# KevinSpevak/openVO

Hardware: AMD Instinct MI355X
Metric: stereo frame-pairs/sec (1280x720) (higher is better)
Workload: dtype int16

## Files before the change

openvo_amd/csrc/match.hip:

```cpp
#include "vo_internal.h"

typedef int v4i __attribute__((ext_vector_type(4)));

#define NIB(x, i) ((__umul24(__builtin_amdgcn_ubfe((x), 4 * (i), 4), 0x00204081u)) & 0x01010101u)
__device__ __forceinline__ void expand64(uint32_t lo, uint32_t hi, v4i (&o)[4])
{
    o[0] = (v4i){ (int)NIB(lo, 0), (int)NIB(lo, 1), (int)NIB(lo, 2), (int)NIB(lo, 3) };
    o[1] = (v4i){ (int)NIB(lo, 4), (int)NIB(lo, 5), (int)NIB(lo, 6), (int)NIB(lo, 7) };
    o[2] = (v4i){ (int)NIB(hi, 0), (int)NIB(hi, 1), (int)NIB(hi, 2), (int)NIB(hi, 3) };
    o[3] = (v4i){ (int)NIB(hi, 4), (int)NIB(hi, 5), (int)NIB(hi, 6), (int)NIB(hi, 7) };
}
#undef NIB

__device__ __forceinline__ uint32_t med3_u32(uint32_t a, uint32_t b, uint32_t c)
{
    uint32_t r;
    asm("v_med3_u32 %0, %1, %2, %3" : "=v"(r) : "v"(a), "v"(b), "v"(c));
    return r;
}

__device__ __forceinline__ void merge2(uint32_t& a0, uint32_t& a1, uint32_t b0, uint32_t b1)
{
    const uint32_t hi = max(a0, b0);
    a0 = min(a0, b0);
// ... 408 lines not shown
{
    if (!ctx || nq < 0 || nt < 0 || (nq && (!q || !idx || !dist)) || (nt && !t)) return vo_fail(ctx, VO_E_ARG, "vo_bf_knn2_hamming: bad argument");
    if (nq > ctx->kp_cap || nt > ctx->kp_cap) return vo_fail(ctx, VO_E_CAP, "descriptor count exceeds capacity %d", ctx->kp_cap);
    if (nq == 0) return VO_OK;
    VO_HIP(ctx, hipSetDevice(ctx->device));
    StageTimer tm(ctx, VO_T_MATCH);
    int rc = xfer_h2d(ctx, ctx->mq, q, (size_t)nq * 32);
    if (!rc && nt) rc = xfer_h2d(ctx, ctx->mt, t, (size_t)nt * 32);
    if (rc) return rc;
    rc = match_knn2(ctx, ctx->mq, nq, ctx->mt, nt, ctx->mw->m_idx, ctx->mw->m_dist);
    if (rc) return rc;
    rc = xfer_d2h(ctx, idx, ctx->mw->m_idx, (size_t)nq * 8);
    if (!rc) rc = xfer_d2h(ctx, dist, ctx->mw->m_dist, (size_t)nq * 8);
    if (rc) return rc;
    return xfer_flush(ctx);
}

__global__ void k_mutual_decode(const int32_t* __restrict__ idx, int nq, const uint32_t* __restrict__ colmin, const uint8_t* __restrict__ t, int nt,
                                uint8_t* __restrict__ mutual, int32_t* __restrict__ t_best)
{
    const int i = blockIdx.x * blockDim.x + threadIdx.x;
    if (i < nq) mutual[i] = knn_mutual(idx[2 * i], i, colmin, nt) ? 1 : 0;
    if (i < nt) {
        const uint32_t key = colmin[i];
        const uint4* tp = (const uint4*)(t + (size_t)i * 32);
        const uint4 a = tp[0], b = tp[1];
        const int tn = __popc(a.x) + __popc(a.y) + __popc(a.z) + __popc(a.w) + __popc(b.x) + __popc(b.y) + __popc(b.z) + __popc(b.w);
        const bool h = key != 0xFFFFFFFFu;
        t_best[2 * i] = h ? (int32_t)(key & 0xFFFFu) : -1;
        t_best[2 * i + 1] = h ? (int32_t)(key >> 16) - 256 + tn : 0x7FFFFFFF;
    }
}

extern "C" int vo_bf_knn2_hamming_mutual(vo_ctx* ctx, const uint8_t* q, int nq, const uint8_t* t, int nt, int32_t* idx, int32_t* dist,
                                         uint8_t* mutual, int32_t* t_best)
{
    if (!ctx || nq < 0 || nt < 0 || (nq && (!q || !idx || !dist || !mutual)) || (nt && !t))
        return vo_fail(ctx, VO_E_ARG, "vo_bf_knn2_hamming_mutual: bad argument");
    if (nq > ctx->kp_cap || nt > ctx->kp_cap) return vo_fail(ctx, VO_E_CAP, "descriptor count exceeds capacity %d", ctx->kp_cap);
    if (nq > 65535) return vo_fail(ctx, VO_E_CAP, "cross-check: query set of %d descriptors exceeds 65535", nq);
    if (t_best)
        for (int j = 0; j < nt; j++) { t_best[2 * j] = -1; t_best[2 * j + 1] = 0x7FFFFFFF; }
    if (nq == 0) return VO_OK;
    VO_HIP(ctx, hipSetDevice(ctx->device));
    StageTimer tm(ctx, VO_T_MATCH);
    int rc = xfer_h2d(ctx, ctx->mq, q, (size_t)nq * 32);
    if (!rc && nt) rc = xfer_h2d(ctx, ctx->mt, t, (size_t)nt * 32);
    if (rc) return rc;
    if ((rc = match_knn2(ctx, ctx->mq, nq, ctx->mt, nt, ctx->mw->m_idx, ctx->mw->m_dist, 1))) return rc;
    int32_t* d_tbest = (int32_t*)ctx->mw->xy_a;
    hipLaunchKernelGGL(k_mutual_decode, dim3(div_up(std::max(nq, std::max(nt, 1)), 256)), dim3(256), 0, ctx->stream, ctx->mw->m_idx, nq,
                       match_colmin(ctx->mw->m_dist, ctx->kp_cap), ctx->mt, nt, ctx->mw->st_a, d_tbest);
    VO_CHECK_LAUNCH(ctx);
    rc = xfer_d2h(ctx, idx, ctx->mw->m_idx, (size_t)nq * 8);
    if (!rc) rc = xfer_d2h(ctx, dist, ctx->mw->m_dist, (size_t)nq * 8);
    if (!rc) rc = xfer_d2h(ctx, mutual, ctx->mw->st_a, (size_t)nq);
    if (!rc && t_best && nt) rc = xfer_d2h(ctx, t_best, d_tbest, (size_t)nt * 8);
    if (rc) return rc;
    return xfer_flush(ctx);
}

extern "C" int vo_bf_knn2_hamming_window(vo_ctx* ctx, const uint8_t* q, int nq, const uint8_t* t, int nt, const float* xy_q, const float* xy_t, float rx,
                                         float ry, int match_flags, int32_t* idx, int32_t* dist, uint8_t* mutual, int32_t* t_best)
{
    const int cross = match_flags & VO_MATCH_CROSSCHECK;
    if (!ctx || nq < 0 || nt < 0 || (nq && (!q || !xy_q || !idx || !dist || (cross && !mutual))) || (nt && (!t || !xy_t)) ||
        (match_flags & ~(VO_MATCH_CROSSCHECK | VO_MATCH_WINDOW)))
        return vo_fail(ctx, VO_E_ARG, "vo_bf_knn2_hamming_window: bad argument");
    if (!(rx >= 0.f) || !(ry >= 0.f) || rx > 3.4028234e38f || ry > 3.4028234e38f)
        return vo_fail(ctx, VO_E_ARG, "vo_bf_knn2_hamming_window: the radii must be finite and >= 0");
    if (nq > ctx->kp_cap || nt > ctx->kp_cap) return vo_fail(ctx, VO_E_CAP, "descriptor count exceeds capacity %d", ctx->kp_cap);
    if (cross && nq > 65535) return vo_fail(ctx, VO_E_CAP, "cross-check: query set of %d descriptors exceeds 65535", nq);
    if (cross && t_best)
        for (int j = 0; j < nt; j++) { t_best[2 * j] = -1; t_best[2 * j + 1] = 0x7FFFFFFF; }
    if (nq == 0) return VO_OK;
    VO_HIP(ctx, hipSetDevice(ctx->device));
    StageTimer tm(ctx, VO_T_MATCH);
    int rc = xfer_h2d(ctx, ctx->mq, q, (size_t)nq * 32);
    if (!rc) rc = xfer_h2d(ctx, ctx->mw->xy_a, xy_q, (size_t)nq * 8);
    if (!rc && nt) rc = xfer_h2d(ctx, ctx->mt, t, (size_t)nt * 32);
    if (!rc && nt) rc = xfer_h2d(ctx, ctx->mw->xy_b, xy_t, (size_t)nt * 8);
    if (rc) return rc;
    if ((rc = match_knn2(ctx, ctx->mq, nq, ctx->mt, nt, ctx->mw->m_idx, ctx->mw->m_dist, cross, ctx->mw->xy_a, ctx->mw->xy_b, rx, ry))) return rc;
    int32_t* d_tbest = (int32_t*)ctx->mw->pts_a;
    if (cross) {
        hipLaunchKernelGGL(k_mutual_decode, dim3(div_up(std::max(nq, std::max(nt, 1)), 256)), dim3(256), 0, ctx->stream, ctx->mw->m_idx, nq,
                           match_colmin(ctx->mw->m_dist, ctx->kp_cap), ctx->mt, nt, ctx->mw->st_a, d_tbest);
        VO_CHECK_LAUNCH(ctx);
    }
    rc = xfer_d2h(ctx, idx, ctx->mw->m_idx, (size_t)nq * 8);
    if (!rc) rc = xfer_d2h(ctx, dist, ctx->mw->m_dist, (size_t)nq * 8);
    if (!rc && cross) rc = xfer_d2h(ctx, mutual, ctx->mw->st_a, (size_t)nq);
    if (!rc && cross && t_best && nt) rc = xfer_d2h(ctx, t_best, d_tbest, (size_t)nt * 8);
    if (rc) return rc;
    return xfer_flush(ctx);
}

static void alt_release(int kind, vo_ctx::AsyncAlt& p)
{
    if (p.stream) (void)hipStreamSynchronize(p.stream);
    match_ws_free(p.mw);
    if (p.result) (void)hipHostFree(p.result);
    if (p.done) (void)hipEventDestroy(p.done);
    if (p.stream && kind == vo_ctx::ALT_MONO) (void)hipStreamDestroy(p.stream);
    p = vo_ctx::AsyncAlt();
}

static int alt_prepare(vo_ctx* ctx, int kind, int k)
{
    vo_ctx::AsyncAlt& p = ctx->alt(kind, k);
    if (p.ready) return VO_OK;
    const bool pose = kind == vo_ctx::ALT_POSE;
    hipError_t e = hipSuccess;
    if (pose) {
        hipStream_t& shared = ctx->pose_streams[k % ctx->n_pose_streams];
        if (!shared) e = hipStreamCreateWithFlags(&shared, hipStreamNonBlocking);
        p.stream = shared;
    } else
        e = hipStreamCreateWithFlags(&p.stream, hipStreamNonBlocking);
    if (e == hipSuccess) e = hipEventCreateWithFlags(&p.done, hipEventDisableTiming);
    const size_t record = pose ? PNP_HDR + pnp_cap(ctx->kp_cap) * 9 + 64 : MONO_HDR + (size_t)ctx->kp_cap * (1 + 4 + 4 + 8) + 64;
    if (e == hipSuccess) e = hipHostMalloc((void**)&p.result, record, hipHostMallocDefault);
    if (e == hipSuccess) e = match_ws_alloc(ctx, p.mw, pose ? MATCH_WS_POSE : 0);
    if (e != hipSuccess) {
        alt_release(kind, p);
        return vo_fail(ctx, VO_E_HIP, "asynchronous %s step: allocation failed: %s", pose ? "pose" : "monocular", hipGetErrorString(e));
    }
    p.ready = true;
    return VO_OK;
}

void alt_free(vo_ctx* ctx)
{
    for (int kind : { vo_ctx::ALT_POSE, vo_ctx::ALT_MONO })
        for (int k = 0; k < vo_ctx::alt_count(kind); k++) alt_release(kind, ctx->alt(kind, k));
    for (hipStream_t& st : ctx->pose_streams) {
        if (st) (void)hipStreamDestroy(st);
        st = nullptr;
    }
}

int alt_open(vo_ctx* ctx, int kind, FrameSlot& a, FrameSlot& b, const char* who, int* k_out)
{
    const int n = vo_ctx::alt_count(kind), next = ctx->alt_next[kind];
    int k = -1;
    for (int i = 0; i < n && k < 0; i++)
        if (!ctx->alt(kind, (next + i) % n).busy) k = (next + i) % n;
    if (k < 0)
        return vo_fail(ctx, VO_E_STATE, "%s: every asynchronous %sstep is still open (end one first)", who, kind == vo_ctx::ALT_POSE ? "pose " : "");
    for (int i = 0; i < n; i++)
        if (int rc = alt_prepare(ctx, kind, (k + i) % n)) return rc;
    if (int rc = sweep_group_close_for(ctx, a)) return rc;
    if (int rc = sweep_group_close_for(ctx, b)) return rc;
    const hipStream_t st = ctx->alt(kind, k).stream;
    VO_HIP(ctx, hipEventRecord(ctx->ev0, ctx->stream));
    hipError_t e = hipStreamWaitEvent(st, ctx->ev0, 0);
    if (e == hipSuccess && a.pending) e = hipStreamWaitEvent(st, a.ready, 0);
    if (e == hipSuccess && b.pending) e = hipStreamWaitEvent(st, b.ready, 0);
    if (e != hipSuccess) return vo_fail(ctx, VO_E_HIP, "hipStreamWaitEvent failed: %s", hipGetErrorString(e));
    *k_out = k;
    return VO_OK;
}

int alt_close(vo_ctx* ctx, int kind, int k, FrameSlot& a, FrameSlot& b, int* ticket_out)
{
    vo_ctx::AsyncAlt& p = ctx->alt(kind, k);
    if (hipEventRecord(p.done, p.stream) != hipSuccess) return vo_fail(ctx, VO_E_HIP, "hipEventRecord failed");
    slot_add_reader(a, p.done);
    slot_add_reader(b, p.done);
    p.busy = true;
    ctx->alt_next[kind] = (k + 1) % vo_ctx::alt_count(kind);
    *ticket_out = k;
    return VO_OK;
}

int alt_ticket(vo_ctx* ctx, int kind, int ticket, bool args_ok, const char* who)
{
    if (!ctx || !args_ok || ticket < 0 || ticket >= vo_ctx::alt_count(kind)) return vo_fail(ctx, VO_E_ARG, "%s: bad argument", who);
    if (!ctx->alt(kind, ticket).busy) return vo_fail(ctx, VO_E_STATE, "%s: ticket %d is not open", who, ticket);
    return VO_OK;
}

int alt_wait(vo_ctx* ctx, vo_ctx::AsyncAlt& p)
{
    VO_HIP(ctx, hipSetDevice(ctx->device));
    p.busy = false;
    VO_HIP(ctx, hipEventSynchronize(p.done));
    return VO_OK;
}
```

openvo_amd/csrc/orb.hip:

```cpp
#include <math.h>
#include <algorithm>
#include "vo_internal.h"

#define NL VO_ORB_LEVELS
#define EDGE VO_ORB_EDGE
#define HALF_PATCH VO_ORB_HALF_PATCH
#define FAST_T 20
#ifndef ORB_FAST_GRID_CAP
#define ORB_FAST_GRID_CAP 2048
#endif
#ifndef ORB_CONE_W
#define ORB_CONE_W 64
#define ORB_CONE_H 48
#endif
#ifndef ORB_FAST_TH
#define ORB_FAST_TH 32
#endif
static_assert(ORB_FAST_TH % 4 == 0 && ORB_FAST_TH >= 4 && (64 + 2) * (ORB_FAST_TH + 2) < 65536, "k_orb_fast_nms: tile height");

struct LevelDev {
    int w, h;
    unsigned off;
    float scale;
    int quota;
    int xt, yt;
    int min_x, max_x, min_y, max_y;
    int cand_off;
};
struct LevelsDev { LevelDev l[NL]; int umax[HALF_PATCH + 2]; };

__constant__ int8_t c_pattern[1024] = {
#include "../../include/vo_orb_pattern.inc"
};

#define CNT_CAND 0
#define CNT_A 8
#define CNT_FIN 16
#define CNT_TOTAL 24
#define CNT_HIST 32

static int cv_round_f(float v) { return (int)nearbyintf(v); }

static void make_lin_coeffs(int srcsize, int dstsize, int32_t* ofs, uint16_t* coef, int* mn, int* mx)
{
    const double inv_scale = (double)dstsize / srcsize;
    const double scale = 1.0 / inv_scale;
    *mn = 0; *mx = dstsize;
    for (int v = 0; v < dstsize; v++) {
        volatile double t = scale * ((double)v + 0.5);
        double fval = t - 0.5;
        int ival = (int)floor(fval);
        ofs[v] = 0; coef[2 * v] = 256; coef[2 * v + 1] = 0;
        if (ival >= 0 && srcsize > 1) {
            if (ival < srcsize - 1) {
                ofs[v] = ival;
                int c1 = (int)nearbyint((fval - (double)ival) * 256.0);
                coef[2 * v + 1] = (uint16_t)c1;
                coef[2 * v] = (uint16_t)(256 - c1);
            } else {
                ofs[v] = srcsize - 1;
                if (v < *mx) *mx = v;
            }
        } else if (v + 1 > *mn)
            *mn = v + 1;
    }
}


int orb_prepare_tables(vo_ctx* ctx, int w, int h)
{
    if (ctx->orb_w == w && ctx->orb_h == h) return VO_OK;
    LevelsDev L;
    memset(&L, 0, sizeof(L));
    std::vector<int32_t> ofs;
    std::vector<uint16_t> coef;
    size_t off = 0;
    int cand_off = 0;
    for (int l = 0; l < NL; l++) {
        float scale = (float)pow((double)1.2f, (double)l);
        float inv = 1.0f / scale;
        LevelDev& d = L.l[l];
        d.w = cv_round_f((float)w * inv);
        d.h = cv_round_f((float)h * inv);
        d.scale = scale;
        d.off = (unsigned)off;
        off += ((size_t)d.w * d.h + 255) & ~(size_t)255;
        d.cand_off = cand_off;
        cand_off += ((d.w + 1) / 2) * ((d.h + 1) / 2);
        ctx->lv[l].w = d.w; ctx->lv[l].h = d.h; ctx->lv[l].off = d.off; ctx->lv[l].scale = scale;
        if (l > 0) {
            const LevelDev& p = L.l[l - 1];
            d.xt = (int)ofs.size();
            ofs.resize(ofs.size() + d.w); coef.resize(coef.size() + 2 * (size_t)d.w);
            make_lin_coeffs(p.w, d.w, ofs.data() + d.xt, coef.data() + 2 * (size_t)d.xt, &d.min_x, &d.max_x);
            d.yt = (int)ofs.size();
            ofs.resize(ofs.size() + d.h); coef.resize(coef.size() + 2 * (size_t)d.h);
            make_lin_coeffs(p.h, d.h, ofs.data() + d.yt, coef.data() + 2 * (size_t)d.yt, &d.min_y, &d.max_y);
        }
    }
    if (off > ctx->pyr_bytes) return vo_fail(ctx, VO_E_CAP, "pyramid of %dx%d exceeds the context capacity", w, h);
    std::vector<int32_t> rects;
    int pyr_nbx, pyr_nby, pyr_buf[2] = { 0, 0 }, pyr_tab = 0;
    {
        const LevelDev& top = L.l[NL - 1];
        pyr_nbx = std::max(1, std::min({ div_up(w, ORB_CONE_W), top.w / 8, 48 }));
        pyr_nby = std::max(1, std::min({ div_up(h, ORB_CONE_H), top.h / 8, 48 }));
        auto intervals = [&](int nb, bool xaxis, std::vector<int32_t>& out) {
            out.assign((size_t)NL * nb * 2, 0);
            for (int b = 0; b < nb; b++) {
                int nlo = 0, nhi = -1;
                for (int l = NL - 1; l >= 0; l--) {
                    const LevelDev& d = L.l[l];
                    const int size = xaxis ? d.w : d.h;
                    int lo = (int)((int64_t)b * size / nb), hi = (int)((int64_t)(b + 1) * size / nb) - 1;
                    if (l < NL - 1 && nlo <= nhi) {
                        const LevelDev& u = L.l[l + 1];
                        const int32_t* o = ofs.data() + (xaxis ? u.xt : u.yt);
                        const int mn = xaxis ? u.min_x : u.min_y, mx = xaxis ? u.max_x : u.max_y;
                        const int slo = nlo < mn ? 0 : (nlo >= mx ? size - 1 : o[nlo]);
                        const int shi = nhi < mn ? 0 : (nhi >= mx ? size - 1 : std::min(o[nhi] + 1, size - 1));
                        if (lo > hi) { lo = slo; hi = shi; }
                        else { lo = std::min(lo, slo); hi = std::max(hi, shi); }
                    }
                    out[((size_t)l * nb + b) * 2] = lo; out[((size_t)l * nb + b) * 2 + 1] = hi;
                    nlo = lo; nhi = hi;
                }
            }
        };
        std::vector<int32_t> rx, ry;
        intervals(pyr_nbx, true, rx);
        intervals(pyr_nby, false, ry);
        for (int l = 0; l < NL; l++) {
            int mw = 0, mh = 0;
            for (int b = 0; b < pyr_nbx; b++) mw = std::max(mw, rx[((size_t)l * pyr_nbx + b) * 2 + 1] - rx[((size_t)l * pyr_nbx + b) * 2] + 1);
            for (int b = 0; b < pyr_nby; b++) mh = std::max(mh, ry[((size_t)l * pyr_nby + b) * 2 + 1] - ry[((size_t)l * pyr_nby + b) * 2] + 1);
            pyr_buf[l & 1] = std::max(pyr_buf[l & 1], ((mw * mh + 15) & ~15));
            if (l > 0) pyr_tab = std::max(pyr_tab, std::max(mw, mh));
        }
        rects = rx;
        rects.insert(rects.end(), ry.begin(), ry.end());
        if (rects.size() > 4096 / 4 * 4) return vo_fail(ctx, VO_E_CAP, "pyramid cone table exceeds its capacity");
    }
    if ((size_t)cand_off > (size_t)ctx->cand_cap * 4) return vo_fail(ctx, VO_E_CAP, "candidate capacity exceeded");
    if (ofs.size() > (size_t)(ctx->max_w + ctx->max_h) * 2 * NL) return vo_fail(ctx, VO_E_CAP, "resize tables exceed capacity");
    {
        int vmax = (int)floor(HALF_PATCH * sqrt(2.f) / 2 + 1);
        int vmin = (int)ceil(HALF_PATCH * sqrt(2.f) / 2);
        for (int v = 0; v <= vmax; v++) L.umax[v] = (int)nearbyint(sqrt((double)HALF_PATCH * HALF_PATCH - v * v));
        for (int v = HALF_PATCH, v0 = 0; v >= vmin; --v) {
            while (L.umax[v0] == L.umax[v0 + 1]) ++v0;
            L.umax[v] = v0;
            ++v0;
        }
    }
    for (int k = 0; k < vo_ctx::MAX_ENGINES; k++)
        if (ctx->la_stream[k]) VO_HIP(ctx, hipStreamSynchronize(ctx->la_stream[k]));
    for (int kind : { vo_ctx::ALT_POSE, vo_ctx::ALT_MONO })
        for (int k = 0; k < vo_ctx::alt_count(kind); k++)
            if (ctx->alt(kind, k).stream) VO_HIP(ctx, hipStreamSynchronize(ctx->alt(kind, k).stream));
    VO_HIP(ctx, hipMemcpyAsync(ctx->rs_ofs, ofs.data(), ofs.size() * 4, hipMemcpyHostToDevice, ctx->stream));
    VO_HIP(ctx, hipMemcpyAsync(ctx->rs_coef, coef.data(), coef.size() * 2, hipMemcpyHostToDevice, ctx->stream));
    VO_HIP(ctx, hipMemcpyAsync(ctx->pyr_rects, rects.data(), rects.size() * 4, hipMemcpyHostToDevice, ctx->stream));
    VO_HIP(ctx, hipStreamSynchronize(ctx->stream));
    ctx->pyr_nbx = pyr_nbx; ctx->pyr_nby = pyr_nby; ctx->pyr_buf[0] = pyr_buf[0]; ctx->pyr_buf[1] = pyr_buf[1]; ctx->pyr_tab = pyr_tab;
    static_assert(sizeof(LevelsDev) <= sizeof(ctx->rs_meta_host), "level table too large");
    memcpy(ctx->rs_meta_host, &L, sizeof(L));
    ctx->orb_quota_nfeatures = -1;
    ctx->orb_w = w; ctx->orb_h = h;
    return VO_OK;
}

struct PyrArgs { int mask_mode, min_d16, max_d16, nbx, nby, bufA, bufB, tab; };

struct OrbJob {
    const uint8_t* img; const int16_t* disp16; const uint8_t* mask;
    uint8_t *pyr_img, *pyr_mask;
    int32_t *cand_pos, *candA_pos, *candB_pos, *counters;
    float *cand_resp, *candA_resp, *candB_resp;
    float *kp_xy, *kp_size, *kp_resp, *kp_angle;
    int32_t* kp_oct;
    uint8_t* desc;
    int32_t* n_kp_host;
    int img_stride, disp_stride, mask_stride, pad;
};
struct OrbJobs { OrbJob j[VO_MAX_SWEEP_GROUP]; };
static_assert(sizeof(LevelsDev) + sizeof(PyrArgs) + sizeof(OrbJobs) + 64 <= 4096, "the ORB kernels' arguments must fit one kernel-argument segment");

template <bool MASK>
__global__ void __launch_bounds__(256) k_orb_pyramid(const LevelsDev L, const PyrArgs A, const OrbJobs jobs, const int32_t* __restrict__ rects,
                                                     const int32_t* __restrict__ ofs, const uint16_t* __restrict__ coef)
{
    const OrbJob& job = jobs.j[blockIdx.z];
    const uint8_t* __restrict__ const src_img = job.img;
    const int16_t* __restrict__ const src_disp = job.disp16;
    const uint8_t* __restrict__ const src_mask = job.mask;
    const int img_stride = job.img_stride, disp_stride = job.disp_stride, mask_stride = job.mask_stride;
    uint8_t* __restrict__ const pimg = job.pyr_img;
    uint8_t* __restrict__ const pmask = job.pyr_mask;
    int32_t* __restrict__ const cnt = job.counters;
    extern __shared__ __attribute__((aligned(16))) uint8_t s_pyr_generic[];
    typedef __attribute__((address_space(3))) uint8_t lds8;
    typedef __attribute__((address_space(3))) uint16_t lds16;
    typedef __attribute__((address_space(3))) int lds32;
    lds8* const s_pyr = (lds8*)s_pyr_generic;
    const unsigned o_img[2] = { 0u, (unsigned)A.bufA }, o_msk[2] = { (unsigned)(A.bufA + A.bufB), (unsigned)(2 * A.bufA + A.bufB) };
    lds16* const taps = (lds16*)(s_pyr + (MASK ? 2 : 1) * (A.bufA + A.bufB));
    lds32* const s_rect = (lds32*)(taps + (size_t)(NL - 1) * 2 * A.tab * 4);
#define RECT(l, k) s_rect[(l) * 4 + (k)]
    const int bx = blockIdx.x, by = blockIdx.y, lane = threadIdx.x & 63, wv = threadIdx.x >> 6;
    if (bx == 0 && by == 0 && threadIdx.x < CNT_HIST) cnt[threadIdx.x] = 0;
    if (threadIdx.x < NL * 4) {
        const int l = threadIdx.x >> 2, k = threadIdx.x & 3;
        RECT(l, k) = k < 2 ? rects[(l * A.nbx + bx) * 2 + k] : rects[NL * A.nbx * 2 + (l * A.nby + by) * 2 + (k - 2)];
    }
    __syncthreads();
    {
        constexpr int TB = 8;
        const int ntap = (NL - 1) * 2 * A.tab;
        for (int ib = threadIdx.x; ib < ntap; ib += TB * blockDim.x) {
            int o0[TB], c0[TB], c1[TB], org[TB], kind[TB];
#pragma unroll
            for (int u = 0; u < TB; u++) {
                const int i = ib + u * blockDim.x;
                kind[u] = 0; o0[u] = 0; c0[u] = 256; c1[u] = 0; org[u] = 0;
                if (i >= ntap) continue;
                const int l = 1 + i / (2 * A.tab), j = i - (l - 1) * 2 * A.tab;
                const bool isx = j < A.tab;
                const int e = isx ? j : j - A.tab;
                const int lo = RECT(l, isx ? 0 : 2), hi = RECT(l, isx ? 1 : 3);
                if (e > hi - lo) continue;
                const LevelDev d = L.l[l];
                const LevelDev p = L.l[l - 1];
                const int v = lo + e;
                const int mn = isx ? d.min_x : d.min_y, mx = isx ? d.max_x : d.max_y, t0 = isx ? d.xt : d.yt;
                const int ssz = isx ? p.w : p.h;
                org[u] = RECT(l - 1, isx ? 0 : 2);
                if (v < mn) { kind[u] = 1; o0[u] = 0; }
                else if (v >= mx) { kind[u] = 1; o0[u] = ssz - 1; }
                else { kind[u] = 2; o0[u] = ofs[t0 + v]; c0[u] = coef[2 * (size_t)(t0 + v)]; c1[u] = coef[2 * (size_t)(t0 + v) + 1]; }
            }
#pragma unroll
            for (int u = 0; u < TB; u++) {
                if (!kind[u]) continue;
                lds16* t = taps + (size_t)(ib + u * blockDim.x) * 4;
                t[0] = (uint16_t)(o0[u] - org[u]); t[1] = (uint16_t)(o0[u] + (kind[u] == 2 ? 1 : 0) - org[u]); t[2] = (uint16_t)c0[u]; t[3] = (uint16_t)c1[u];
            }
        }
    }
    {
        const LevelDev d = L.l[0];
        const int x0 = RECT(0, 0), x1 = RECT(0, 1), y0 = RECT(0, 2), y1 = RECT(0, 3);
        const int nw = x1 - x0 + 1, nh = y1 - y0 + 1;
        lds8* const b0i = s_pyr + o_img[0];
        lds8* const b0m = s_pyr + o_msk[0];
        const int ox0 = (int)((long long)bx * d.w / A.nbx), ox1 = (int)((long long)(bx + 1) * d.w / A.nbx);
        const int oy0 = (int)((long long)by * d.h / A.nby), oy1 = (int)((long long)(by + 1) * d.h / A.nby);
        constexpr int RB0 = 12;
        for (int xx = lane; xx < nw; xx += 64) {
            const int x = x0 + xx;
            const bool ownx = x >= ox0 && x < ox1;
            for (int yb = wv; yb < nh; yb += 4 * RB0) {
                uint8_t v[RB0], m[RB0];
#pragma unroll
                for (int u = 0; u < RB0; u++) {
                    const int yy = min(yb + 4 * u, nh - 1), y = y0 + yy;
                    v[u] = src_img[(size_t)y * img_stride + x];
                    if (MASK) {
                        if (A.mask_mode == 1) {
                            const int dd = src_disp[(size_t)y * disp_stride + x];
                            m[u] = (dd >= A.min_d16 && dd <= A.max_d16) ? 255 : 0;
                        } else
                            m[u] = src_mask[(size_t)y * mask_stride + x];
                    }
                }
#pragma unroll
                for (int u = 0; u < RB0; u++) {
                    const int yy = yb + 4 * u, y = y0 + yy;
                    if (yy >= nh) break;
                    const bool own = ownx && y >= oy0 && y < oy1;
                    b0i[yy * nw + xx] = v[u];
                    if (own) pimg[(size_t)y * d.w + x] = v[u];
                    if (MASK) {
                        b0m[yy * nw + xx] = m[u];
                        if (own) pmask[(size_t)y * d.w + x] = m[u];
                    }
                }
            }
        }
    }
    __syncthreads();
    for (int l = 1; l < NL; l++) {
        const LevelDev d = L.l[l];
        const int x0 = RECT(l, 0), x1 = RECT(l, 1), y0 = RECT(l, 2), y1 = RECT(l, 3);
        const int nw = x1 - x0 + 1, nh = y1 - y0 + 1;
        const int pnw = RECT(l - 1, 1) - RECT(l - 1, 0) + 1;
        const int ox0 = (int)((long long)bx * d.w / A.nbx), ox1 = (int)((long long)(bx + 1) * d.w / A.nbx);
        const int oy0 = (int)((long long)by * d.h / A.nby), oy1 = (int)((long long)(by + 1) * d.h / A.nby);
        lds8* const di = s_pyr + o_img[l & 1];
        lds8* const dm = s_pyr + o_msk[l & 1];
        const lds8* const si = s_pyr + o_img[(l - 1) & 1];
        const lds8* const sm = s_pyr + o_msk[(l - 1) & 1];
        const lds16* const tx = taps + (size_t)(l - 1) * 2 * A.tab * 4;
        const lds16* const ty = tx + (size_t)A.tab * 4;
        for (int xx = lane; xx < nw; xx += 64) {
            const int x = x0 + xx;
            const unsigned a0 = tx[4 * xx], a1 = tx[4 * xx + 1], xc0 = tx[4 * xx + 2], xc1 = tx[4 * xx + 3];
            const bool ownx = x >= ox0 && x < ox1;
            for (int yb = wv; yb < nh; yb += 16) {
                unsigned r0[4], r1[4], yc0[4], yc1[4], ti[4][4], tm[4][4];
// ... 829 lines not shown
```

openvo_amd/csrc/sgbm.hip:

```cpp
#include "vo_internal.h"
#include <stdlib.h>
#include <algorithm>
#include <type_traits>

typedef short s16x2 __attribute__((ext_vector_type(2)));
typedef unsigned short u16x2 __attribute__((ext_vector_type(2)));

#define MAXC 0x7FFF
#define MAXC2 0x7FFF7FFFu
#define D2_EMPTY 0x7FFFFFFF

__device__ __forceinline__ s16x2 as_s(uint32_t v) { return __builtin_bit_cast(s16x2, v); }
__device__ __forceinline__ uint32_t as_u(s16x2 v) { return __builtin_bit_cast(uint32_t, v); }
__device__ __forceinline__ uint32_t pk_min(uint32_t a, uint32_t b) { return as_u(__builtin_elementwise_min(as_s(a), as_s(b))); }
__device__ __forceinline__ uint32_t pk_max(uint32_t a, uint32_t b) { return as_u(__builtin_elementwise_max(as_s(a), as_s(b))); }
__device__ __forceinline__ uint32_t pk_add(uint32_t a, uint32_t b) { return as_u(as_s(a) + as_s(b)); }
__device__ __forceinline__ uint32_t pk_sub(uint32_t a, uint32_t b) { return as_u(as_s(a) - as_s(b)); }
__device__ __forceinline__ uint32_t pk_add_sat(uint32_t a, uint32_t b) { return as_u(__builtin_elementwise_add_sat(as_s(a), as_s(b))); }
__device__ __forceinline__ uint32_t pk_sub_sat_u(uint32_t a, uint32_t b)
{
    return __builtin_bit_cast(uint32_t, __builtin_elementwise_sub_sat(__builtin_bit_cast(u16x2, a), __builtin_bit_cast(u16x2, b)));
}
__device__ __forceinline__ uint32_t pk_shr2(uint32_t a)
{
// ... 1207 lines not shown
}
__device__ __forceinline__ void uf_union(int* L, int a, int b)
{
    for (int it = 0; it < (1 << 24); it++) {
        a = uf_find_halve(L, a);
        b = uf_find_halve(L, b);
        if (a == b) return;
        if (a < b) { int t = a; a = b; b = t; }
        int old = atomicMin(&L[a], b);
        if (old == a) return;
        a = old;
    }
}

__global__ void __launch_bounds__(256) k_ccl_rows(const int16_t* __restrict__ img, int W, int newVal, int maxDiff,
                                                 int* __restrict__ L, int* __restrict__ runlen, int* __restrict__ size)
{
    __shared__ int s_tot[256];
    const int y = blockIdx.x, tid = threadIdx.x;
    const int per = (W + 255) / 256;
    const int xa = tid * per, xb = min(xa + per, W);
    const int16_t* r = img + (size_t)y * W;
    int last = -1;
    for (int x = xa; x < xb; x++) {
        const int v = r[x];
        const bool valid = v != newVal;
        const bool start = valid && (x == 0 || r[x - 1] == newVal || abs(v - r[x - 1]) > maxDiff);
        if (start) last = x;
    }
    s_tot[tid] = last;
    __syncthreads();
    for (int o = 1; o < 256; o <<= 1) {
        int v = tid >= o ? s_tot[tid - o] : -1;
        __syncthreads();
        s_tot[tid] = max(s_tot[tid], v);
        __syncthreads();
    }
    int cur = tid > 0 ? s_tot[tid - 1] : -1;
    for (int x = xa; x < xb; x++) {
        const int v = r[x];
        const size_t i = (size_t)y * W + x;
        if (v == newVal) { L[i] = -1; continue; }
        const bool start = x == 0 || r[x - 1] == newVal || abs(v - r[x - 1]) > maxDiff;
        if (start) { cur = x; size[i] = 0; }
        L[i] = y * W + cur;
        const bool end = x == W - 1 || r[x + 1] == newVal || abs(v - r[x + 1]) > maxDiff;
        if (end) runlen[(size_t)y * W + cur] = x - cur + 1;
    }
}

#define RUN_TOUCH (1 << 30)
__global__ void k_ccl_vmerge(PostJobs jobs, int W, int H, int newVal, int maxDiff, int maxSize)
{
    const PostJob& job = jobs.j[blockIdx.z];
    const int16_t* __restrict__ const img = job.dst;
    int* __restrict__ const L = job.L;
    int* __restrict__ const runlen = job.runlen;
    const int x = blockIdx.x * blockDim.x + threadIdx.x;
    if (x >= W) return;
    for (int y = blockIdx.y; y + 1 < H; y += gridDim.y) {
    const int i = y * W + x;
    const int v = img[i], u = img[i + W];
    if (v == newVal || u == newVal || abs(v - u) > maxDiff) continue;
    const int a = L[i], b = L[i + W];
    bool head_a = x == 0, head_b = x == 0, joined_left = false;
    if (x > 0) {
        const int v1 = img[i - 1], u1 = img[i + W - 1];
        head_a = v1 == newVal || abs(v - v1) > maxDiff;
        head_b = u1 == newVal || abs(u - u1) > maxDiff;
        joined_left = v1 != newVal && u1 != newVal && abs(v1 - u1) <= maxDiff && !head_a && !head_b;
    }
    if (joined_left) continue;
    const int ha = head_a ? i : a, hb = head_b ? i + W : b;
    const int la = ((volatile int*)runlen)[ha], lb = ((volatile int*)runlen)[hb];
    const bool big_a = (la & ~RUN_TOUCH) > maxSize, big_b = (lb & ~RUN_TOUCH) > maxSize;
    if (big_a && big_b) continue;
    if (big_a != big_b) {
        const int hs = big_a ? hb : ha, ls = big_a ? lb : la;
        if (!(ls & RUN_TOUCH)) atomicOr(&runlen[hs], RUN_TOUCH);
        continue;
    }
    uf_union(L, a, b);
    }
}

__global__ void k_ccl_sizes(PostJobs jobs, int W, int H, int newVal, int maxDiff, int maxSize)
{
    const PostJob& job = jobs.j[blockIdx.z];
    const int16_t* __restrict__ const img = job.dst;
    int* __restrict__ const L = job.L;
    const int* __restrict__ const runlen = job.runlen;
    int* __restrict__ const size = job.size;
    const int x = blockIdx.x * blockDim.x + threadIdx.x;
    if (x >= W) return;
    for (int y = blockIdx.y; y < H; y += gridDim.y) {
    const int i = y * W + x;
    const int v = img[i];
    if (v == newVal) continue;
    const bool start = x == 0 || img[i - 1] == newVal || abs(v - img[i - 1]) > maxDiff;
    if (!start) continue;
    const int root = uf_find_halve(L, i);
    L[i] = root;
    if (((volatile int*)size)[root] > maxSize) continue;
    const int len = runlen[i];
    atomicAdd(&size[root], (len & ~RUN_TOUCH) + ((len & RUN_TOUCH) ? maxSize + 1 : 0));
    }
}

__global__ void k_ccl_apply(PostJobs jobs, int n, int newVal, int maxSize)
{
    const PostJob& job = jobs.j[blockIdx.y];
    int16_t* __restrict__ const img = job.dst;
    const int* __restrict__ const L = job.L;
    const int* __restrict__ const size = job.size;
    for (int i = blockIdx.x * blockDim.x + threadIdx.x; i < n; i += gridDim.x * blockDim.x) {
        const int r = L[i];
        if (r >= 0 && size[uf_find(L, r)] <= maxSize) img[i] = (int16_t)newVal;
    }
}

static PathPlan make_plan(const SgbmGeom& g, int mode)
{
    static const int sx5[] = { 1, -1, 1, -1, 0 }, sy5[] = { 0, 0, 1, 1, 1 };
    static const int sx8[] = { 1, -1, 1, -1, 1, -1, 0, 0 }, sy8[] = { 0, 0, 1, 1, -1, -1, -1, 1 };
    PathPlan p;
    p.n_dirs = mode == 1 ? 8 : 5;
    p.first_wave[0] = 0;
    for (int k = 0; k < p.n_dirs; k++) {
        p.sx[k] = mode == 1 ? sx8[k] : sx5[k];
        p.sy[k] = mode == 1 ? sy8[k] : sy5[k];
        p.nlines[k] = p.sy[k] == 0 ? g.H : (p.sx[k] == 0 ? g.W1 : g.W1 + g.H - 1);
        p.first_wave[k + 1] = p.first_wave[k] + div_up(p.nlines[k], 4);
    }
    for (int k = p.n_dirs; k < VO_MAX_DIRS; k++) { p.sx[k] = p.sy[k] = p.nlines[k] = 0; p.first_wave[k + 1] = p.first_wave[p.n_dirs]; }
    return p;
}

static int ensure_S(vo_ctx* ctx, int vols)
{
    if (ctx->ws->S_vols >= vols) return VO_OK;
    if (ctx->ws->S) (void)hipFree(ctx->ws->S);
    ctx->ws->S = nullptr; ctx->ws->S_vols = 0;
    VO_HIP(ctx, hipMalloc((void**)&ctx->ws->S, ctx->vol_cells * sizeof(int16_t) * vols + 256));
    ctx->ws->S_vols = vols;
    return VO_OK;
}

static_assert(VO_MAX_SWEEP_GROUP == DG_MAXJOBS, "include/vo355.h promises what one sweep launch carries");
struct SweepGroup {
    typedef int (*Launch)(vo_ctx*, const DiagJobs&, const SgbmGeom&);
    typedef int (*WeLaunch)(vo_ctx*, const WeJobs&, int, const SgbmGeom&);
    struct Member {
        int engine;
        FrameSlot* f;
        int w, h;
        SgbmGeom g;
        DiagJob job;
        WeJob we;
        PostJob post;
    };
    Launch launch = nullptr;
    WeLaunch we_launch = nullptr;
    int nstrips = 0;
    int n = 0;
    Member m[DG_MAXJOBS];
    bool want_defer = false, did_defer = false;
    Member cand;
    Launch cand_launch = nullptr;
    WeLaunch cand_we_launch = nullptr;
    int cand_nstrips = 0;
};

template <int NP>
static int we2_launch_jobs(vo_ctx* ctx, const WeJobs& jobs, int n, const SgbmGeom& g)
{
    const dim3 grid(n, div_up(div_up(g.H, 4), 2));
    if (g.D != g.Dp) hipLaunchKernelGGL((k_sgbm_we2<NP, true>), grid, dim3(256), 0, ctx->stream, jobs, g, ctx->dump);
    else hipLaunchKernelGGL((k_sgbm_we2<NP, false>), grid, dim3(256), 0, ctx->stream, jobs, g, ctx->dump);
    VO_CHECK_LAUNCH(ctx);
    return VO_OK;
}

template <int NP, bool PAD, int NWC, bool REV, bool WTA>
static int diag_launch_jobs(vo_ctx* ctx, const DiagJobs& jobs, const SgbmGeom& g)
{
    constexpr int UW = 4 * NWC, CW = UW + 2;
    const size_t lds = (size_t)DG_RING * 2 * CW * g.Dp * 2 + (WTA ? (size_t)NWC * 4 * 2 * g.Dp * 2 : 0) + 64 * 4;
    auto kern = k_sgbm_diag<NP, PAD, NWC, REV, WTA>;
    if (int rca = lds_allow_big(ctx, (const void*)kern)) return rca;
    const int per = ctx->tune_diag_wgs > 0 ? ctx->tune_diag_wgs : div_up(g.W1, UW) + 2;
    const int wgs = jobs.n * min(jobs.nstrips, per);
    hipLaunchKernelGGL(kern, dim3(wgs), dim3((NWC + 1) * 64), lds, ctx->stream, jobs, g, jobs.j[0].ctl, ctx->dump, ctx->sw_ctl_words / 2);
    VO_CHECK_LAUNCH(ctx);
    return VO_OK;
}

template <int NP, bool PAD, int NWC, bool REV, bool WTA>
static int launch_diag_k(vo_ctx* ctx, const SgbmGeom& g, const int16_t* in1, int16_t* sout, int* ctl)
{
    constexpr int UW = 4 * NWC;
    DiagJobs jobs;
    memset(&jobs, 0, sizeof(jobs));
    jobs.n = 1;
    jobs.nstrips = div_up(g.W1 + g.H - 1, UW);
    const size_t need = (size_t)jobs.nstrips * (g.H + 1) * DG_GLANES * NP * sizeof(uint64_t);
    bool cleared = false;
    if (need > ctx->ws->sw_bnd_bytes) {
        if (ctx->ws->sw_bnd) (void)hipFree(ctx->ws->sw_bnd);
        ctx->ws->sw_bnd = nullptr; ctx->ws->sw_bnd_bytes = 0;
        VO_HIP(ctx, hipMalloc((void**)&ctx->ws->sw_bnd, need + 256));
        ctx->ws->sw_bnd_bytes = need;
        VO_HIP(ctx, hipMemsetAsync(ctx->ws->sw_bnd, 0, need, ctx->stream));
        cleared = true;
    }
    DiagJob& j = jobs.j[0];
    j.C = ctx->ws->C; j.in1 = in1; j.sout = sout; j.bnd = ctx->ws->sw_bnd; j.aux0 = ctx->ws->rec; j.aux1 = ctx->ws->rec + (size_t)ctx->max_w * ctx->max_h + 64;
    j.tag = ++ctx->ws->sw_tag;
    if (j.tag == 0) j.tag = ++ctx->ws->sw_tag;
    j.sink = ctx->max_w * ctx->max_h;
    j.dbg = ctx->tune_diag_dbg;
    j.spin_limit = ctx->tune_spin_limit;
    j.vol_bytes = (uint32_t)(((size_t)g.W1 * g.H + 1) * g.Dp * 2);
    j.rec_bytes = (uint32_t)(((size_t)ctx->max_w * ctx->max_h + 64) * 4);
    j.ctl = ctl;
    if (ctx->fault_sweep > 0 && --ctx->fault_sweep == 0) {
        j.dbg |= 2;
        j.spin_limit = 64;
    }
    if constexpr (WTA && !REV) {
        SweepGroup* const G = ctx->grp;
        if (G && G->want_defer) {
            if (cleared) VO_HIP(ctx, hipEventRecord(ctx->ws_alt[ctx->cur_engine].mid, ctx->stream));
            G->cand.job = j; G->cand.g = g;
            G->cand_launch = &diag_launch_jobs<NP, PAD, NWC, REV, WTA>;
            G->cand_nstrips = jobs.nstrips;
            G->did_defer = true;
            return VO_OK;
        }
    }
    return diag_launch_jobs<NP, PAD, NWC, REV, WTA>(ctx, jobs, g);
}

template <int NP, bool REV, bool WTA>
static int launch_diag(vo_ctx* ctx, const SgbmGeom& g, const int16_t* in1, int16_t* sout, int* ctl)
{
    const bool pad = g.D != g.Dp;
    if constexpr (NP <= 4) {
        const int nwc = ctx->tune_diag_nwc ? ctx->tune_diag_nwc : (ctx->cur_engine >= 0 ? 11 : 7);
        if (nwc == 15)
            return pad ? launch_diag_k<NP, true, 15, REV, WTA>(ctx, g, in1, sout, ctl) : launch_diag_k<NP, false, 15, REV, WTA>(ctx, g, in1, sout, ctl);
        if (nwc == 11)
            return pad ? launch_diag_k<NP, true, 11, REV, WTA>(ctx, g, in1, sout, ctl) : launch_diag_k<NP, false, 11, REV, WTA>(ctx, g, in1, sout, ctl);
    }

    return pad ? launch_diag_k<NP, true, 7, REV, WTA>(ctx, g, in1, sout, ctl) : launch_diag_k<NP, false, 7, REV, WTA>(ctx, g, in1, sout, ctl);
}

template <int NP>
static int launch_agg(vo_ctx* ctx, const SgbmGeom& g, const PathPlan& plan, size_t vol)
{
    const bool pad = g.D != g.Dp;
    const bool hh = plan.n_dirs == 8;
    int rc;
    if (g.ur < 100) {
        if ((rc = ensure_S(ctx, 3))) return rc;
        int16_t* const Swe = ctx->ws->S;
        int16_t* const Srev = ctx->ws->S + vol;
        int16_t* const ck = ctx->ws->S + 2 * vol;
        int* const ctlA = ctx->ws->sw_ctl;
        int* const ctlB = ctx->ws->sw_ctl + ctx->sw_ctl_words / 2;
        const bool cut = g.W1 % 16 == 0 && g.W1 >= 32 && !(ctx->tune_diag_dbg & 8);
        SweepGroup* const G = ctx->grp;
        const bool defer_we = cut && G && G->want_defer && !hh && !(ctx->tune_diag_dbg & 16);
        if (G) G->cand_we_launch = nullptr;
        {
            StageTimer t(ctx, VO_T_SGBM_AGG, defer_we ? 0 : 1);
            if (ctx->tune_diag_dbg & 8) {
            } else if (cut) {
                WeJobs wj;
                memset(&wj, 0, sizeof(wj));
                wj.j[0].C = ctx->ws->C; wj.j[0].Swe = Swe; wj.j[0].ckpt = ck;
                if (defer_we) {
                    G->cand.we = wj.j[0];
                    G->cand_we_launch = &we2_launch_jobs<NP>;
                } else if ((rc = we2_launch_jobs<NP>(ctx, wj, 1, g))) return rc;
            } else if (g.W1 % 8 == 0 && g.W1 >= 16) {
                const int nw = div_up(g.H, 4);
                if (pad) hipLaunchKernelGGL((k_sgbm_we<NP, true>), dim3(div_up(nw, 4)), dim3(256), 0, ctx->stream, ctx->ws->C, Swe, ck, g, ctx->dump);
                else hipLaunchKernelGGL((k_sgbm_we<NP, false>), dim3(div_up(nw, 4)), dim3(256), 0, ctx->stream, ctx->ws->C, Swe, ck, g, ctx->dump);
            } else {
                PathPlan pp = plan;
                pp.n_dirs = 1;
                pp.sx[0] = 1; pp.sy[0] = 0; pp.nlines[0] = g.H;
                pp.first_wave[0] = 0;
                for (int k = 0; k < VO_MAX_DIRS; k++) pp.first_wave[k + 1] = div_up(g.H, 4);
                for (int k = 1; k < VO_MAX_DIRS; k++) pp.sx[k] = pp.sy[k] = pp.nlines[k] = 0;
                const int nwp = pp.first_wave[1];
                if (pad) hipLaunchKernelGGL((k_sgbm_pair<NP, true>), dim3(div_up(nwp, 4)), dim3(256), 0, ctx->stream, ctx->ws->C, Swe, ck, vol, g, pp, ctx->dump);
                else hipLaunchKernelGGL((k_sgbm_pair<NP, false>), dim3(div_up(nwp, 4)), dim3(256), 0, ctx->stream, ctx->ws->C, Swe, ck, vol, g, pp, ctx->dump);
            }
            VO_CHECK_LAUNCH(ctx);
            if (ctx->cur_engine >= 0 && ctx->ws_alt[ctx->cur_engine].mid) {
                vo_ctx::SgbmWs& a = ctx->ws_alt[ctx->cur_engine];
                if (hipEventRecord(a.mid, ctx->stream) == hipSuccess) a.mid_valid = true;
            }
            if (hh && (rc = launch_diag<NP, true, false>(ctx, g, Swe, Srev, ctlA))) return rc;
        }
        {
            StageTimer t(ctx, VO_T_SGBM_WTA, ctx->grp && ctx->grp->want_defer ? 0 : 1);
            if (!(ctx->tune_diag_dbg & 16) && (rc = launch_diag<NP, false, true>(ctx, g, hh ? Srev : Swe, nullptr, hh ? ctlB : ctlA))) return rc;
        }
        ctx->last_paths = 3;
        ctx->last_schedule = (g.W1 % 8 == 0 && g.W1 >= 16) ? VO_SCHED_DIAG : VO_SCHED_DIAG_RAGGED;
        return VO_OK;
    }
    if ((rc = ensure_S(ctx, plan.n_dirs))) return rc;
    {
        StageTimer t(ctx, VO_T_SGBM_AGG);
        const int nwaves = plan.first_wave[plan.n_dirs];
        constexpr int PF = NP <= 4 ? 8 : 4;
        if (pad) hipLaunchKernelGGL((k_sgbm_paths<NP, PF, true>), dim3(div_up(nwaves, 4)), dim3(256), 0, ctx->stream, ctx->ws->C, ctx->ws->S, vol, g, plan, ctx->dump);
        else hipLaunchKernelGGL((k_sgbm_paths<NP, PF, false>), dim3(div_up(nwaves, 4)), dim3(256), 0, ctx->stream, ctx->ws->C, ctx->ws->S, vol, g, plan, ctx->dump);
        VO_CHECK_LAUNCH(ctx);
    }
    {
        StageTimer t(ctx, VO_T_SGBM_WTA);
        const size_t sh = (size_t)16 * g.Dp * sizeof(int16_t);
        const long long npix = (long long)g.W1 * g.H;
        hipLaunchKernelGGL((k_sgbm_wta<NP>), dim3((unsigned)((npix + 15) / 16)), dim3(256), sh, ctx->stream, ctx->ws->S, vol, plan.n_dirs,
                           g, ctx->ws->disp_tmp, ctx->ws->ccl_size);
        VO_CHECK_LAUNCH(ctx);
    }
    ctx->last_paths = plan.n_dirs;
    ctx->last_schedule = VO_SCHED_UNFUSED;
    return VO_OK;
}

static int sgbm_run_impl(vo_ctx* ctx, FrameSlot& f, int w, int h, const uint8_t* srcL, const uint8_t* srcR);
static int sgbm_post(vo_ctx* ctx, FrameSlot& f, int w, int h, const SgbmGeom& g);
static PostJob post_job(const vo_ctx* ctx, const FrameSlot& f);
static int sgbm_post_launch(vo_ctx* ctx, const PostJobs& jobs, int n, const SgbmGeom& g, bool rows);
static uint32_t pk_rep_host(int v) { return (uint32_t)(v & 0xFFFF) * 0x00010001u; }
static int post_rows_per_block(int w) { return std::min(6, (int)(150 * 1024 / ((size_t)w * 6)) - 2); }

static int sgbm_run_done(vo_ctx* ctx)
{
    if (ctx->ws == &ctx->main_ws && ctx->ws->done) {
        VO_HIP(ctx, hipEventRecord(ctx->ws->done, ctx->stream));
        ctx->ws->done_valid = true;
        ctx->ws->done_on_engine0 = false;
    }
    return VO_OK;
}

int sgbm_run(vo_ctx* ctx, FrameSlot& f, int w, int h, const uint8_t* srcL, const uint8_t* srcR, bool* deferred)
{
    int rc;
    if (deferred) *deferred = false;
    if (ctx->cur_engine < 0 && sweep_group_has_engine(ctx, 0) && (rc = sweep_group_close(ctx, VO_GRP_CONSUMER))) return rc;
    const bool shared = ctx->ws == &ctx->main_ws;
    if (shared && ctx->ws->done_valid && !(ctx->cur_engine == 0 && ctx->ws->done_on_engine0)) VO_HIP(ctx, hipStreamWaitEvent(ctx->stream, ctx->ws->done, 0));
    if (++ctx->sweep_gen_next <= 0) ctx->sweep_gen_next = 1;
    f.disp_gen = ctx->sweep_gen_next;
    const bool defer = deferred && ctx->cur_engine >= 0 && sweep_group_size(ctx) > 1 && ctx->sg.set && ctx->sg.ur < 100 && ctx->sg.mode == 0 &&
                       ctx->ws_alt[ctx->cur_engine].mid != nullptr;
    if (defer) {
        if (!ctx->grp) ctx->grp = new SweepGroup();
        ctx->grp->want_defer = true;
        ctx->grp->did_defer = false;
    }
    rc = sgbm_run_impl(ctx, f, w, h, srcL, srcR);
    if (defer) {
        SweepGroup* const G = ctx->grp;
        G->want_defer = false;
        if (!rc && G->did_defer) {
            G->did_defer = false;
            if (G->n > 0 && (G->n >= DG_MAXJOBS || G->launch != G->cand_launch || G->we_launch != G->cand_we_launch || G->nstrips != G->cand_nstrips ||
                             memcmp(&G->m[0].g, &G->cand.g, sizeof(SgbmGeom))) &&
                (rc = sweep_group_close(ctx, VO_GRP_OTHER)))
                return rc;
            SweepGroup::Member& m = G->m[G->n++];
            m = G->cand;
            m.engine = ctx->cur_engine; m.f = &f; m.w = w; m.h = h;
            m.post = post_job(ctx, f);
            G->launch = G->cand_launch; G->we_launch = G->cand_we_launch; G->nstrips = G->cand_nstrips;
            f.in_group = true;
            *deferred = true;
            return VO_OK;
        }
    }
    if (int rcd = sgbm_run_done(ctx)) return rcd;
    return rc;
}

bool sweep_group_has_engine(const vo_ctx* ctx, int engine)
{
    if (ctx->grp)
        for (int i = 0; i < ctx->grp->n; i++)
            if (ctx->grp->m[i].engine == engine) return true;
    return false;
}
int sweep_group_members(const vo_ctx* ctx) { return ctx->grp ? ctx->grp->n : 0; }
void sweep_group_free(vo_ctx* ctx) { delete ctx->grp; ctx->grp = nullptr; }

struct MemberScope {
    vo_ctx* c;
    hipStream_t stream; uint8_t* stage_in; vo_ctx::SgbmWs* ws; OrbWs* orbws; int cur_engine;
    explicit MemberScope(vo_ctx* ctx) : c(ctx), stream(ctx->stream), stage_in(ctx->stage_in), ws(ctx->ws), orbws(ctx->orbws), cur_engine(ctx->cur_engine) {}
    void enter(int e)
    {
        c->stream = c->la_stream[e]; c->stage_in = c->la_stage[e];
        c->ws = e == 0 ? &c->main_ws : &c->ws_alt[e]; c->orbws = &c->ws_alt[e].orb; c->cur_engine = e;
    }
    ~MemberScope() { c->stream = stream; c->stage_in = stage_in; c->ws = ws; c->orbws = orbws; c->cur_engine = cur_engine; }
    MemberScope(const MemberScope&) = delete;
    MemberScope& operator=(const MemberScope&) = delete;
};

static int sweep_member_back(vo_ctx* ctx, SweepGroup::Member& m)
{
    FrameSlot& f = *m.f;
    int rc = sgbm_post(ctx, f, m.w, m.h, m.g);
    if (!rc) rc = sgbm_run_done(ctx);
    if (!rc && ctx->la_orb) {
        const int* q = ctx->la_orb_params;
        rc = orb_slot_enqueue(ctx, f, q[0], q[1], q[2], q[3]);
        if (!rc) { memcpy(f.kp_params, q, sizeof(f.kp_params)); f.kp_pending = true; }
    }
    if (!rc && hipEventRecord(f.ready, ctx->stream) != hipSuccess) rc = vo_fail(ctx, VO_E_HIP, "hipEventRecord failed");
    return rc;
}

int engine_behind_chain(vo_ctx* ctx, int engine)
{
    vo_ctx::SgbmWs& a = ctx->ws_alt[engine];
    if (!a.chain) return VO_OK;
    if (hipEventQuery(a.chain) != hipSuccess) {
        (void)hipGetLastError();
        VO_HIP(ctx, hipStreamWaitEvent(ctx->la_stream[engine], a.chain, 0));
    }
    a.chain = nullptr;
    return VO_OK;
}

int sweep_group_close(vo_ctx* ctx, int why)
{
    SweepGroup* const G = ctx->grp;
    if (!G || G->n == 0) return VO_OK;
    (void)hipSetDevice(ctx->device);
    const int n = G->n;
    G->n = 0;
    for (int i = 0; i < n; i++) G->m[i].f->in_group = false;
    ctx->grp_closed[why]++;
    int rc = VO_OK;
    {
        MemberScope scope(ctx);
        SweepGroup::Member& last = G->m[n - 1];
        scope.enter(last.engine);
        DiagJobs jobs;
        WeJobs we;
        PostJobs post;
        memset(&jobs, 0, sizeof(jobs));
        memset(&we, 0, sizeof(we));
        memset(&post, 0, sizeof(post));
        jobs.n = n; jobs.nstrips = G->nstrips;
        jobs.j[0] = last.job; we.j[0] = last.we; post.j[0] = last.post;
        bool main_member = last.engine == 0;
        for (int i = 0; i + 1 < n && !rc; i++) {
            jobs.j[i + 1] = G->m[i].job; we.j[i + 1] = G->m[i].we; post.j[i + 1] = G->m[i].post;
            main_member |= G->m[i].engine == 0;
            const vo_ctx::SgbmWs& a = ctx->ws_alt[G->m[i].engine];
            if (!a.mid_valid || hipStreamWaitEvent(ctx->stream, a.mid, 0) != hipSuccess) rc = vo_fail(ctx, VO_E_HIP, "sweep group: waiting for a member's early stages failed");
        }
        if (!rc && G->we_launch) {
            StageTimer t(ctx, VO_T_SGBM_AGG, n);
            rc = G->we_launch(ctx, we, n, last.g);
        }
        if (!rc) {
            StageTimer t(ctx, VO_T_SGBM_WTA, n);
            rc = G->launch(ctx, jobs, last.g);
        }
        const bool post_here = post_rows_per_block(last.g.W) >= 1;
        if (!rc && post_here) {
            if (!(ctx->tune_diag_dbg & 32)) {
                StageTimer t(ctx, VO_T_SGBM_POST, n);
                rc = sgbm_post_launch(ctx, post, n, last.g, true);
            }
            if (!rc && main_member && ctx->main_ws.done) {
                if (hipEventRecord(ctx->main_ws.done, ctx->stream) == hipSuccess) { ctx->main_ws.done_valid = true; ctx->main_ws.done_on_engine0 = false; }
                else rc = vo_fail(ctx, VO_E_HIP, "hipEventRecord failed");
            }
        }
        hipEvent_t const swept = ctx->ws_alt[last.engine].swept;
        if (!rc && post_here) {
            if (ctx->la_orb) {
                const int* q = ctx->la_orb_params;
                FrameSlot* fs[DG_MAXJOBS];
                OrbWs* ows[DG_MAXJOBS];
                for (int i = 0; i < n; i++) { fs[i] = G->m[i].f; ows[i] = &ctx->ws_alt[G->m[i].engine].orb; }
                rc = orb_slots_enqueue(ctx, fs, ows, n, q[0], q[1], q[2], q[3]);
                for (int i = 0; i < n && !rc; i++) { memcpy(fs[i]->kp_params, q, sizeof(fs[i]->kp_params)); fs[i]->kp_pending = true; }
            }
            for (int i = 0; i < n && !rc; i++)
                if (hipEventRecord(G->m[i].f->ready, ctx->stream) != hipSuccess) rc = vo_fail(ctx, VO_E_HIP, "hipEventRecord failed");
            if (!rc && n > 1) {
                if (hipEventRecord(swept, ctx->stream) != hipSuccess) rc = vo_fail(ctx, VO_E_HIP, "hipEventRecord failed");
                for (int i = 0; i + 1 < n && !rc; i++) ctx->ws_alt[G->m[i].engine].chain = swept;
            }
            if (!rc && main_member) ctx->main_ws.done_on_engine0 = last.engine == 0;
        } else if (!rc) {
            if (n > 1 && hipEventRecord(swept, ctx->stream) != hipSuccess) rc = vo_fail(ctx, VO_E_HIP, "hipEventRecord failed");
            if (!rc) rc = sweep_member_back(ctx, last);
            for (int i = 0; i + 1 < n && !rc; i++) {
                scope.enter(G->m[i].engine);
                if (hipStreamWaitEvent(ctx->stream, swept, 0) != hipSuccess) rc = vo_fail(ctx, VO_E_HIP, "hipStreamWaitEvent failed");
                if (!rc) rc = sweep_member_back(ctx, G->m[i]);
            }
        }
    }
    if (rc) {
        for (int i = 0; i < n; i++) {
            FrameSlot& f = *G->m[i].f;
            f.kp_pending = false; f.has_pair = false; f.has_disp = false;
            if (f.counted && ctx->inflight > 0) ctx->inflight--;
            f.counted = false;
        }
    }
    return rc;
}

static int sgbm_run_impl(vo_ctx* ctx, FrameSlot& f, int w, int h, const uint8_t* srcL, const uint8_t* srcR)
{
    const uint8_t* const dL = srcL ? srcL : f.left;
    const uint8_t* const dR = srcL ? srcR : f.right;
    int16_t* const d_disp = f.disp16;
    const SgbmEff& e = ctx->sg;
    if (!e.set) return vo_fail(ctx, VO_E_STATE, "vo_set_sgbm has not been called");
    SgbmGeom g;
    g.W = w; g.H = h; g.D = e.D; g.Dp = (e.D + 31) & ~31; g.minD = e.minD; g.P1 = e.P1; g.P2 = e.P2; g.ur = e.ur; g.d12 = e.d12;
    g.ftzero = e.ftzero; g.SW2 = e.SW2;
    {
        const int u = 100 - e.ur;
        g.urM = u > 1 ? (uint32_t)((0x100000000ull + (uint64_t)u - 1) / (uint64_t)u) : 0xFFFFFFFFu;
        g.urAdd = u > 1 ? (uint32_t)(u - 1) : 1u;
    }
    g.minX1 = e.maxD > 0 ? e.maxD : 0;
    int maxX1 = w + (e.minD < 0 ? e.minD : 0);
    g.W1 = maxX1 - g.minX1;
    g.invalid16 = (e.minD - 1) * 16;
    const int n = w * h;
    if (g.W1 <= 0) {
        if (srcL) {
            VO_HIP(ctx, hipMemcpyAsync(f.left, srcL, (size_t)n, hipMemcpyDeviceToDevice, ctx->stream));
            VO_HIP(ctx, hipMemcpyAsync(f.right, srcR, (size_t)n, hipMemcpyDeviceToDevice, ctx->stream));
        }
        std::vector<int16_t> inv((size_t)n, (int16_t)g.invalid16);
        VO_HIP(ctx, hipMemcpyAsync(d_disp, inv.data(), (size_t)n * 2, hipMemcpyHostToDevice, ctx->stream));
        VO_HIP(ctx, hipStreamSynchronize(ctx->stream));
        ctx->last_cells = 0;
        return VO_OK;
    }
    const size_t vol = (size_t)g.W1 * h * g.Dp;
    if (vol > ctx->vol_cells || e.D > 256)
        return vo_fail(ctx, VO_E_CAP, "cost volume %zu cells exceeds the capacity given to vo_create (or D > 256)", vol);
    if (((size_t)g.W1 * h + 1) * g.Dp * 2 >= 0xFFFFFF00ull)
        return vo_fail(ctx, VO_E_CAP, "cost volume of %zu bytes exceeds the 4 GiB a volume kernel addresses", ((size_t)g.W1 * h + 1) * g.Dp * 2);
    const PathPlan plan = make_plan(g, e.mode);
    ctx->last_cells = (int64_t)g.W1 * h * g.D;
    {
        StageTimer t(ctx, VO_T_SGBM_COST);
        const int dbg = ctx->tune_diag_dbg;
        hipLaunchKernelGGL(k_sgbm_planes, dim3(div_up(w, 256), std::min(h, 128)), dim3(256), 0, ctx->stream, dL, dR, w, h, g.ftzero,
                           ctx->ws->planesL, ctx->ws->planesR, (g.ur >= 100 || post_rows_per_block(w) < 1) ? ctx->ws->ccl_size : nullptr, ctx->ws->sw_ctl, ctx->sw_ctl_words,
                           (uint32_t*)(ctx->ws->C + vol), g.Dp / 2, pk_rep_host(g.P2), srcL ? f.left : nullptr, srcL ? f.right : nullptr);
        const int bx = ((g.Dp / 2 + 63) / 64) * 64;
        const int TY = ctx->tune_sweep_ty;
        const int nw = bx / 64;
#define LAUNCH_SWEEP(XT, SW)                                                                                                   \
    hipLaunchKernelGGL((k_sgbm_cost_sweep<XT, SW>), dim3(8 * div_up(div_up(g.W1, XT) * div_up(h, TY), 8)), dim3(bx),            \
                       (size_t)nw * (((2 * SW + 1) <= 5 ? 0 : (2 * SW + 1) * XT * 64) + 12 * (64 + (XT + 2 * SW - 1) / 2)) * 4, ctx->stream, ctx->ws->planesL, ctx->ws->planesR, g, TY, ctx->ws->C)
        if (dbg & 4) {
        } else
        switch (g.SW2) {
            case 0: LAUNCH_SWEEP(8, 0); break;
            case 1: LAUNCH_SWEEP(8, 1); break;
            case 2: LAUNCH_SWEEP(8, 2); break;
            case 3: LAUNCH_SWEEP(8, 3); break;
            case 4: LAUNCH_SWEEP(8, 4); break;
            case 5: LAUNCH_SWEEP(8, 5); break;
            default:
                hipLaunchKernelGGL(k_sgbm_cost_generic, dim3(g.W1, h), dim3(bx), 0, ctx->stream, ctx->ws->planesL, ctx->ws->planesR, g, ctx->ws->C);
        }
#undef LAUNCH_SWEEP
        VO_CHECK_LAUNCH(ctx);
    }
    int rc;
    switch (g.Dp / 32) {
        case 1: rc = launch_agg<1>(ctx, g, plan, vol); break;
        case 2: rc = launch_agg<2>(ctx, g, plan, vol); break;
        case 3: rc = launch_agg<3>(ctx, g, plan, vol); break;
        case 4: rc = launch_agg<4>(ctx, g, plan, vol); break;
        case 5: rc = launch_agg<5>(ctx, g, plan, vol); break;
        case 6: rc = launch_agg<6>(ctx, g, plan, vol); break;
        case 7: rc = launch_agg<7>(ctx, g, plan, vol); break;
        default: rc = launch_agg<8>(ctx, g, plan, vol); break;
    }
    if (rc) return rc;
    if (ctx->grp && ctx->grp->did_defer) return VO_OK;
    return sgbm_post(ctx, f, w, h, g);
}

static PostJob post_job(const vo_ctx* ctx, const FrameSlot& f)
{
    PostJob j;
    j.aux0 = ctx->ws->rec; j.aux1 = ctx->ws->rec + (size_t)ctx->max_w * ctx->max_h + 64;
    j.dst = f.disp16;
    j.L = ctx->ws->ccl_label; j.runlen = ctx->ws->ccl_runlen; j.size = ctx->ws->ccl_size;
    j.ctlA = ctx->ws->sw_ctl; j.ctlB = ctx->ws->sw_ctl + ctx->sw_ctl_words / 2;
    j.sweep_word = f.sweep_word; j.gen = f.disp_gen;
    return j;
}

static int sgbm_post_launch(vo_ctx* ctx, const PostJobs& jobs, int n, const SgbmGeom& g, bool rows)
{
    const SgbmEff& e = ctx->sg;
    const int w = g.W, h = g.H, npix = w * h;
    const int newVal = g.invalid16, maxDiff = 16 * e.speckleRange;
    const bool speckle = e.speckleWindow > 0;
    if (rows) {
        const int rb = post_rows_per_block(w);
        if (int rca = lds_allow_big(ctx, (const void*)k_sgbm_post_rows)) return rca;
        hipLaunchKernelGGL(k_sgbm_post_rows, dim3(div_up(h, rb), n), dim3(512), (size_t)(rb + 2) * w * 6, ctx->stream, jobs, g, rb, speckle ? 1 : 0, maxDiff,
                           ctx->d_sweep_errs);
    }
    if (speckle) {
        hipLaunchKernelGGL(k_ccl_vmerge, dim3(div_up(w, 256), std::min(h, 128), n), dim3(256), 0, ctx->stream, jobs, w, h, newVal, maxDiff, e.speckleWindow);
        hipLaunchKernelGGL(k_ccl_sizes, dim3(div_up(w, 256), std::min(h, 128), n), dim3(256), 0, ctx->stream, jobs, w, h, newVal, maxDiff, e.speckleWindow);
        hipLaunchKernelGGL(k_ccl_apply, dim3(std::min(div_up(npix, 256), 1024), n), dim3(256), 0, ctx->stream, jobs, npix, newVal, e.speckleWindow);
    }
    VO_CHECK_LAUNCH(ctx);
    return VO_OK;
}

static int sgbm_post(vo_ctx* ctx, FrameSlot& f, int w, int h, const SgbmGeom& g)
{
    const SgbmEff& e = ctx->sg;
    int16_t* const d_disp = f.disp16;
    const bool fused = g.ur < 100;
    if (!(ctx->tune_diag_dbg & 32)) {
        StageTimer t(ctx, VO_T_SGBM_POST);
        const int newVal = g.invalid16, maxDiff = 16 * e.speckleRange;
        const bool speckle = e.speckleWindow > 0;
        PostJobs jobs;
        memset(&jobs, 0, sizeof(jobs));
        jobs.j[0] = post_job(ctx, f);
        const bool rows = fused && post_rows_per_block(w) >= 1;
        if (!rows) {
            if (fused) {
                hipLaunchKernelGGL(k_sgbm_fin, dim3(div_up(g.W1, 256), g.H), dim3(256), 0, ctx->stream, ctx->ws->rec, ctx->ws->rec + (size_t)ctx->max_w * ctx->max_h + 64,
                                   g, ctx->ws->disp_tmp, ctx->ws->ccl_size, ctx->ws->sw_ctl, ctx->ws->sw_ctl + ctx->sw_ctl_words / 2, f.sweep_word, f.disp_gen, ctx->d_sweep_errs);
            }
            hipLaunchKernelGGL(k_lr_median3, dim3(div_up(w, 256), h), dim3(256), 0, ctx->stream, ctx->ws->disp_tmp, ctx->ws->ccl_size, g, d_disp);
            if (speckle)
                hipLaunchKernelGGL(k_ccl_rows, dim3(h), dim3(256), 0, ctx->stream, d_disp, w, newVal, maxDiff, ctx->ws->ccl_label, ctx->ws->ccl_runlen, ctx->ws->ccl_size);
            VO_CHECK_LAUNCH(ctx);
        }
        return sgbm_post_launch(ctx, jobs, 1, g, rows);
    }
// ... 3 lines not shown
```

openvo_amd/csrc/vo_ctx.hip:

```cpp
#include <stdarg.h>
#include <stdlib.h>
#include "vo_internal.h"

int vo_fail(vo_ctx* ctx, int code, const char* fmt, ...)
{
    char buf[1024];
    va_list ap;
    va_start(ap, fmt);
    vsnprintf(buf, sizeof(buf), fmt, ap);
    va_end(ap);
    if (ctx) ctx->err = buf;
    return code;
}

static thread_local std::string g_create_err;

static const size_t ARENA_BASE = 4096;

static void* arena_take(vo_ctx* ctx, size_t bytes)
{
    const size_t need = (bytes + 63) & ~(size_t)63;
    if (ARENA_BASE + ctx->arena_off + need > ctx->pinned_bytes) return nullptr;
    void* p = (char*)ctx->pinned + ARENA_BASE + ctx->arena_off;
    ctx->arena_off += need;
    return p;
}

void* xfer_stage(vo_ctx* ctx, size_t bytes) { return arena_take(ctx, bytes); }

int xfer_flush(vo_ctx* ctx)
{
    VO_HIP(ctx, hipStreamSynchronize(ctx->stream));
    for (const auto& c : ctx->pending) memcpy(c.dst, c.src, c.bytes);
    ctx->pending.clear();
    ctx->arena_off = 0;
    return VO_OK;
}

int xfer_h2d(vo_ctx* ctx, void* dev_dst, const void* host_src, size_t bytes)
{
    if (bytes == 0) return VO_OK;
    void* st = arena_take(ctx, bytes);
    if (!st && bytes + 64 <= ctx->pinned_bytes - ARENA_BASE) {
        int rc = xfer_flush(ctx);
        if (rc) return rc;
        st = arena_take(ctx, bytes);
    }
    if (!st) {
        VO_HIP(ctx, hipMemcpyAsync(dev_dst, host_src, bytes, hipMemcpyHostToDevice, ctx->stream));
        return VO_OK;
    }
    memcpy(st, host_src, bytes);
    VO_HIP(ctx, hipMemcpyAsync(dev_dst, st, bytes, hipMemcpyHostToDevice, ctx->stream));
    return VO_OK;
}

int xfer_d2h(vo_ctx* ctx, void* host_dst, const void* dev_src, size_t bytes)
{
    if (bytes == 0) return VO_OK;
    void* st = arena_take(ctx, bytes);
    if (!st && bytes + 64 <= ctx->pinned_bytes - ARENA_BASE) {
        int rc = xfer_flush(ctx);
        if (rc) return rc;
        st = arena_take(ctx, bytes);
    }
    if (!st) {
        VO_HIP(ctx, hipMemcpyAsync(host_dst, dev_src, bytes, hipMemcpyDeviceToHost, ctx->stream));
        return VO_OK;
    }
    VO_HIP(ctx, hipMemcpyAsync(st, dev_src, bytes, hipMemcpyDeviceToHost, ctx->stream));
    ctx->pending.push_back({host_dst, st, bytes});
    return VO_OK;
}

template <typename T>
static int dalloc(vo_ctx* ctx, T** p, size_t count)
{
    VO_HIP(ctx, hipMalloc((void**)p, count * sizeof(T) + 256));
    return VO_OK;
}
#define DALLOC(p, n)                         \
    do {                                     \
        int rc__ = dalloc(ctx, &(p), (n));   \
        if (rc__) { g_create_err = ctx->err; vo_destroy(ctx); return rc__; } \
    } while (0)

extern "C" const char* vo_last_error(const vo_ctx* ctx)
{
    return ctx ? ctx->err.c_str() : g_create_err.c_str();
}

int orb_ws_alloc(vo_ctx* ctx, OrbWs& o)
{
    const size_t cand = (size_t)ctx->cand_cap * 4 * sizeof(int32_t);
    void** ps[] = { (void**)&o.pyr_img, (void**)&o.pyr_mask,
                    (void**)&o.cand_pos, (void**)&o.cand_resp, (void**)&o.candA_pos, (void**)&o.candA_resp, (void**)&o.candB_pos,
                    (void**)&o.candB_resp, (void**)&o.counters };
    const size_t sz[] = { ctx->pyr_bytes, ctx->pyr_bytes, cand, cand, cand, cand, cand,
                          cand, 8192 * 4 };
    for (size_t k = 0; k < sizeof(ps) / sizeof(ps[0]); k++)
        if (hipMalloc(ps[k], sz[k] + 256) != hipSuccess) return VO_E_HIP;
    return VO_OK;
}

void orb_ws_free(OrbWs& o)
{
    void* ps[] = { o.pyr_img, o.pyr_mask, o.cand_pos, o.cand_resp, o.candA_pos, o.candA_resp,
                   o.candB_pos, o.candB_resp, o.counters };
    for (void* p : ps) if (p) (void)hipFree(p);
    o = OrbWs();
}

static void sgbm_ws_free(vo_ctx::SgbmWs& a)
{
    void** ps[] = { (void**)&a.planesL, (void**)&a.planesR, (void**)&a.C, (void**)&a.S, (void**)&a.sw_ctl, (void**)&a.disp_tmp,
                    (void**)&a.ccl_runlen, (void**)&a.ccl_label, (void**)&a.ccl_size, (void**)&a.rec, (void**)&a.sw_bnd };
    for (void** q : ps) { if (*q) (void)hipFree(*q); *q = nullptr; }
    if (a.done) (void)hipEventDestroy(a.done);
    a.done = nullptr;
    a.S_vols = 0; a.sw_bnd_bytes = 0; a.ready = false; a.done_valid = false;
}

static hipError_t sgbm_ws_alloc(vo_ctx* ctx, vo_ctx::SgbmWs& a)
{
    const size_t npx = (size_t)ctx->max_w * ctx->max_h;
    const int vols = 3;
    void** ps[] = { (void**)&a.planesL, (void**)&a.planesR, (void**)&a.C, (void**)&a.S, (void**)&a.sw_ctl, (void**)&a.disp_tmp,
                    (void**)&a.ccl_runlen, (void**)&a.ccl_label, (void**)&a.ccl_size, (void**)&a.rec };
    const size_t sz[] = { npx * 2 * 4, npx * 6 * 4, ctx->vol_cells * 2, ctx->vol_cells * 2 * vols, ctx->sw_ctl_words * sizeof(int), npx * 2,
                          npx * 4, npx * 4, npx * 4, (npx + 64) * 8 };
    hipError_t e = hipSuccess;
    for (size_t k = 0; k < sizeof(ps) / sizeof(ps[0]) && e == hipSuccess; k++) e = hipMalloc(ps[k], sz[k] + 256);
    if (e == hipSuccess) e = dev_zero(a.sw_ctl, ctx->sw_ctl_words * sizeof(int));
    if (e == hipSuccess && !a.done) e = hipEventCreateWithFlags(&a.done, hipEventDisableTiming);
    if (e != hipSuccess) { sgbm_ws_free(a); return e; }
    a.S_vols = vols;
    a.ready = true;
    return hipSuccess;
}

int lds_allow_big(vo_ctx* ctx, const void* fn)
{
    for (const void* f : ctx->big_lds) if (f == fn) return VO_OK;
    VO_HIP(ctx, hipFuncSetAttribute(fn, hipFuncAttributeMaxDynamicSharedMemorySize, 160 * 1024));
    ctx->big_lds.push_back(fn);
    return VO_OK;
}

extern "C" int vo_create(int device_id, int max_w, int max_h, int max_disp, int max_kp, vo_ctx** out)
{
    if (!out) return VO_E_ARG;
    *out = nullptr;
    if (max_w < 64 || max_h < 64 || max_disp < 16 || max_disp > 256 || max_disp % 16 || max_kp < 16) {
        g_create_err = "vo_create: need max_w,max_h >= 64, 16 <= max_disp <= 256 (multiple of 16), max_kp >= 16";
        return VO_E_ARG;
    }
    int ndev = 0;
    hipError_t e = hipGetDeviceCount(&ndev);
    if (e != hipSuccess || ndev <= 0) {
        g_create_err = std::string("vo_create: no HIP device available (") + hipGetErrorString(e) +
                       "); libvo355 has no CPU fallback";
        return VO_E_HIP;
    }
    if (device_id < 0 || device_id >= ndev) { g_create_err = "vo_create: bad device id"; return VO_E_ARG; }
    vo_ctx* ctx = new vo_ctx();
    ctx->device = device_id;
    ctx->max_w = max_w; ctx->max_h = max_h; ctx->max_disp = max_disp; ctx->max_kp = max_kp;
    if ((e = hipSetDevice(device_id)) != hipSuccess) { g_create_err = hipGetErrorString(e); delete ctx; return VO_E_HIP; }
    hipDeviceProp_t prop;
    if (hipGetDeviceProperties(&prop, device_id) == hipSuccess) {
        char generic[96];
        snprintf(generic, sizeof(generic), "AMD GPU, %d CUs, %.0f GB", prop.multiProcessorCount, (double)prop.totalGlobalMem / 1e9);
        snprintf(ctx->devname, sizeof(ctx->devname), "%s (%s)", prop.name[0] ? prop.name : generic, prop.gcnArchName);
    }
    if ((e = hipStreamCreateWithFlags(&ctx->stream, hipStreamNonBlocking)) != hipSuccess) { g_create_err = hipGetErrorString(e); delete ctx; return VO_E_HIP; }
    (void)hipEventCreate(&ctx->ev0);
    (void)hipEventCreate(&ctx->ev1);

    const size_t npx = (size_t)max_w * max_h;
    ctx->kp_cap = max_kp * 2 + 1024;
    for (int s = 0; s <= VO_NUM_SLOTS; s++) {
        FrameSlot& f = ctx->slots[s];
        DALLOC(f.left, npx); DALLOC(f.right, npx); DALLOC(f.disp16, npx);
        (void)hipEventCreateWithFlags(&f.ready, hipEventDisableTiming);
        DALLOC(f.kp_xy, (size_t)ctx->kp_cap * 2); DALLOC(f.kp_size, ctx->kp_cap); DALLOC(f.kp_angle, ctx->kp_cap);
        DALLOC(f.kp_resp, ctx->kp_cap); DALLOC(f.kp_oct, ctx->kp_cap); DALLOC(f.desc, (size_t)ctx->kp_cap * 32);
        DALLOC(f.mono_depth, ctx->kp_cap); DALLOC(f.mono_serial_dev, 16);
        DALLOC(f.kp_xyz, (size_t)ctx->kp_cap * 3); DALLOC(f.kp_disp, ctx->kp_cap); DALLOC(f.kp_rdesc, (size_t)ctx->kp_cap * 32);
        if (dev_zero(f.mono_serial_dev, 64) != hipSuccess) { g_create_err = "clearing a slot's depth serial failed"; vo_destroy(ctx); return VO_E_HIP; }
    }
    {
        FrameSlot& r = ctx->sparse_r;
        DALLOC(r.kp_xy, (size_t)ctx->kp_cap * 2); DALLOC(r.kp_size, ctx->kp_cap); DALLOC(r.kp_angle, ctx->kp_cap);
        DALLOC(r.kp_resp, ctx->kp_cap); DALLOC(r.kp_oct, ctx->kp_cap); DALLOC(r.desc, (size_t)ctx->kp_cap * 32);
        ctx->sp_main.l = &ctx->slots[VO_NUM_SLOTS]; ctx->sp_main.r = &r;
    }
    ctx->stage_bytes = npx * 3;
    DALLOC(ctx->stage_in, ctx->stage_bytes * 2);
    for (int c = 0; c < 2; c++) { DALLOC(ctx->map1[c], npx * 2); DALLOC(ctx->map2[c], npx); }
    ctx->vol_cells = npx * (size_t)((max_disp + 31) & ~31);
    ctx->sw_ctl_words = 2 * 2048;
    if (sgbm_ws_alloc(ctx, ctx->main_ws) != hipSuccess) { g_create_err = "hipMalloc failed (SGBM workspace)"; vo_destroy(ctx); return VO_E_HIP; }
    DALLOC(ctx->dump, 4096);
    ctx->pyr_bytes = npx * 4;
    DALLOC(ctx->rs_ofs, (size_t)(max_w + max_h) * 2 * VO_ORB_LEVELS);
    DALLOC(ctx->rs_coef, (size_t)(max_w + max_h) * 4 * VO_ORB_LEVELS);
    DALLOC(ctx->pyr_rects, 4096);
    ctx->cand_cap = (int)((size_t)((max_w + 1) / 2) * ((max_h + 1) / 2));
    if (orb_ws_alloc(ctx, (*ctx->orbws))) { g_create_err = "hipMalloc failed (ORB workspace)"; vo_destroy(ctx); return VO_E_HIP; }
    DALLOC(ctx->host_mask_dev, npx);
    DALLOC(ctx->mq, (size_t)ctx->kp_cap * 32); DALLOC(ctx->mt, (size_t)ctx->kp_cap * 32);
    if (match_ws_alloc(ctx, ctx->main_mw, MATCH_WS_POSE) != hipSuccess) { g_create_err = "hipMalloc failed (match scratch)"; vo_destroy(ctx); return VO_E_HIP; }
    DALLOC(ctx->red, 4096);
    ctx->pinned_bytes = 8 << 20;
    if (hipHostMalloc(&ctx->pinned, ctx->pinned_bytes, hipHostMallocDefault) != hipSuccess ||
        hipHostMalloc((void**)&ctx->slot_words, 256 * sizeof(int32_t), hipHostMallocDefault) != hipSuccess) {
        g_create_err = "hipHostMalloc failed"; vo_destroy(ctx); return VO_E_HIP;
    }
    memset(ctx->slot_words, 0, 256 * sizeof(int32_t));
    static_assert(128 + 4 * (VO_NUM_SLOTS + 1) <= 256 && VO_NUM_SLOTS + 1 <= 32, "slot_words layout");
    for (int s = 0; s <= VO_NUM_SLOTS; s++) {
        ctx->slots[s].n_kp_host = ctx->slot_words + s; ctx->slots[s].sweep_word = ctx->slot_words + 64 + s;
        ctx->slots[s].sp_rec = ctx->slot_words + 128 + 4 * s;
    }
    ctx->sparse_r.n_kp_host = ctx->slot_words + 32;
    DALLOC(ctx->d_sweep_errs, 64);
    if (dev_zero(ctx->d_sweep_errs, 64 * sizeof(int)) != hipSuccess) { g_create_err = "clearing the sweep error counter failed"; vo_destroy(ctx); return VO_E_HIP; }
    if (const char* e8 = getenv("VO_ENGINES")) { int v = atoi(e8); if (v >= 1 && v <= vo_ctx::MAX_ENGINES) ctx->n_engines = v; }
    {
        const double per_engine = (double)ctx->vol_cells * 2.0 * 5.0 + (double)npx * 64.0;
        size_t free_b = 0, total_b = 0;
        double budget = 96e9;
        if (hipMemGetInfo(&free_b, &total_b) == hipSuccess) budget = 0.4 * (double)free_b;
        const int fit = (int)(budget / per_engine);
        ctx->engines_fit = fit < 2 ? 2 : fit;
        if (ctx->n_engines > ctx->engines_fit) ctx->n_engines = ctx->engines_fit;
    }
    if (const char* eq = getenv("GPU_MAX_HW_QUEUES")) { int v = atoi(eq); if (v >= 1) ctx->hw_queues = v; }
    if (const char* eg = getenv("VO_SWEEP_GROUP")) { int v = atoi(eg); if (v >= 1 && v <= VO_MAX_SWEEP_GROUP) ctx->sweep_group_req = v; }
    if (const char* e9 = getenv("VO_POSE_STREAMS")) { int v = atoi(e9); if (v >= 1 && v <= vo_ctx::N_POSE_STREAMS) ctx->n_pose_streams = v; }
    if (const char* e27 = getenv("VO_STAGGER")) ctx->tune_stagger = atoi(e27);
    if (const char* e25 = getenv("VO_DIAG_WAVES")) { const int v = atoi(e25); ctx->tune_diag_nwc = (v == 7 || v == 11 || v == 15) ? v : 0; }
#ifdef VO_TEST_HOOKS
    if (const char* e27 = getenv("VO_DIAG_WGS")) ctx->tune_diag_wgs = atoi(e27);
    if (const char* e26 = getenv("VO_DIAG_DEBUG")) ctx->tune_diag_dbg = atoi(e26);
    if (const char* e10 = getenv("VO_FAULT_PREFETCH")) ctx->fault_prefetch = atoi(e10);
    if (const char* e11 = getenv("VO_FAULT_SWEEP")) ctx->fault_sweep = atoi(e11);
    if (const char* e12 = getenv("VO_FAULT_PNP_RANGE")) ctx->fault_pnp_range = atoi(e12);
#endif
    if (const char* e6 = getenv("VO_SWEEP_TY")) { int v = atoi(e6); if (v >= 4 && v <= 4096) ctx->tune_sweep_ty = v; }
    *out = ctx;
    return VO_OK;
}

extern "C" void vo_destroy(vo_ctx* ctx)
{
    if (!ctx) return;
    (void)hipSetDevice(ctx->device);
    (void)sweep_group_close(ctx, VO_GRP_OTHER);
    sweep_group_free(ctx);
    if (ctx->stage_thread.joinable()) {
        { std::lock_guard<std::mutex> lk(ctx->stage_mu); ctx->stage_stop = true; }
        ctx->stage_cv.notify_all();
        ctx->stage_thread.join();
    }
    for (int k = 0; k < vo_ctx::MAX_ENGINES; k++) if (ctx->la_stream[k]) (void)hipStreamSynchronize(ctx->la_stream[k]);
    if (ctx->stream) (void)hipStreamSynchronize(ctx->stream);
    for (int s = 0; s <= VO_NUM_SLOTS; s++) {
        FrameSlot& f = ctx->slots[s];
        void* ps[] = { f.left, f.right, f.disp16, f.kp_xy, f.kp_size, f.kp_angle, f.kp_resp, f.kp_oct, f.desc, f.mono_depth, f.mono_serial_dev,
                       f.kp_xyz, f.kp_disp, f.kp_rdesc };
        for (void* p : ps) if (p) (void)hipFree(p);
        if (f.ready) (void)hipEventDestroy(f.ready);
    }
    void* ps[] = { ctx->stage_in, ctx->map1[0], ctx->map1[1], ctx->map2[0], ctx->map2[1], ctx->dump, ctx->rs_ofs, ctx->rs_coef, ctx->pyr_rects,
                   ctx->host_mask_dev, ctx->mq, ctx->mt, ctx->red, ctx->img3_ws, ctx->d_sweep_errs, ctx->sparse_r.kp_xy, ctx->sparse_r.kp_size,
                   ctx->sparse_r.kp_angle, ctx->sparse_r.kp_resp, ctx->sparse_r.kp_oct, ctx->sparse_r.desc };
    for (void* p : ps) if (p) (void)hipFree(p);
    alt_free(ctx);
    for (LandmarkMap& m : ctx->maps) map_free(m);
    sparse_ws_free(ctx->sp_main);
    for (SparseWs& w : ctx->sp_alt) sparse_ws_free(w);
    match_ws_free(ctx->main_mw);
    sgbm_ws_free(ctx->main_ws);
    orb_ws_free(ctx->main_ws.orb);
    if (ctx->pinned) (void)hipHostFree(ctx->pinned);
    if (ctx->slot_words) (void)hipHostFree(ctx->slot_words);
    for (hipEvent_t e : ctx->ev_pool) (void)hipEventDestroy(e);
    if (ctx->staged) (void)hipFree(ctx->staged);
    for (int k = 0; k < vo_ctx::MAX_ENGINES; k++) {
        vo_ctx::SgbmWs& a = ctx->ws_alt[k];
        sgbm_ws_free(a);
        orb_ws_free(a.orb);
        if (ctx->la_stage[k]) (void)hipFree(ctx->la_stage[k]);
        if (a.pinned) (void)hipHostFree(a.pinned);
        if (a.h2d_done) (void)hipEventDestroy(a.h2d_done);
        if (a.mid) (void)hipEventDestroy(a.mid);
        if (a.swept) (void)hipEventDestroy(a.swept);
        if (ctx->la_stream[k]) (void)hipStreamDestroy(ctx->la_stream[k]);
    }
    for (vo_ctx::HostStage& hs : ctx->host_stage) {
        if (hs.pinned) (void)hipHostFree(hs.pinned);
        if (hs.h2d_done) (void)hipEventDestroy(hs.h2d_done);
    }
    if (ctx->ev0) (void)hipEventDestroy(ctx->ev0);
    if (ctx->ev1) (void)hipEventDestroy(ctx->ev1);
    if (ctx->stream) (void)hipStreamDestroy(ctx->stream);
    delete ctx;
}

extern "C" int vo_set_engines(vo_ctx* ctx, int n)
{
    if (!ctx) return VO_E_ARG;
    if (n > 0) {
        if (int rc = sweep_group_close(ctx, VO_GRP_OTHER)) return rc;
        if (n > vo_ctx::MAX_ENGINES) n = vo_ctx::MAX_ENGINES;
        if (n > ctx->engines_fit) n = ctx->engines_fit;
        ctx->n_engines = n;
        ctx->next_engine %= n;
    }
    return ctx->n_engines;
}

extern "C" int vo_set_sweep_group(vo_ctx* ctx, int n)
{
    if (!ctx) return VO_E_ARG;
    if (n > 0) {
        if (int rc = sweep_group_close(ctx, VO_GRP_OTHER)) return rc;
        ctx->sweep_group_req = n > VO_MAX_SWEEP_GROUP ? VO_MAX_SWEEP_GROUP : n;
    }
    return sweep_group_size(ctx);
}

extern "C" int vo_lookahead_flush(vo_ctx* ctx)
{
    if (!ctx) return VO_E_ARG;
    if (sweep_group_members(ctx) > 0) {
        VO_HIP(ctx, hipSetDevice(ctx->device));
        if (int rc = sweep_group_close(ctx, VO_GRP_FLUSH)) return rc;
    }
    return sweep_group_size(ctx);
}

extern "C" int vo_sweep_group_stats(vo_ctx* ctx, int64_t* closed4, int* open_members)
{
    if (!ctx || !closed4) return vo_fail(ctx, VO_E_ARG, "vo_sweep_group_stats: bad argument");
    for (int i = 0; i < 4; i++) closed4[i] = ctx->grp_closed[i];
    if (open_members) *open_members = sweep_group_members(ctx);
    return VO_OK;
}

extern "C" int vo_device_name(const vo_ctx* ctx, char* buf, int buflen)
{
    if (!ctx || !buf || buflen <= 0) return VO_E_ARG;
    snprintf(buf, buflen, "%s", ctx->devname);
    return VO_OK;
}

extern "C" int vo_synchronize(vo_ctx* ctx)
{
    if (!ctx) return VO_E_ARG;
    if (int rc = sweep_group_close(ctx, VO_GRP_CONSUMER)) return rc;
    for (int k = 0; k < vo_ctx::MAX_ENGINES; k++)
        if (ctx->la_stream[k]) VO_HIP(ctx, hipStreamSynchronize(ctx->la_stream[k]));
    for (int kind : { vo_ctx::ALT_POSE, vo_ctx::ALT_MONO })
        for (int k = 0; k < vo_ctx::alt_count(kind); k++)
            if (ctx->alt(kind, k).stream) VO_HIP(ctx, hipStreamSynchronize(ctx->alt(kind, k).stream));
    VO_HIP(ctx, hipStreamSynchronize(ctx->stream));
    return VO_OK;
}

extern "C" int vo_set_rectify_maps(vo_ctx* ctx, int cam, const int16_t* map1, const uint16_t* map2, int w, int h)
{
    if (!ctx || cam < 0 || cam > 1 || !map1 || !map2) return vo_fail(ctx, VO_E_ARG, "vo_set_rectify_maps: bad argument");
    if (w > ctx->max_w || h > ctx->max_h || w <= 0 || h <= 0) return vo_fail(ctx, VO_E_CAP, "maps %dx%d exceed context %dx%d", w, h, ctx->max_w, ctx->max_h);
    VO_HIP(ctx, hipSetDevice(ctx->device));
    VO_HIP(ctx, hipMemcpyAsync(ctx->map1[cam], map1, (size_t)w * h * 4, hipMemcpyHostToDevice, ctx->stream));
    VO_HIP(ctx, hipMemcpyAsync(ctx->map2[cam], map2, (size_t)w * h * 2, hipMemcpyHostToDevice, ctx->stream));
    VO_HIP(ctx, hipStreamSynchronize(ctx->stream));
    ctx->map_w = w; ctx->map_h = h; ctx->has_map[cam] = true;
    return VO_OK;
}

extern "C" int vo_set_sgbm(vo_ctx* ctx, int minDisparity, int numDisparities, int blockSize, int P1, int P2,
                           int disp12MaxDiff, int preFilterCap, int uniquenessRatio, int speckleWindowSize,
                           int speckleRange, int mode)
{
    if (!ctx) return VO_E_ARG;
    if (numDisparities <= 0 || numDisparities % 16) return vo_fail(ctx, VO_E_ARG, "numDisparities must be a positive multiple of 16");
    if (numDisparities > ctx->max_disp) return vo_fail(ctx, VO_E_CAP, "numDisparities %d > max_disp %d", numDisparities, ctx->max_disp);
    if (mode != 0 && mode != 1) return vo_fail(ctx, VO_E_ARG, "mode must be 0 (MODE_SGBM) or 1 (MODE_HH)");
    if (int rc = sweep_group_close(ctx, VO_GRP_OTHER)) return rc;
    SgbmEff& e = ctx->sg;
    e.minD = minDisparity; e.D = numDisparities; e.maxD = minDisparity + numDisparities;
    e.ur = uniquenessRatio >= 0 ? uniquenessRatio : 10;
    e.d12 = disp12MaxDiff > 0 ? disp12MaxDiff : 1;
    e.P1 = P1 > 0 ? P1 : 2;
    int p2 = P2 > 0 ? P2 : 5;
    e.P2 = p2 > e.P1 + 1 ? p2 : e.P1 + 1;
    int bs = blockSize > 0 ? blockSize : 5;
    e.SW2 = e.SH2 = bs / 2;
    e.ftzero = (preFilterCap > 15 ? preFilterCap : 15) | 1;
    e.speckleWindow = speckleWindowSize; e.speckleRange = speckleRange; e.mode = mode;
    if (e.SW2 > 5) return vo_fail(ctx, VO_E_ARG, "blockSize > 11 is not supported");
    if (e.P2 > 8000 || e.ftzero > 127) return vo_fail(ctx, VO_E_ARG, "P2 > 8000 or preFilterCap > 127 would overflow int16 costs");
    {
        const int side = 2 * e.SW2 + 1, cmax = side * side * (2 * e.ftzero + 63);
        if (cmax + e.P2 > 32767)
            return vo_fail(ctx, VO_E_ARG, "blockSize %d with preFilterCap %d and P2 %d lets a path cost reach %d: beyond the int16 OpenCV computes in",
                           side, e.ftzero, e.P2, cmax + e.P2);
    }
    e.set = true;
    return VO_OK;
}

static void sparse_void_ahead(vo_ctx* ctx)
{
    for (int s = 0; s < VO_NUM_SLOTS; s++) { ctx->slots[s].sp_pending = false; ctx->slots[s].sp_ahead = false; }
}

extern "C" int vo_set_Q(vo_ctx* ctx, const double* Q16)
{
    if (!ctx || !Q16) return VO_E_ARG;
    memcpy(ctx->Q, Q16, sizeof(ctx->Q));
    ctx->has_Q = true;
    sparse_void_ahead(ctx);
    return VO_OK;
}

extern "C" int vo_set_roi(vo_ctx* ctx, int x0, int y0, int x1, int y1)
{
    if (!ctx) return VO_E_ARG;
    if (x0 < 0 || y0 < 0) return vo_fail(ctx, VO_E_ARG, "negative ROI origin is not supported");
    if (int rc = sweep_group_close(ctx, VO_GRP_OTHER)) return rc;
    ctx->roi[0] = x0; ctx->roi[1] = y0; ctx->roi[2] = x1; ctx->roi[3] = y1;
    ctx->has_roi = true;
    sparse_void_ahead(ctx);
    return VO_OK;
}

__global__ void k_bgr2gray(const uint8_t* __restrict__ bgr, int n, uint8_t* __restrict__ gray)
{
    int i = blockIdx.x * blockDim.x + threadIdx.x;
    if (i >= n) return;
    int b = bgr[3 * (size_t)i], g = bgr[3 * (size_t)i + 1], r = bgr[3 * (size_t)i + 2];
    gray[i] = (uint8_t)((b * 3735 + g * 19235 + r * 9798 + (1 << 14)) >> 15);
}

__global__ void k_remap(const uint8_t* __restrict__ src, int sw, int sh, const int16_t* __restrict__ map1,
                        const uint16_t* __restrict__ map2, int w, int h, uint8_t* __restrict__ dst)
{
    int x = blockIdx.x * blockDim.x + threadIdx.x, y = blockIdx.y;
    if (x >= w) return;
    size_t i = (size_t)y * w + x;
    int sx = map1[2 * i], sy = map1[2 * i + 1];
    int f = map2[i] & 1023, fx = f & 31, fy = f >> 5;
    int w00 = (32 - fx) * (32 - fy) * 32, w01 = fx * (32 - fy) * 32, w10 = (32 - fx) * fy * 32, w11 = fx * fy * 32;
    int p00 = 0, p01 = 0, p10 = 0, p11 = 0;
    bool x0ok = (unsigned)sx < (unsigned)sw, x1ok = (unsigned)(sx + 1) < (unsigned)sw;
    if ((unsigned)sy < (unsigned)sh) {
        if (x0ok) p00 = src[(size_t)sy * sw + sx];
        if (x1ok) p01 = src[(size_t)sy * sw + sx + 1];
    }
    if ((unsigned)(sy + 1) < (unsigned)sh) {
        if (x0ok) p10 = src[(size_t)(sy + 1) * sw + sx];
        if (x1ok) p11 = src[(size_t)(sy + 1) * sw + sx + 1];
    }
    int v = (p00 * w00 + p01 * w01 + p10 * w10 + p11 * w11 + (1 << 14)) >> 15;
    dst[i] = (uint8_t)min(v, 255);
}

static int check_slot(vo_ctx* ctx, int slot)
{
    if (!ctx) return VO_E_ARG;
    if (slot < 0 || slot >= VO_NUM_SLOTS) return vo_fail(ctx, VO_E_ARG, "slot %d out of range [0,%d)", slot, VO_NUM_SLOTS);
    return VO_OK;
}

typedef uint32_t ingest_u32x4 __attribute__((ext_vector_type(4)));
__global__ void __launch_bounds__(256) k_ingest_copy(const uint8_t* __restrict__ src, uint8_t* __restrict__ dst, size_t bytes)
{
    const size_t n16 = bytes / 16, stride = (size_t)gridDim.x * blockDim.x, i0 = (size_t)blockIdx.x * blockDim.x + threadIdx.x;
    for (size_t i = i0; i < n16; i += stride)
        ((ingest_u32x4*)dst)[i] = __builtin_nontemporal_load((const ingest_u32x4*)src + i);
    for (size_t i = n16 * 16 + i0; i < bytes; i += stride) dst[i] = src[i];
}

static int ingest_bytes(vo_ctx* ctx, uint8_t* dst, const uint8_t* src, size_t bytes, hipMemcpyKind kind, bool by_kernel)
{
    if (by_kernel && ((uintptr_t)src % 16 == 0) && ((uintptr_t)dst % 16 == 0)) {
        const int blocks = (int)((bytes / 16 + 255) / 256 < 2048 ? (bytes / 16 + 255) / 256 : 2048);
        hipLaunchKernelGGL(k_ingest_copy, dim3(blocks < 1 ? 1 : blocks), dim3(256), 0, ctx->stream, src, dst, bytes);
        return VO_OK;
    }
    VO_HIP(ctx, hipMemcpyAsync(dst, src, bytes, kind, ctx->stream));
    return VO_OK;
}

static int ingest(vo_ctx* ctx, int cam, const uint8_t* host, int w, int h, int channels, int preprocessed, uint8_t* dst,
                  uint8_t* stage, hipMemcpyKind kind = hipMemcpyHostToDevice, bool by_kernel = false)
{
    const size_t n = (size_t)w * h;
    const bool need_remap = !preprocessed;
    if (need_remap && (!ctx->has_map[cam] || ctx->map_w != w || ctx->map_h != h))
        return vo_fail(ctx, VO_E_STATE, "rectification maps for camera %d not set for %dx%d", cam, w, h);
    uint8_t* gray = need_remap ? stage + n * 3 : dst;
    if (channels == 3) {
        if (int rcb = ingest_bytes(ctx, stage, host, n * 3, kind, by_kernel)) return rcb;
        hipLaunchKernelGGL(k_bgr2gray, dim3(div_up((int)n, 256)), dim3(256), 0, ctx->stream, stage, (int)n, gray);
    } else {
        if (int rcb = ingest_bytes(ctx, gray, host, n, kind, by_kernel)) return rcb;
    }
    if (need_remap)
        hipLaunchKernelGGL(k_remap, dim3(div_up(w, 256), h), dim3(256), 0, ctx->stream, gray, w, h, ctx->map1[cam],
                           ctx->map2[cam], w, h, dst);
    VO_CHECK_LAUNCH(ctx);
    return VO_OK;
}

extern "C" int vo_upload_pair(vo_ctx* ctx, int slot, const uint8_t* left, const uint8_t* right, int w, int h,
                              int channels, int preprocessed)
{
    int rc = check_slot(ctx, slot);
    if (rc) return rc;
    if (!left || !right || (channels != 1 && channels != 3)) return vo_fail(ctx, VO_E_ARG, "vo_upload_pair: bad argument");
    if (w > ctx->max_w || h > ctx->max_h || w < 16 || h < 16) return vo_fail(ctx, VO_E_CAP, "image %dx%d exceeds context %dx%d", w, h, ctx->max_w, ctx->max_h);
    VO_HIP(ctx, hipSetDevice(ctx->device));
    FrameSlot& f = ctx->slots[slot];
    if ((rc = slot_wait(ctx, f)) || (rc = slot_before_overwrite(ctx, f))) return rc;
    StageTimer t(ctx, VO_T_UPLOAD);
    rc = ingest(ctx, 0, left, w, h, channels, preprocessed, f.left, ctx->stage_in);
    if (rc) return rc;
    rc = ingest(ctx, 1, right, w, h, channels, preprocessed, f.right, ctx->stage_in);
    if (rc) return rc;
    f.w = w; f.h = h; f.has_pair = true; f.has_disp = false; f.has_kp = false; f.kp_depth = false; f.sp_pending = false; f.n_kp = 0; f.kp_pending = false;
    return VO_OK;
}

extern "C" int vo_upload_mono(vo_ctx* ctx, int slot, const uint8_t* img, int w, int h, int channels)
{
    int rc = check_slot(ctx, slot);
    if (rc) return rc;
    if (!img || (channels != 1 && channels != 3)) return vo_fail(ctx, VO_E_ARG, "vo_upload_mono: bad argument");
    if (w > ctx->max_w || h > ctx->max_h || w < 16 || h < 16) return vo_fail(ctx, VO_E_CAP, "image %dx%d exceeds context %dx%d", w, h, ctx->max_w, ctx->max_h);
    VO_HIP(ctx, hipSetDevice(ctx->device));
    FrameSlot& f = ctx->slots[slot];
    if ((rc = slot_wait(ctx, f)) || (rc = slot_before_overwrite(ctx, f))) return rc;
    StageTimer t(ctx, VO_T_UPLOAD);
    if ((rc = ingest(ctx, 0, img, w, h, channels, 1, f.left, ctx->stage_in))) return rc;
    f.w = w; f.h = h; f.has_pair = true; f.has_disp = false; f.has_kp = false; f.kp_depth = false; f.sp_pending = false; f.n_kp = 0; f.kp_pending = false;
    return VO_OK;
}

extern "C" int vo_stage_pairs_alloc(vo_ctx* ctx, int n, int w, int h, int channels)
{
    if (!ctx || n <= 0 || (channels != 1 && channels != 3)) return vo_fail(ctx, VO_E_ARG, "vo_stage_pairs_alloc: bad argument");
    if (w > ctx->max_w || h > ctx->max_h || w < 16 || h < 16) return vo_fail(ctx, VO_E_CAP, "image %dx%d exceeds context", w, h);
    VO_HIP(ctx, hipSetDevice(ctx->device));
    if (ctx->staged) { (void)hipFree(ctx->staged); ctx->staged = nullptr; }
    ctx->staged_n = 0;
    const size_t per = (size_t)w * h * channels;
    VO_HIP(ctx, hipMalloc((void**)&ctx->staged, per * 2 * n));
    ctx->staged_n = n; ctx->staged_w = w; ctx->staged_h = h; ctx->staged_ch = channels;
    return VO_OK;
}

extern "C" int vo_stage_pair(vo_ctx* ctx, int index, const uint8_t* left, const uint8_t* right)
{
    if (!ctx || !left || !right || index < 0 || index >= ctx->staged_n) return vo_fail(ctx, VO_E_ARG, "vo_stage_pair: bad index");
    VO_HIP(ctx, hipSetDevice(ctx->device));
    const size_t per = (size_t)ctx->staged_w * ctx->staged_h * ctx->staged_ch;
    VO_HIP(ctx, hipMemcpyAsync(ctx->staged + per * 2 * index, left, per, hipMemcpyHostToDevice, ctx->stream));
    VO_HIP(ctx, hipMemcpyAsync(ctx->staged + per * (2 * index + 1), right, per, hipMemcpyHostToDevice, ctx->stream));
    VO_HIP(ctx, hipStreamSynchronize(ctx->stream));
    return VO_OK;
}

extern "C" int vo_load_staged_pair(vo_ctx* ctx, int slot, int index, int preprocessed)
{
    int rc = check_slot(ctx, slot);
    if (rc) return rc;
    if (index < 0 || index >= ctx->staged_n) return vo_fail(ctx, VO_E_ARG, "vo_load_staged_pair: bad index");
    VO_HIP(ctx, hipSetDevice(ctx->device));
    FrameSlot& f = ctx->slots[slot];
    const int w = ctx->staged_w, h = ctx->staged_h;
    const size_t per = (size_t)w * h * ctx->staged_ch;
    StageTimer t(ctx, VO_T_UPLOAD);
    if ((rc = slot_wait(ctx, f)) || (rc = slot_before_overwrite(ctx, f))) return rc;
    rc = ingest(ctx, 0, ctx->staged + per * 2 * index, w, h, ctx->staged_ch, preprocessed, f.left, ctx->stage_in, hipMemcpyDeviceToDevice);
    if (rc) return rc;
    rc = ingest(ctx, 1, ctx->staged + per * (2 * index + 1), w, h, ctx->staged_ch, preprocessed, f.right, ctx->stage_in, hipMemcpyDeviceToDevice);
    if (rc) return rc;
    f.w = w; f.h = h; f.has_pair = true; f.has_disp = false; f.has_kp = false; f.kp_depth = false; f.sp_pending = false; f.n_kp = 0; f.kp_pending = false;
    return VO_OK;
}

struct EngineScope {
    vo_ctx* ctx;
    int engine;
    hipStream_t stream0;
    EngineScope(vo_ctx* c, int e) : ctx(c), engine(e), stream0(c->stream)
    {
        ctx->stream = ctx->la_stream[engine];
        std::swap(ctx->stage_in, ctx->la_stage[engine]);
        ctx->ws = engine == 0 ? &ctx->main_ws : &ctx->ws_alt[engine];
        ctx->orbws = &ctx->ws_alt[engine].orb;
        ctx->cur_engine = engine;
    }
    ~EngineScope()
    {
        ctx->cur_engine = -1;
        ctx->ws = &ctx->main_ws;
        ctx->orbws = &ctx->main_ws.orb;
        std::swap(ctx->stage_in, ctx->la_stage[engine]);
        ctx->stream = stream0;
    }
    EngineScope(const EngineScope&) = delete;
    EngineScope& operator=(const EngineScope&) = delete;
};

static int engine_prepare(vo_ctx* ctx, int engine, bool want_sgbm)
{
    if (!ctx->la_stream[engine]) VO_HIP(ctx, hipStreamCreateWithFlags(&ctx->la_stream[engine], hipStreamNonBlocking));
    if (!ctx->ws_alt[engine].mid) {
        VO_HIP(ctx, hipEventCreateWithFlags(&ctx->ws_alt[engine].mid, hipEventDisableTiming));
        VO_HIP(ctx, hipEventCreateWithFlags(&ctx->ws_alt[engine].swept, hipEventDisableTiming));
    }
    if (!ctx->la_stage[engine]) {
        VO_HIP(ctx, hipMalloc((void**)&ctx->la_stage[engine], ctx->stage_bytes * 2 + 256));
        if (orb_ws_alloc(ctx, ctx->ws_alt[engine].orb)) return vo_fail(ctx, VO_E_HIP, "hipMalloc failed (look-ahead ORB workspace)");
    }
    if (!want_sgbm || engine == 0 || ctx->ws_alt[engine].ready) return VO_OK;
    const hipError_t e = sgbm_ws_alloc(ctx, ctx->ws_alt[engine]);
    if (e != hipSuccess) return vo_fail(ctx, VO_E_HIP, "look-ahead engine %d: workspace allocation failed: %s", engine, hipGetErrorString(e));
    return VO_OK;
}

int slot_wait(vo_ctx* ctx, FrameSlot& f)
{
    if (int rc = sweep_group_close_for(ctx, f)) return rc;
    if (f.pending) {
        VO_HIP(ctx, hipStreamWaitEvent(ctx->stream, f.ready, 0));
        f.pending = false;
        if (f.counted && ctx->inflight > 0) ctx->inflight--;
        f.counted = false;
    }
    return VO_OK;
}

extern "C" int vo_lookahead_drop(vo_ctx* ctx, int slot)
{
    if (!ctx || slot < 0 || slot >= VO_NUM_SLOTS) return vo_fail(ctx, VO_E_ARG, "vo_lookahead_drop: bad slot");
    FrameSlot& f = ctx->slots[slot];
    if (int rc = sweep_group_close_for(ctx, f)) return rc;
    if (f.pending && f.counted && ctx->inflight > 0) ctx->inflight--;
    f.counted = false;
    return VO_OK;
}

int slot_before_overwrite(vo_ctx* ctx, FrameSlot& f)
{
    if (int rc = sweep_group_close_for(ctx, f)) return rc;
    if (f.pending) VO_HIP(ctx, hipStreamWaitEvent(ctx->stream, f.ready, 0));
    for (hipEvent_t& r : f.readers)
        if (r) { VO_HIP(ctx, hipStreamWaitEvent(ctx->stream, r, 0)); r = nullptr; }
    if (f.depth_writer) { VO_HIP(ctx, hipStreamWaitEvent(ctx->stream, f.depth_writer, 0)); f.depth_writer = nullptr; }
    f.mono_serial = 0;
    return VO_OK;
}

void slot_add_reader(FrameSlot& f, hipEvent_t done)
{
    for (hipEvent_t r : f.readers) if (r == done) return;
    for (hipEvent_t& r : f.readers)
        if (!r || hipEventQuery(r) == hipSuccess) { r = done; return; }
    (void)hipEventSynchronize(f.readers[0]);
    f.readers[0] = f.readers[1];
    f.readers[1] = done;
}

static int prefetch_pair(vo_ctx* ctx, int slot, const uint8_t* srcL, const uint8_t* srcR, bool from_host, int w, int h,
                         int channels, int preprocessed, vo_ctx::HostStage* hs = nullptr, const SparseReq* sp = nullptr)
{
    int rc;
    FrameSlot& f = ctx->slots[slot];
    const int engine = ctx->next_engine;
    if ((rc = engine_prepare(ctx, engine, sp == nullptr))) return rc;
    if (sp && (rc = sparse_ws_prepare(ctx, ctx->sp_alt[engine], ctx->la_stream[engine], true))) return rc;
    if ((f.in_group || sweep_group_has_engine(ctx, engine)) && (rc = sweep_group_close(ctx, f.in_group ? VO_GRP_CONSUMER : VO_GRP_OTHER))) return rc;
    bool deferred = false;
    const size_t per = (size_t)w * h * channels;
    hipMemcpyKind kind = hipMemcpyDeviceToDevice;
    if (hs) {
        kind = hipMemcpyHostToDevice;
    } else if (from_host) {
        vo_ctx::SgbmWs& a = ctx->ws_alt[engine];
        if (!a.pinned) {
            VO_HIP(ctx, hipHostMalloc((void**)&a.pinned, ctx->stage_bytes * 2, hipHostMallocDefault));
            VO_HIP(ctx, hipEventCreateWithFlags(&a.h2d_done, hipEventDisableTiming));
        }
        if (a.h2d_valid) VO_HIP(ctx, hipEventSynchronize(a.h2d_done));
        memcpy(a.pinned, srcL, per);
        memcpy(a.pinned + per, srcR, per);
        srcL = a.pinned; srcR = a.pinned + per;
        kind = hipMemcpyHostToDevice;
    }
    ctx->next_engine = (engine + 1) % ctx->n_engines;
    f.w = w; f.h = h; f.has_kp = false; f.kp_depth = false; f.sp_pending = false; f.sp_ahead = false; f.n_kp = 0; f.kp_pending = false;
    if (sp) { f.mono_serial = 0; f.kp_params[0] = f.kp_params[1] = f.kp_params[2] = f.kp_params[3] = -1; }
    {
        EngineScope on_engine(ctx, engine);
        rc = engine_behind_chain(ctx, engine);
        const int stagger = ctx->tune_stagger >= 0 ? ctx->tune_stagger : (7 * ctx->n_engines + 8) / 16;
        if (!sp && stagger > 0 && stagger < ctx->n_engines) {
            vo_ctx::SgbmWs& p = ctx->ws_alt[(engine - stagger + ctx->n_engines) % ctx->n_engines];
            if (p.mid_valid) (void)hipStreamWaitEvent(ctx->stream, p.mid, 0);
        }
        if (!rc) rc = slot_before_overwrite(ctx, f);
        const bool in_place = !sp && kind == hipMemcpyDeviceToDevice && preprocessed && channels == 1;
        if (!rc && !in_place) {
            StageTimer t(ctx, VO_T_UPLOAD);
            const bool pinned_src = hs != nullptr || from_host;
            rc = ingest(ctx, 0, srcL, w, h, channels, preprocessed, f.left, ctx->stage_in, kind, pinned_src);
            if (!rc) rc = ingest(ctx, 1, srcR, w, h, channels, preprocessed, f.right, ctx->stage_in, kind, pinned_src);
        }
        if (!rc && hs) {
            std::lock_guard<std::mutex> lk(ctx->stage_mu);
            if (hipEventRecord(hs->h2d_done, ctx->stream) == hipSuccess) hs->valid = true;
            else rc = vo_fail(ctx, VO_E_HIP, "hipEventRecord failed");
        } else if (!rc && from_host) {
            vo_ctx::SgbmWs& a = ctx->ws_alt[engine];
            if (hipEventRecord(a.h2d_done, ctx->stream) == hipSuccess) a.h2d_valid = true;
            else rc = vo_fail(ctx, VO_E_HIP, "hipEventRecord failed");
        }
#ifdef VO_TEST_HOOKS
        if (!rc && ctx->fault_prefetch > 0 && --ctx->fault_prefetch == 0)
            rc = vo_fail(ctx, VO_E_STATE, "injected failure (VO_FAULT_PREFETCH) inside the engine scope");
#endif
        if (!rc && sp) rc = sparse_enqueue(ctx, f, ctx->sp_alt[engine], *sp);
        else if (!rc) rc = in_place ? sgbm_run(ctx, f, w, h, srcL, srcR, &deferred) : sgbm_run(ctx, f, w, h, nullptr, nullptr, &deferred);
        if (!rc && !sp && !deferred && ctx->la_orb) {
            const int* q = ctx->la_orb_params;
            rc = orb_slot_enqueue(ctx, f, q[0], q[1], q[2], q[3]);
            if (!rc) { memcpy(f.kp_params, q, sizeof(f.kp_params)); f.kp_pending = true; }
        }
        if (!rc && !deferred && hipEventRecord(f.ready, ctx->stream) != hipSuccess) rc = vo_fail(ctx, VO_E_HIP, "hipEventRecord failed");
    }
    if (rc) {
        f.kp_pending = false; f.has_pair = false; f.has_disp = false;
        if (f.counted && ctx->inflight > 0) ctx->inflight--;
        f.counted = false;
        return rc;
    }
    f.has_pair = true; f.has_disp = sp == nullptr;
    if (sp) { f.sp_req = *sp; f.sp_pending = true; }
    if (!f.counted) ctx->inflight++;
    f.pending = true; f.counted = true;
    if (deferred && sweep_group_members(ctx) >= sweep_group_size(ctx)) return sweep_group_close(ctx, VO_GRP_FULL);
    return VO_OK;
}

extern "C" int vo_prefetch_staged_pair(vo_ctx* ctx, int slot, int index, int preprocessed)
{
    int rc = check_slot(ctx, slot);
    if (rc) return rc;
    if (index < 0 || index >= ctx->staged_n) return vo_fail(ctx, VO_E_ARG, "vo_prefetch_staged_pair: bad index");
    if (!ctx->sg.set) return vo_fail(ctx, VO_E_STATE, "vo_set_sgbm has not been called");
    VO_HIP(ctx, hipSetDevice(ctx->device));
    const size_t per = (size_t)ctx->staged_w * ctx->staged_h * ctx->staged_ch;
    return prefetch_pair(ctx, slot, ctx->staged + per * 2 * index, ctx->staged + per * (2 * index + 1), false, ctx->staged_w,
                         ctx->staged_h, ctx->staged_ch, preprocessed);
}

static int host_stage_wait(vo_ctx* ctx, int buf);
static int sparse_entry_check(vo_ctx* ctx, const SparseReq& q, const char* who)
{
    if (int rc = sparse_req_check(ctx, q, who)) return rc;
    if (!ctx->has_Q) return vo_fail(ctx, VO_E_STATE, "vo_set_Q has not been called");
    return VO_OK;
}

extern "C" int vo_prefetch_staged_pair_sparse(vo_ctx* ctx, int slot, int index, int preprocessed, int nfeatures, float min_disp, float max_disp,
                                              float row_tol, int max_hamming)
{
    int rc = check_slot(ctx, slot);
    if (rc) return rc;
    if (index < 0 || index >= ctx->staged_n) return vo_fail(ctx, VO_E_ARG, "vo_prefetch_staged_pair_sparse: bad index");
    const SparseReq q = { nfeatures, min_disp, max_disp, row_tol, max_hamming, ctx->sp_assoc_flags, ctx->sp_assoc_ratio };
    if ((rc = sparse_entry_check(ctx, q, "vo_prefetch_staged_pair_sparse"))) return rc;
    VO_HIP(ctx, hipSetDevice(ctx->device));
    const size_t per = (size_t)ctx->staged_w * ctx->staged_h * ctx->staged_ch;
    return prefetch_pair(ctx, slot, ctx->staged + per * 2 * index, ctx->staged + per * (2 * index + 1), false, ctx->staged_w,
                         ctx->staged_h, ctx->staged_ch, preprocessed, nullptr, &q);
}

extern "C" int vo_prefetch_pair_sparse(vo_ctx* ctx, int slot, const uint8_t* left, const uint8_t* right, int w, int h, int channels,
                                       int preprocessed, int nfeatures, float min_disp, float max_disp, float row_tol, int max_hamming)
{
    int rc = check_slot(ctx, slot);
    if (rc) return rc;
    if (!left || !right || (channels != 1 && channels != 3)) return vo_fail(ctx, VO_E_ARG, "vo_prefetch_pair_sparse: bad argument");
    if (w > ctx->max_w || h > ctx->max_h || w < 16 || h < 16) return vo_fail(ctx, VO_E_CAP, "image %dx%d exceeds context %dx%d", w, h, ctx->max_w, ctx->max_h);
    const SparseReq q = { nfeatures, min_disp, max_disp, row_tol, max_hamming, ctx->sp_assoc_flags, ctx->sp_assoc_ratio };
    if ((rc = sparse_entry_check(ctx, q, "vo_prefetch_pair_sparse"))) return rc;
    VO_HIP(ctx, hipSetDevice(ctx->device));
    return prefetch_pair(ctx, slot, left, right, true, w, h, channels, preprocessed, nullptr, &q);
}

extern "C" int vo_prefetch_host_staged_sparse(vo_ctx* ctx, int slot, int buf, int w, int h, int channels, int preprocessed, int nfeatures,
                                              float min_disp, float max_disp, float row_tol, int max_hamming)
{
    int rc = check_slot(ctx, slot);
    if (rc) return rc;
    if (buf < 0 || buf >= vo_ctx::N_HOST_STAGE || (channels != 1 && channels != 3)) return vo_fail(ctx, VO_E_ARG, "vo_prefetch_host_staged_sparse: bad argument");
    if (w > ctx->max_w || h > ctx->max_h || w < 16 || h < 16) return vo_fail(ctx, VO_E_CAP, "image %dx%d exceeds context %dx%d", w, h, ctx->max_w, ctx->max_h);
    const SparseReq q = { nfeatures, min_disp, max_disp, row_tol, max_hamming, ctx->sp_assoc_flags, ctx->sp_assoc_ratio };
    if ((rc = sparse_entry_check(ctx, q, "vo_prefetch_host_staged_sparse"))) return rc;
    vo_ctx::HostStage& hs = ctx->host_stage[buf];
    if (!hs.pinned) return vo_fail(ctx, VO_E_STATE, "staging buffer %d has not been filled (vo_host_stage_pair / vo_host_stage_begin)", buf);
    if ((rc = host_stage_wait(ctx, buf))) return vo_fail(ctx, rc, "the copy into staging buffer %d failed", buf);
    VO_HIP(ctx, hipSetDevice(ctx->device));
    const size_t per = (size_t)w * h * channels;
    return prefetch_pair(ctx, slot, hs.pinned, hs.pinned + per, true, w, h, channels, preprocessed, &hs, &q);
}

extern "C" int vo_prefetch_staged_mono(vo_ctx* ctx, int slot, int index, int nfeatures)
{
    int rc = check_slot(ctx, slot);
    if (rc) return rc;
    if (index < 0 || index >= ctx->staged_n) return vo_fail(ctx, VO_E_ARG, "vo_prefetch_staged_mono: bad index");
    if (nfeatures < 0 || nfeatures > ctx->max_kp) return vo_fail(ctx, VO_E_CAP, "nfeatures %d exceeds max_kp %d", nfeatures, ctx->max_kp);
    VO_HIP(ctx, hipSetDevice(ctx->device));
    FrameSlot& f = ctx->slots[slot];
    const int span = ctx->n_engines < 4 ? ctx->n_engines : 4;
    const int engine = ctx->mono_engine % span;
    if ((rc = engine_prepare(ctx, engine, true))) return rc;
    if ((f.in_group || sweep_group_has_engine(ctx, engine)) && (rc = sweep_group_close(ctx, f.in_group ? VO_GRP_CONSUMER : VO_GRP_OTHER))) return rc;
    ctx->mono_engine = (engine + 1) % span;
    const size_t per = (size_t)ctx->staged_w * ctx->staged_h * ctx->staged_ch;
    const int w = ctx->staged_w, h = ctx->staged_h;
    f.w = w; f.h = h; f.has_kp = false; f.kp_depth = false; f.sp_pending = false; f.n_kp = 0; f.kp_pending = false; f.has_disp = false;
    {
        EngineScope on_engine(ctx, engine);
        rc = engine_behind_chain(ctx, engine);
        if (!rc) rc = slot_before_overwrite(ctx, f);
        if (!rc) {
            StageTimer t(ctx, VO_T_UPLOAD);
            rc = ingest(ctx, 0, ctx->staged + per * 2 * index, w, h, ctx->staged_ch, 1, f.left, ctx->stage_in, hipMemcpyDeviceToDevice);
        }
        const int params[4] = { nfeatures, 0, 0, 0 };
        if (!rc) rc = orb_slot_enqueue(ctx, f, nfeatures, 0, 0, 0);
        if (!rc) { memcpy(f.kp_params, params, sizeof(f.kp_params)); f.kp_pending = true; }
        if (!rc && hipEventRecord(f.ready, ctx->stream) != hipSuccess) rc = vo_fail(ctx, VO_E_HIP, "hipEventRecord failed");
    }
    if (rc) {
        f.kp_pending = false; f.has_pair = false;
        if (f.counted && ctx->inflight > 0) ctx->inflight--;
        f.counted = false;
        return rc;
    }
    f.has_pair = true;
    if (!f.counted) ctx->inflight++;
    f.pending = true; f.counted = true;
    return VO_OK;
}

extern "C" int vo_prefetch_pair(vo_ctx* ctx, int slot, const uint8_t* left, const uint8_t* right, int w, int h, int channels,
                                int preprocessed)
{
    int rc = check_slot(ctx, slot);
    if (rc) return rc;
    if (!left || !right || (channels != 1 && channels != 3)) return vo_fail(ctx, VO_E_ARG, "vo_prefetch_pair: bad argument");
    if (w > ctx->max_w || h > ctx->max_h || w < 16 || h < 16) return vo_fail(ctx, VO_E_CAP, "image %dx%d exceeds context %dx%d", w, h, ctx->max_w, ctx->max_h);
    if (!ctx->sg.set) return vo_fail(ctx, VO_E_STATE, "vo_set_sgbm has not been called");
    VO_HIP(ctx, hipSetDevice(ctx->device));
    return prefetch_pair(ctx, slot, left, right, true, w, h, channels, preprocessed);
}

static int host_stage_alloc(vo_ctx* ctx)
{
    std::lock_guard<std::mutex> lk(ctx->stage_mu);
    for (vo_ctx::HostStage& q : ctx->host_stage) {
        if (q.pinned) continue;
        if (hipHostMalloc((void**)&q.pinned, ctx->stage_bytes * 2, hipHostMallocDefault) != hipSuccess) return VO_E_HIP;
        if (hipEventCreateWithFlags(&q.h2d_done, hipEventDisableTiming) != hipSuccess) return VO_E_HIP;
    }
    return VO_OK;
}

static void host_stage_loop(vo_ctx* ctx)
{
    (void)hipSetDevice(ctx->device);
    for (;;) {
        vo_ctx::StageJob job;
        hipEvent_t wait_for = nullptr;
        {
            std::unique_lock<std::mutex> lk(ctx->stage_mu);
            ctx->stage_cv.wait(lk, [&] { return ctx->stage_stop || !ctx->stage_jobs.empty(); });
            if (ctx->stage_stop) return;
            job = ctx->stage_jobs.front();
            ctx->stage_jobs.pop_front();
            vo_ctx::HostStage& hs = ctx->host_stage[job.buf];
            if (hs.valid) wait_for = hs.h2d_done;
        }
        int rc = VO_OK;
        if (wait_for && hipEventSynchronize(wait_for) != hipSuccess) rc = VO_E_HIP;
        if (!rc) {
            vo_ctx::HostStage& hs = ctx->host_stage[job.buf];
            memcpy(hs.pinned, job.left, job.per);
            memcpy(hs.pinned + job.per, job.right, job.per);
        }
        {
            std::lock_guard<std::mutex> lk(ctx->stage_mu);
            ctx->host_stage[job.buf].state = rc;
        }
        ctx->stage_cv.notify_all();
    }
}

static int host_stage_wait(vo_ctx* ctx, int buf)
{
    std::unique_lock<std::mutex> lk(ctx->stage_mu);
    vo_ctx::HostStage& hs = ctx->host_stage[buf];
    ctx->stage_cv.wait(lk, [&] { return hs.state != 1; });
    const int rc = hs.state;
    hs.state = 0;
    return rc;
}

extern "C" int vo_host_stage_begin(vo_ctx* ctx, int buf, const uint8_t* left, const uint8_t* right, int w, int h, int channels)
{
    if (!ctx || buf < 0 || buf >= vo_ctx::N_HOST_STAGE || !left || !right || (channels != 1 && channels != 3))
        return vo_fail(ctx, VO_E_ARG, "vo_host_stage_begin: bad argument");
    if (w > ctx->max_w || h > ctx->max_h || w < 16 || h < 16) return vo_fail(ctx, VO_E_CAP, "image %dx%d exceeds context %dx%d", w, h, ctx->max_w, ctx->max_h);
    VO_HIP(ctx, hipSetDevice(ctx->device));
    if (host_stage_alloc(ctx)) return vo_fail(ctx, VO_E_HIP, "pinned staging memory: allocation failed");
    {
        std::lock_guard<std::mutex> lk(ctx->stage_mu);
        vo_ctx::HostStage& hs = ctx->host_stage[buf];
        if (hs.state == 1) return vo_fail(ctx, VO_E_STATE, "vo_host_stage_begin: a copy into buffer %d is still pending", buf);
        hs.state = 1;
        ctx->stage_jobs.push_back({ buf, left, right, (size_t)w * h * channels });
        if (!ctx->stage_thread.joinable()) ctx->stage_thread = std::thread(host_stage_loop, ctx);
    }
    ctx->stage_cv.notify_all();
    return VO_OK;
}

extern "C" int vo_host_stage_wait(vo_ctx* ctx, int buf)
{
    if (!ctx || buf < 0 || buf >= vo_ctx::N_HOST_STAGE) return vo_fail(ctx, VO_E_ARG, "vo_host_stage_wait: bad argument");
    const int rc = host_stage_wait(ctx, buf);
    return rc ? vo_fail(ctx, rc, "the copy into staging buffer %d failed", buf) : VO_OK;
}

extern "C" int vo_host_stage_pair(vo_ctx* ctx, int buf, const uint8_t* left, const uint8_t* right, int w, int h, int channels)
{
    if (!ctx || buf < 0 || buf >= vo_ctx::N_HOST_STAGE || !left || !right || (channels != 1 && channels != 3)) return VO_E_ARG;
    if (w > ctx->max_w || h > ctx->max_h || w < 16 || h < 16) return VO_E_CAP;
    if (hipSetDevice(ctx->device) != hipSuccess) return VO_E_HIP;
    if (host_stage_alloc(ctx)) return VO_E_HIP;
    if (int rcw = host_stage_wait(ctx, buf)) return rcw;
    vo_ctx::HostStage& hs = ctx->host_stage[buf];
    hipEvent_t wait_for = nullptr;
    { std::lock_guard<std::mutex> lk(ctx->stage_mu); if (hs.valid) wait_for = hs.h2d_done; }
    if (wait_for && hipEventSynchronize(wait_for) != hipSuccess) return VO_E_HIP;
    const size_t per = (size_t)w * h * channels;
    memcpy(hs.pinned, left, per);
    memcpy(hs.pinned + per, right, per);
    return VO_OK;
}

extern "C" int vo_host_stage_fetch(vo_ctx* ctx, int buf, uint8_t* left, uint8_t* right, int w, int h, int channels)
{
    if (!ctx || buf < 0 || buf >= vo_ctx::N_HOST_STAGE || !left || !right || (channels != 1 && channels != 3)) return VO_E_ARG;
    vo_ctx::HostStage& hs = ctx->host_stage[buf];
    if (!hs.pinned || (size_t)w * h * channels > ctx->stage_bytes) return VO_E_STATE;
    if (int rcw = host_stage_wait(ctx, buf)) return rcw;
    const size_t per = (size_t)w * h * channels;
    memcpy(left, hs.pinned, per);
    memcpy(right, hs.pinned + per, per);
    return VO_OK;
}

extern "C" int vo_prefetch_host_staged(vo_ctx* ctx, int slot, int buf, int w, int h, int channels, int preprocessed)
{
    int rc = check_slot(ctx, slot);
    if (rc) return rc;
    if (buf < 0 || buf >= vo_ctx::N_HOST_STAGE || (channels != 1 && channels != 3)) return vo_fail(ctx, VO_E_ARG, "vo_prefetch_host_staged: bad argument");
    if (w > ctx->max_w || h > ctx->max_h || w < 16 || h < 16) return vo_fail(ctx, VO_E_CAP, "image %dx%d exceeds context %dx%d", w, h, ctx->max_w, ctx->max_h);
    if (!ctx->sg.set) return vo_fail(ctx, VO_E_STATE, "vo_set_sgbm has not been called");
    vo_ctx::HostStage& hs = ctx->host_stage[buf];
    if (!hs.pinned) return vo_fail(ctx, VO_E_STATE, "staging buffer %d has not been filled (vo_host_stage_pair / vo_host_stage_begin)", buf);
    if ((rc = host_stage_wait(ctx, buf))) return vo_fail(ctx, rc, "the copy into staging buffer %d failed", buf);
    VO_HIP(ctx, hipSetDevice(ctx->device));
    const size_t per = (size_t)w * h * channels;
    return prefetch_pair(ctx, slot, hs.pinned, hs.pinned + per, true, w, h, channels, preprocessed, &hs);
// ... 57 lines not shown
    hipLaunchKernelGGL(k_bgr2gray, dim3(div_up((int)n, 256)), dim3(256), 0, ctx->stream, ctx->stage_in, (int)n, ctx->stage_in + n * 3);
    VO_CHECK_LAUNCH(ctx);
    VO_HIP(ctx, hipMemcpyAsync(gray, ctx->stage_in + n * 3, n, hipMemcpyDeviceToHost, ctx->stream));
    VO_HIP(ctx, hipStreamSynchronize(ctx->stream));
    return VO_OK;
}

extern "C" int vo_remap(vo_ctx* ctx, int cam, const uint8_t* src, int w, int h, uint8_t* dst)
{
    if (!ctx || !src || !dst || cam < 0 || cam > 1) return vo_fail(ctx, VO_E_ARG, "vo_remap: bad argument");
    if (!ctx->has_map[cam]) return vo_fail(ctx, VO_E_STATE, "maps of camera %d not set", cam);
    if ((size_t)w * h > (size_t)ctx->max_w * ctx->max_h) return vo_fail(ctx, VO_E_CAP, "image too large");
    VO_HIP(ctx, hipSetDevice(ctx->device));
    const size_t n = (size_t)w * h, nm = (size_t)ctx->map_w * ctx->map_h;
    VO_HIP(ctx, hipMemcpyAsync(ctx->stage_in, src, n, hipMemcpyHostToDevice, ctx->stream));
    uint8_t* out = ctx->stage_in + ctx->stage_bytes;
    hipLaunchKernelGGL(k_remap, dim3(div_up(ctx->map_w, 256), ctx->map_h), dim3(256), 0, ctx->stream, ctx->stage_in, w, h,
                       ctx->map1[cam], ctx->map2[cam], ctx->map_w, ctx->map_h, out);
    VO_CHECK_LAUNCH(ctx);
    VO_HIP(ctx, hipMemcpyAsync(dst, out, nm, hipMemcpyDeviceToHost, ctx->stream));
    VO_HIP(ctx, hipStreamSynchronize(ctx->stream));
    return VO_OK;
}

__global__ void k_disp_to_f32(const int16_t* __restrict__ d, int n, float* __restrict__ out)
{
    int i = blockIdx.x * blockDim.x + threadIdx.x;
    if (i < n) out[i] = (float)d[i] / 16.0f;
}

static int ensure_img3(vo_ctx* ctx, size_t bytes)
{
    if (ctx->img3_ws_bytes >= bytes) return VO_OK;
    if (ctx->img3_ws) (void)hipFree(ctx->img3_ws);
    ctx->img3_ws = nullptr; ctx->img3_ws_bytes = 0;
    VO_HIP(ctx, hipMalloc((void**)&ctx->img3_ws, bytes));
    ctx->img3_ws_bytes = bytes;
    return VO_OK;
}

extern "C" int vo_download_disparity_f32(vo_ctx* ctx, int slot, float* out)
{
    int rc = check_slot(ctx, slot);
    if (rc) return rc;
    FrameSlot& f = ctx->slots[slot];
    if (!f.has_disp || !out) return vo_fail(ctx, VO_E_STATE, "slot %d holds no disparity", slot);
    VO_HIP(ctx, hipSetDevice(ctx->device));
    if ((rc = slot_wait(ctx, f))) return rc;
    const int n = f.w * f.h;
    if ((rc = ensure_img3(ctx, (size_t)n * 12))) return rc;
    hipLaunchKernelGGL(k_disp_to_f32, dim3(div_up(n, 256)), dim3(256), 0, ctx->stream, f.disp16, n, ctx->img3_ws);
    VO_CHECK_LAUNCH(ctx);
    VO_HIP(ctx, hipMemcpyAsync(out, ctx->img3_ws, (size_t)n * 4, hipMemcpyDeviceToHost, ctx->stream));
    VO_HIP(ctx, hipStreamSynchronize(ctx->stream));
    return slot_health(ctx, f, slot);
}

extern "C" int vo_download_left(vo_ctx* ctx, int slot, uint8_t* out)
{
    int rc = check_slot(ctx, slot);
    if (rc) return rc;
    FrameSlot& f = ctx->slots[slot];
    if (!f.has_pair || !out) return vo_fail(ctx, VO_E_STATE, "slot %d holds no image", slot);
    VO_HIP(ctx, hipSetDevice(ctx->device));
    if ((rc = slot_wait(ctx, f))) return rc;
    VO_HIP(ctx, hipMemcpyAsync(out, f.left, (size_t)f.w * f.h, hipMemcpyDeviceToHost, ctx->stream));
    VO_HIP(ctx, hipStreamSynchronize(ctx->stream));
    return VO_OK;
}

extern "C" int vo_download_right(vo_ctx* ctx, int slot, uint8_t* out)
{
    int rc = check_slot(ctx, slot);
    if (rc) return rc;
    FrameSlot& f = ctx->slots[slot];
    if (!f.has_pair || !out) return vo_fail(ctx, VO_E_STATE, "slot %d holds no image", slot);
    VO_HIP(ctx, hipSetDevice(ctx->device));
    if ((rc = slot_wait(ctx, f))) return rc;
    VO_HIP(ctx, hipMemcpyAsync(out, f.right, (size_t)f.w * f.h, hipMemcpyDeviceToHost, ctx->stream));
    VO_HIP(ctx, hipStreamSynchronize(ctx->stream));
    return VO_OK;
}

extern "C" int vo_slot_num_keypoints(vo_ctx* ctx, int slot, int* n_out)
{
    int rc = check_slot(ctx, slot);
    if (rc) return rc;
    if (!n_out) return VO_E_ARG;
    *n_out = ctx->slots[slot].has_kp ? ctx->slots[slot].n_kp : 0;
    return VO_OK;
}

extern "C" int vo_enable_timing(vo_ctx* ctx, int on)
{
    if (!ctx) return VO_E_ARG;
    ctx->timing = on != 0;
    ctx->timing_mask = on == 1 ? ~0u : (unsigned)on >> 1;
    return VO_OK;
}

static void resolve_events(vo_ctx* ctx)
{
    if (ctx->ev_used == 0) return;
    (void)hipStreamSynchronize(ctx->stream);
    for (size_t i = 0; i < ctx->ev_used; i++) {
        float ms = 0;
        if (hipEventElapsedTime(&ms, ctx->ev_pool[2 * i], ctx->ev_pool[2 * i + 1]) == hipSuccess) {
            ctx->t_ms[ctx->ev_stage[i]] += ms;
            ctx->t_n[ctx->ev_stage[i]] += ctx->ev_entries[i];
        }
    }
    ctx->ev_used = 0;
}

StageTimer::StageTimer(vo_ctx* ctx, int s, int entries) : c(ctx), stage(s), idx(-1)
{
    if (!c->timing || !((c->timing_mask >> s) & 1u) || entries <= 0) return;
    if (c->ev_used * 2 + 2 > c->ev_pool.size()) {
        if (c->ev_pool.size() >= 32768) resolve_events(c);
        else
            for (int k = 0; k < 512; k++) { hipEvent_t e; if (hipEventCreate(&e) == hipSuccess) c->ev_pool.push_back(e); }
    }
    if (c->ev_used * 2 + 2 > c->ev_pool.size()) return;
    idx = (long)c->ev_used++;
    if (c->ev_stage.size() <= (size_t)idx) { c->ev_stage.resize(idx + 1); c->ev_entries.resize(idx + 1); }
    c->ev_stage[idx] = s;
    c->ev_entries[idx] = entries;
    (void)hipEventRecord(c->ev_pool[2 * idx], c->stream);
}
StageTimer::~StageTimer()
{
    if (idx >= 0) (void)hipEventRecord(c->ev_pool[2 * idx + 1], c->stream);
}

extern "C" int vo_get_timings(vo_ctx* ctx, double* ms_out, int64_t* launches_out, int reset)
{
    if (!ctx) return VO_E_ARG;
    resolve_events(ctx);
    for (int i = 0; i < VO_T_NSTAGES; i++) {
        if (ms_out) ms_out[i] = ctx->t_ms[i];
        if (launches_out) launches_out[i] = ctx->t_n[i];
        if (reset) { ctx->t_ms[i] = 0; ctx->t_n[i] = 0; }
    }
    return VO_OK;
}

extern "C" int vo_get_stage_timeline(vo_ctx* ctx, int cap, int32_t* stage_out, int32_t* entries_out, double* begin_ms_out, double* end_ms_out, int* n_out)
{
    if (!ctx || !n_out || cap < 0 || (cap > 0 && (!stage_out || !entries_out || !begin_ms_out || !end_ms_out)))
        return vo_fail(ctx, VO_E_ARG, "vo_get_stage_timeline: bad argument");
    *n_out = 0;
    if (ctx->ev_used == 0) return VO_OK;
    VO_HIP(ctx, hipSetDevice(ctx->device));
    for (int k = 0; k < vo_ctx::MAX_ENGINES; k++)
        if (ctx->la_stream[k]) VO_HIP(ctx, hipStreamSynchronize(ctx->la_stream[k]));
    for (int kind : { vo_ctx::ALT_POSE, vo_ctx::ALT_MONO })
        for (int k = 0; k < vo_ctx::alt_count(kind); k++)
            if (ctx->alt(kind, k).stream) VO_HIP(ctx, hipStreamSynchronize(ctx->alt(kind, k).stream));
    VO_HIP(ctx, hipStreamSynchronize(ctx->stream));
    int n = 0;
    for (size_t i = 0; i < ctx->ev_used; i++) {
        float t0 = 0, dt = 0;
        if (hipEventElapsedTime(&t0, ctx->ev_pool[0], ctx->ev_pool[2 * i]) != hipSuccess ||
            hipEventElapsedTime(&dt, ctx->ev_pool[2 * i], ctx->ev_pool[2 * i + 1]) != hipSuccess) {
            (void)hipGetLastError();
            continue;
        }
        if (n < cap) { stage_out[n] = ctx->ev_stage[i]; entries_out[n] = ctx->ev_entries[i]; begin_ms_out[n] = t0; end_ms_out[n] = (double)t0 + (double)dt; }
        n++;
    }
    *n_out = n;
    return VO_OK;
}

int slot_health(vo_ctx* ctx, const FrameSlot& f, int slot)
{
    if (f.disp_gen != 0 && f.sweep_word && *(volatile int32_t*)f.sweep_word == f.disp_gen)
        return vo_fail(ctx, VO_E_SWEEP, "slot %d: a strip hand-off of this pair's aggregation sweep gave up waiting (GPU oversubscribed?): "
                                        "its disparity is undefined and nothing computed from it is handed out; submit the pair again", slot);
    return VO_OK;
}

extern "C" int vo_sgbm_sweep_status(vo_ctx* ctx, int* error_out)
{
    if (!ctx || !error_out) return VO_E_ARG;
    VO_HIP(ctx, hipSetDevice(ctx->device));
    int rc = vo_synchronize(ctx);
    if (rc) return rc;
    int n = 0;
    VO_HIP(ctx, hipMemcpy(&n, ctx->d_sweep_errs, sizeof(int), hipMemcpyDeviceToHost));
    *error_out = n;
    return VO_OK;
}

typedef uint32_t copy_u32x4 __attribute__((ext_vector_type(4)));
template <bool NT>
__global__ void __launch_bounds__(256) k_copy_stream(const copy_u32x4* __restrict__ src, copy_u32x4* __restrict__ dst, size_t n16)
{
    const size_t stride = (size_t)gridDim.x * blockDim.x;
    for (size_t i = (size_t)blockIdx.x * blockDim.x + threadIdx.x; i < n16; i += stride) {
        if (NT) __builtin_nontemporal_store(__builtin_nontemporal_load(src + i), dst + i);
        else dst[i] = src[i];
    }
}

extern "C" int vo_measure_copy(vo_ctx* ctx, int64_t bytes, int reps, int nontemporal, double* gb_per_s)
{
    if (!ctx || !gb_per_s || reps <= 0) return vo_fail(ctx, VO_E_ARG, "vo_measure_copy: bad argument");
    const int64_t cap = (int64_t)ctx->vol_cells * 2;
    if (bytes <= 0 || bytes > cap) bytes = cap;
    bytes &= ~(int64_t)4095;
    if (bytes <= 0 || !ctx->ws->C || !ctx->ws->S) return vo_fail(ctx, VO_E_STATE, "vo_measure_copy: no volumes to copy between");
    VO_HIP(ctx, hipSetDevice(ctx->device));
    for (int k = 0; k < vo_ctx::MAX_ENGINES; k++)
        if (ctx->la_stream[k]) VO_HIP(ctx, hipStreamSynchronize(ctx->la_stream[k]));
    VO_HIP(ctx, hipStreamSynchronize(ctx->stream));
    hipEvent_t e0, e1;
    VO_HIP(ctx, hipEventCreate(&e0));
    VO_HIP(ctx, hipEventCreate(&e1));
    const size_t n16 = (size_t)bytes / 16;
    const int blocks = 256 * 16;
    auto kern = nontemporal ? k_copy_stream<true> : k_copy_stream<false>;
    auto launch = [&]() { hipLaunchKernelGGL(kern, dim3(blocks), dim3(256), 0, ctx->stream, (const copy_u32x4*)ctx->ws->S, (copy_u32x4*)ctx->ws->C, n16); };
    launch();
    VO_HIP(ctx, hipEventRecord(e0, ctx->stream));
    for (int r = 0; r < reps; r++) launch();
    VO_HIP(ctx, hipEventRecord(e1, ctx->stream));
    VO_HIP(ctx, hipEventSynchronize(e1));
    float ms = 0.f;
    VO_HIP(ctx, hipEventElapsedTime(&ms, e0, e1));
    (void)hipEventDestroy(e0);
    (void)hipEventDestroy(e1);
    *gb_per_s = ms > 0.f ? 2.0 * (double)bytes * reps / (ms * 1e-3) / 1e9 : 0.0;
    return VO_OK;
}

__global__ void k_clock_probe(unsigned long long* out, unsigned long long ticks)
{
    const unsigned long long c0 = __builtin_amdgcn_s_memtime(), w0 = __builtin_amdgcn_s_memrealtime();
    unsigned long long w = w0;
    unsigned v = threadIdx.x;
    while (w - w0 < ticks) {
#pragma unroll
        for (int i = 0; i < 64; i++) asm volatile("v_pk_add_i16 %0, %0, %0" : "+v"(v));
        w = __builtin_amdgcn_s_memrealtime();
    }
    const unsigned long long c1 = __builtin_amdgcn_s_memtime();
    if (threadIdx.x == 0) { out[0] = c1 - c0; out[1] = w - w0; out[2] = v; }
}

extern "C" int vo_shader_clock(vo_ctx* ctx, int micros, double* mhz)
{
    if (!ctx || !mhz || micros <= 0 || micros > 1000000) return vo_fail(ctx, VO_E_ARG, "vo_shader_clock: bad argument");
    VO_HIP(ctx, hipSetDevice(ctx->device));
    unsigned long long* d = (unsigned long long*)ctx->red;
    hipLaunchKernelGGL(k_clock_probe, dim3(1), dim3(64), 0, ctx->stream, d, (unsigned long long)micros * 100ull);
    VO_CHECK_LAUNCH(ctx);
    unsigned long long h[2] = { 0, 0 };
    VO_HIP(ctx, hipStreamSynchronize(ctx->stream));
    VO_HIP(ctx, hipMemcpy(h, d, 16, hipMemcpyDeviceToHost));
    *mhz = h[1] ? (double)h[0] / ((double)h[1] / 100.0) : 0.0;
    return VO_OK;
}

extern "C" int vo_sgbm_sweep_stats(vo_ctx* ctx, int block, int32_t* out, int n_words)
{
    if (!ctx || !out || block < 0 || block > 1 || n_words <= 0) return vo_fail(ctx, VO_E_ARG, "vo_sgbm_sweep_stats: bad argument");
    VO_HIP(ctx, hipSetDevice(ctx->device));
    int rc = vo_synchronize(ctx);
    if (rc) return rc;
    const int half = ctx->sw_ctl_words / 2;
    if (n_words > half) n_words = half;
    VO_HIP(ctx, hipMemcpy(out, ctx->ws->sw_ctl + block * half, (size_t)n_words * sizeof(int32_t), hipMemcpyDeviceToHost));
    return VO_OK;
}

extern "C" int vo_lookahead_depth(vo_ctx* ctx, int* depth_out)
{
    if (!ctx || !depth_out) return VO_E_ARG;
    *depth_out = ctx->inflight;
    return VO_OK;
}

extern "C" int vo_slot_ready(vo_ctx* ctx, int slot, int* ready_out)
{
    if (!ctx || slot < 0 || slot >= VO_NUM_SLOTS || !ready_out) return vo_fail(ctx, VO_E_ARG, "vo_slot_ready: bad argument");
    FrameSlot& f = ctx->slots[slot];
    *ready_out = 1;
    if (int rc = sweep_group_close_for(ctx, f)) return rc;
    if (f.pending) {
        const hipError_t e = hipEventQuery(f.ready);
        if (e == hipErrorNotReady) *ready_out = 0;
        else if (e != hipSuccess) return vo_fail(ctx, VO_E_HIP, "hipEventQuery failed: %s", hipGetErrorString(e));
    }
    return VO_OK;
}

extern "C" int vo_sgbm_last_schedule(vo_ctx* ctx, int* schedule_out)
{
    if (!ctx || !schedule_out) return VO_E_ARG;
    *schedule_out = ctx->last_schedule;
    return VO_OK;
}

extern "C" int vo_sgbm_last_geometry(vo_ctx* ctx, int64_t* cells, int* n_paths)
{
    if (!ctx) return VO_E_ARG;
    if (cells) *cells = ctx->last_cells;
    if (n_paths) *n_paths = ctx->last_paths;
    return VO_OK;
}

#ifdef VO_TEST_HOOKS
extern "C" int vo_test_plant_keypoints(vo_ctx* ctx, int slot, int n, const float* xy, const uint8_t* desc, const float* xyz, const uint8_t* rdesc)
{
    if (!ctx || slot < 0 || slot >= VO_NUM_SLOTS || n < 0) return vo_fail(ctx, VO_E_ARG, "vo_test_plant_keypoints: bad argument");
    if (n > ctx->kp_cap) return vo_fail(ctx, VO_E_CAP, "vo_test_plant_keypoints: %d keypoints exceed capacity %d", n, ctx->kp_cap);
    if (n > 0 && (!xy || !desc || !xyz)) return vo_fail(ctx, VO_E_ARG, "vo_test_plant_keypoints: null pointer");
    FrameSlot& f = ctx->slots[slot];
    VO_HIP(ctx, hipSetDevice(ctx->device));
    int rc;
    if ((rc = slot_wait(ctx, f)) || (rc = slot_before_overwrite(ctx, f))) return rc;
    f.has_kp = false; f.kp_depth = false; f.kp_pending = false; f.sp_pending = false; f.sp_ahead = false;
    f.mono_serial = 0;
    f.kp_params[0] = f.kp_params[1] = f.kp_params[2] = f.kp_params[3] = -1;
    f.sp_req.nfeatures = -1;
    if ((rc = xfer_h2d(ctx, f.kp_xy, xy, (size_t)n * 8))) return rc;
    if ((rc = xfer_h2d(ctx, f.desc, desc, (size_t)n * 32))) return rc;
    if ((rc = xfer_h2d(ctx, f.kp_xyz, xyz, (size_t)n * 12))) return rc;
    if (rdesc) { if ((rc = xfer_h2d(ctx, f.kp_rdesc, rdesc, (size_t)n * 32))) return rc; }
    else if (n > 0) VO_HIP(ctx, hipMemsetAsync(f.kp_rdesc, 0, (size_t)n * 32, ctx->stream));
    if (n > 0) {
        VO_HIP(ctx, hipMemsetAsync(f.kp_size, 0, (size_t)n * 4, ctx->stream));
        VO_HIP(ctx, hipMemsetAsync(f.kp_angle, 0, (size_t)n * 4, ctx->stream));
        VO_HIP(ctx, hipMemsetAsync(f.kp_resp, 0, (size_t)n * 4, ctx->stream));
        VO_HIP(ctx, hipMemsetAsync(f.kp_oct, 0, (size_t)n * 4, ctx->stream));
        VO_HIP(ctx, hipMemsetAsync(f.kp_disp, 0, (size_t)n * 4, ctx->stream));
    }
    if ((rc = xfer_flush(ctx))) return rc;
    f.sp_rec[0] = f.sp_rec[1] = f.sp_rec[2] = f.sp_rec[3] = n;
    *f.n_kp_host = n;
    f.n_kp = n;
    f.has_kp = true; f.kp_depth = true;
    return VO_OK;
}

extern "C" int vo_test_plant_map(vo_ctx* ctx, int map, int n, const float* xyz, const uint8_t* desc, const uint8_t* rdesc, const int32_t* octave,
                                 const int32_t* obs, const int32_t* last)
{
    if (!ctx || map < 0 || map >= VO_NUM_MAPS || !ctx->maps[map].used || n < 0) return vo_fail(ctx, VO_E_ARG, "vo_test_plant_map: bad argument");
    LandmarkMap& m = ctx->maps[map];
    if (n > m.capacity) return vo_fail(ctx, VO_E_CAP, "vo_test_plant_map: %d landmarks exceed capacity %d", n, m.capacity);
    if (n > 0 && (!xyz || !desc || !rdesc || !octave || !obs || !last)) return vo_fail(ctx, VO_E_ARG, "vo_test_plant_map: null pointer");
    int top = -1;
    for (int i = 0; i < n; i++) {
        if (last[i] < 0 || obs[i] < 1) return vo_fail(ctx, VO_E_ARG, "vo_test_plant_map: need last >= 0 and obs >= 1");
        if (last[i] > top) top = last[i];
    }
    VO_HIP(ctx, hipSetDevice(ctx->device));
    const MapSet& s = m.set[m.cur];
    int rc;
    if ((rc = xfer_h2d(ctx, s.xyz, xyz, (size_t)n * 12)) || (rc = xfer_h2d(ctx, s.desc, desc, (size_t)n * 32)) ||
        (rc = xfer_h2d(ctx, s.rdesc, rdesc, (size_t)n * 32)) || (rc = xfer_h2d(ctx, s.oct, octave, (size_t)n * 4)) ||
        (rc = xfer_h2d(ctx, s.obs, obs, (size_t)n * 4)) || (rc = xfer_h2d(ctx, s.last, last, (size_t)n * 4)) || (rc = xfer_flush(ctx)))
        return rc;
    m.n = n; m.view_n = 0; m.max_serial = top;
    return VO_OK;
}
// ... 2 lines not shown
```

openvo_amd/csrc/vo_internal.h:

```cpp
#pragma once
#include <hip/hip_runtime.h>
#include <stdint.h>
#include <stdio.h>
#include <string.h>
#include <string>
#include <vector>
#include <deque>
#include <thread>
#include <mutex>
#include <condition_variable>
#include "../../include/vo355.h"

#define VO_ORB_LEVELS 8
#define VO_ORB_EDGE 31
#define VO_ORB_HALF_PATCH 15

struct SgbmEff {
    int minD, maxD, D, ur, d12, P1, P2, SW2, SH2, ftzero, minX1, maxX1, W1, invalid16;
    int speckleWindow, speckleRange, mode;
    bool set;
};

struct OrbLevel {
    int w, h;
    size_t off;
    float scale;
    int quota;
};

struct FrameSlot {
    uint8_t* left = nullptr;
    uint8_t* right = nullptr;
    int16_t* disp16 = nullptr;
    float* kp_xy = nullptr;
    float* kp_size = nullptr;
    float* kp_angle = nullptr;
    float* kp_resp = nullptr;
    int32_t* kp_oct = nullptr;
    uint8_t* desc = nullptr;
    int n_kp = 0;
    int w = 0, h = 0;
    bool has_pair = false, has_disp = false, has_kp = false;
    hipEvent_t ready = nullptr;
    bool pending = false;
    bool counted = false;
    hipEvent_t readers[2] = {nullptr, nullptr};
    double* mono_depth = nullptr;
    uint32_t* mono_serial_dev = nullptr;
    uint32_t mono_serial = 0;
    hipEvent_t depth_writer = nullptr;
    int32_t* n_kp_host = nullptr;
    bool kp_pending = false;
    int32_t* sweep_word = nullptr;
    int32_t disp_gen = 0;
    int kp_params[4] = {0, 0, 0, 0};
    float* kp_xyz = nullptr;
    float* kp_disp = nullptr;
    bool kp_depth = false;
    uint8_t* kp_rdesc = nullptr;
    int32_t* sp_rec = nullptr;
    bool sp_pending = false;
    bool sp_ahead = false;
    struct SparseReq { int nfeatures; float min_disp, max_disp, row_tol; int max_hamming; int assoc_flags; float assoc_ratio; } sp_req = {-1, 0.f, 0.f, 0.f, 0, 0, 0.f};
    bool in_group = false;
};

struct OrbWs {
    uint8_t *pyr_img = nullptr, *pyr_mask = nullptr;
    int32_t *cand_pos = nullptr, *candA_pos = nullptr, *candB_pos = nullptr, *counters = nullptr;
    float *cand_resp = nullptr, *candA_resp = nullptr, *candB_resp = nullptr;
    hipEvent_t done = nullptr;
    bool done_valid = false;
};

struct SparseWs {
    FrameSlot *l = nullptr, *r = nullptr;
    OrbWs orb_r;
    int32_t* match = nullptr;
    float *disp = nullptr, *xyz = nullptr;
    int32_t* ticket = nullptr;
    uint32_t* claim = nullptr;
    FrameSlot* own = nullptr;
    int32_t* own_words = nullptr;
    bool ready = false, orb_ready = false;
};
typedef FrameSlot::SparseReq SparseReq;

struct MapSet {
    float* xyz = nullptr;
    uint8_t *desc = nullptr, *rdesc = nullptr;
    int32_t *oct = nullptr, *obs = nullptr, *last = nullptr;
};
struct LandmarkMap {
    bool used = false;
    int capacity = 0, n = 0, cur = 0, view_n = 0;
    int max_serial = -1;
    MapSet set[2];
    int32_t *view_src = nullptr, *d_q = nullptr, *d_t = nullptr;
    uint8_t *claimed = nullptr, *d_mask = nullptr;
    std::vector<uint8_t> seen;
};
void map_free(LandmarkMap& m);

struct vo_ctx {
    int device = 0;
    hipStream_t stream = nullptr;
    static const int MAX_ENGINES = 24;
    hipStream_t la_stream[MAX_ENGINES] = {};
    int cur_engine = -1;
    int tune_stagger = -1;
    uint8_t* la_stage[MAX_ENGINES] = {};
    struct SgbmWs {
        uint32_t *planesL = nullptr, *planesR = nullptr;
        int16_t *C = nullptr, *S = nullptr, *disp_tmp = nullptr;
        int32_t *ccl_runlen = nullptr, *ccl_label = nullptr, *ccl_size = nullptr;
        int32_t* rec = nullptr;
        int S_vols = 0;
        uint64_t* sw_bnd = nullptr;
        size_t sw_bnd_bytes = 0;
        int* sw_ctl = nullptr;
        uint32_t sw_tag = 0;
        hipEvent_t done = nullptr;
        bool done_valid = false;
        bool done_on_engine0 = false;
        bool ready = false;
        OrbWs orb;
        uint8_t* pinned = nullptr;
        hipEvent_t h2d_done = nullptr;
        bool h2d_valid = false;
        hipEvent_t mid = nullptr;
        bool mid_valid = false;
        hipEvent_t swept = nullptr;
        hipEvent_t chain = nullptr;
    } ws_alt[MAX_ENGINES];
    SgbmWs main_ws;
    SgbmWs* ws = &main_ws;
    OrbWs* orbws = &main_ws.orb;
    bool la_orb = false;
    int la_orb_params[4] = {0, 0, 0, 0};
    int32_t* slot_words = nullptr;
    int32_t sweep_gen_next = 0;
    int* d_sweep_errs = nullptr;
    int tune_spin_limit = 1 << 22;
    int fault_sweep = 0;
    int engines_fit = 24;
    int n_engines = 16;
    int next_engine = 0;
    int hw_queues = 4;
    int sweep_group_req = 0;
    struct SweepGroup* grp = nullptr;
    int64_t grp_closed[4] = {0, 0, 0, 0};
    int max_w = 0, max_h = 0, max_disp = 0, max_kp = 0, kp_cap = 0;
    std::string err;
    char devname[256] = {0};

    SgbmEff sg{};
    double Q[16];
    bool has_Q = false;
    int roi[4] = {0, 0, 0, 0};
    bool has_roi = false;

    int16_t* map1[2] = {nullptr, nullptr};
    uint16_t* map2[2] = {nullptr, nullptr};
    int map_w = 0, map_h = 0;
    bool has_map[2] = {false, false};

    FrameSlot slots[VO_NUM_SLOTS + 1];
    FrameSlot sparse_r;
    LandmarkMap maps[VO_NUM_MAPS];
    SparseWs sp_main;
    SparseWs sp_alt[MAX_ENGINES];

    uint8_t* stage_in = nullptr;
    size_t stage_bytes = 0;

    size_t vol_cells = 0;
    int16_t* dump = nullptr;
    int sw_ctl_words = 0;
    int tune_diag_wgs = 0;
    int tune_diag_dbg = 0;
    int tune_diag_nwc = 0;
    int64_t last_cells = 0;
    int last_paths = 0;
    int last_schedule = 0;

    OrbLevel lv[VO_ORB_LEVELS];
    int orb_w = 0, orb_h = 0;
    size_t pyr_bytes = 0;
    int32_t* rs_ofs = nullptr;
    uint16_t* rs_coef = nullptr;
    int32_t* pyr_rects = nullptr;
    int pyr_nbx = 0, pyr_nby = 0, pyr_buf[2] = {0, 0}, pyr_tab = 0;
    char rs_meta_host[1024];
    int orb_quota_nfeatures = -1;
    int cand_cap = 0;
    uint8_t* host_mask_dev = nullptr;

    struct MatchWs {
        int32_t *m_idx = nullptr, *m_count = nullptr, *m_dist = nullptr, *mq_idx = nullptr, *mt_idx = nullptr;
        float *pts_a = nullptr, *pts_b = nullptr, *xy_a = nullptr, *xy_b = nullptr;
        uint8_t *st_a = nullptr, *st_b = nullptr, *clique_ws = nullptr;
        size_t clique_ws_bytes = 0;
        uint8_t* ransac_ws = nullptr;
        size_t ransac_ws_bytes = 0;
    };
    MatchWs main_mw;
    MatchWs* mw = &main_mw;
    bool has_win = false;
    float win_rx = 0.f, win_ry = 0.f;
    bool has_loop = false;
    int loop_max = 0;
    int sp_assoc_flags = 0;
    float sp_assoc_ratio = 0.f;
    uint8_t* mq = nullptr;
    uint8_t* mt = nullptr;
    double* red = nullptr;
    struct AsyncAlt {
        hipStream_t stream = nullptr;
        hipEvent_t done = nullptr;
        uint8_t* result = nullptr;
        bool ready = false, busy = false;
        MatchWs mw;
    };
    enum { ALT_POSE = 0, ALT_MONO = 1 };
    static const int N_POSE_ALT = VO_NUM_POSE_ASYNC;
    static const int N_POSE_STREAMS = 3;
    int n_pose_streams = N_POSE_STREAMS;
    hipStream_t pose_streams[N_POSE_STREAMS] = {};
    struct PoseAlt : AsyncAlt {
        int slot_a = -1, slot_b = -1;
        int32_t gen_a = 0, gen_b = 0;
        bool pnp = false, want = false;
        int nq = 0;
    } pose_alt[N_POSE_ALT];
    static const int N_MONO_ALT = VO_NUM_MONO_ASYNC;
    struct MonoAlt : AsyncAlt {
        bool want = false;
        bool pose = false;
        int nq = 0, nb = 0, min_n = 0;
    } mono_alt[N_MONO_ALT];
    int alt_next[2] = {0, 0};
    uint32_t mono_serial_next = 0;
    AsyncAlt& alt(int kind, int k) { return kind == ALT_POSE ? static_cast<AsyncAlt&>(pose_alt[k]) : mono_alt[k]; }
    static int alt_count(int kind) { return kind == ALT_POSE ? N_POSE_ALT : N_MONO_ALT; }
    std::vector<const void*> big_lds;
    float* img3_ws = nullptr;
    size_t img3_ws_bytes = 0;
    void* pinned = nullptr;
    size_t pinned_bytes = 0;
    size_t arena_off = 0;
    struct PendingCopy { void* dst; const void* src; size_t bytes; };
    std::vector<PendingCopy> pending;

    static const int N_HOST_STAGE = VO_NUM_HOST_STAGE;
    struct HostStage { uint8_t* pinned = nullptr; hipEvent_t h2d_done = nullptr; bool valid = false; int state = 0; } host_stage[VO_NUM_HOST_STAGE];
    struct StageJob { int buf; const uint8_t *left, *right; size_t per; };
    std::thread stage_thread;
    std::mutex stage_mu;
    std::condition_variable stage_cv;
    std::deque<StageJob> stage_jobs;
    bool stage_stop = false;

    uint8_t* staged = nullptr;
    int staged_n = 0, staged_w = 0, staged_h = 0, staged_ch = 1;

    int tune_sweep_ty = 30;
    int mono_engine = 0;
    int inflight = 0;
    int fault_pnp_range = 0;
    int fault_prefetch = 0;

    bool timing = false;
    unsigned timing_mask = ~0u;
    std::vector<hipEvent_t> ev_pool;
    std::vector<int> ev_stage;
    std::vector<int> ev_entries;
    size_t ev_used = 0;
    hipEvent_t ev0 = nullptr, ev1 = nullptr;
    double t_ms[VO_T_NSTAGES] = {0};
    int64_t t_n[VO_T_NSTAGES] = {0};
};

int vo_fail(vo_ctx* ctx, int code, const char* fmt, ...);
#define VO_HIP(ctx, call)                                                               \
    do {                                                                                \
        hipError_t e__ = (call);                                                        \
        if (e__ != hipSuccess)                                                          \
            return vo_fail(ctx, VO_E_HIP, "%s failed: %s (%s:%d)", #call,              \
                           hipGetErrorString(e__), __FILE__, __LINE__);                 \
    } while (0)

#define VO_CHECK_LAUNCH(ctx) VO_HIP(ctx, hipGetLastError())

struct StageTimer {
    vo_ctx* c;
    int stage;
    long idx;
    StageTimer(vo_ctx* ctx, int s, int entries = 1);
    ~StageTimer();
};

static inline int div_up(int a, int b) { return (a + b - 1) / b; }

int xfer_h2d(vo_ctx* ctx, void* dev_dst, const void* host_src, size_t bytes);
int xfer_d2h(vo_ctx* ctx, void* host_dst, const void* dev_src, size_t bytes);
int xfer_flush(vo_ctx* ctx);

int slot_wait(vo_ctx* ctx, FrameSlot& f);
int slot_before_overwrite(vo_ctx* ctx, FrameSlot& f);
void slot_add_reader(FrameSlot& f, hipEvent_t done);
int orb_slot_enqueue(vo_ctx* ctx, FrameSlot& f, int nfeatures, int mask_mode, int min_disp16, int max_disp16);
int orb_slots_enqueue(vo_ctx* ctx, FrameSlot* const* f, OrbWs* const* ws, int n, int nfeatures, int mask_mode, int min_disp16, int max_disp16);
struct OrbIn {
    FrameSlot* fs; OrbWs* ws;
    const uint8_t* img; const int16_t* disp16; const uint8_t* mask;
    int img_stride, disp_stride, mask_stride;
};
int orb_enqueue_jobs(vo_ctx* ctx, const OrbIn* in, int n, int w, int h, int nfeatures, int mask_mode, int min_d16, int max_d16);
int orb_enqueue(vo_ctx* ctx, FrameSlot* fs, const uint8_t* d_img, int img_stride, int w, int h, int nfeatures, int mask_mode,
                const int16_t* d_disp16, int disp_stride, int min_d16, int max_d16, const uint8_t* d_mask, int mask_stride);
int sparse_req_check(vo_ctx* ctx, const SparseReq& q, const char* who);
int sparse_ws_prepare(vo_ctx* ctx, SparseWs& ws, hipStream_t stream, bool own_sets, bool with_orb = true);
int orb_ws_alloc(vo_ctx* ctx, OrbWs& o);
void orb_ws_free(OrbWs& o);
void sparse_ws_free(SparseWs& ws);
int sparse_enqueue(vo_ctx* ctx, FrameSlot& f, SparseWs& ws, const SparseReq& q);
static inline bool slot_sparse(const FrameSlot& f) { return f.has_kp && f.kp_depth; }
int lds_allow_big(vo_ctx* ctx, const void* fn);
static inline hipError_t dev_zero(void* p, size_t bytes)
{
    const hipError_t e = hipMemsetAsync(p, 0, bytes, nullptr);
    return e != hipSuccess ? e : hipStreamSynchronize(nullptr);
}
size_t pose_ws_bytes(int nq);
void* xfer_stage(vo_ctx* ctx, size_t bytes);

__device__ __forceinline__ double wave_sum_f64_dpp(double v)
{
#define DPP_ADD64(ctrl, rmask)                                                                             \
    {                                                                                                      \
        const int lo = __builtin_amdgcn_update_dpp(0, __double2loint(v), ctrl, rmask, 0xf, false);         \
        const int hi = __builtin_amdgcn_update_dpp(0, __double2hiint(v), ctrl, rmask, 0xf, false);         \
        v += __hiloint2double(hi, lo);                                                                     \
    }
    DPP_ADD64(0x111, 0xf) DPP_ADD64(0x112, 0xf) DPP_ADD64(0x114, 0xf) DPP_ADD64(0x118, 0xf)
    DPP_ADD64(0x142, 0xa) DPP_ADD64(0x143, 0xc)
#undef DPP_ADD64
    return __hiloint2double(__builtin_amdgcn_readlane(__double2hiint(v), 63), __builtin_amdgcn_readlane(__double2loint(v), 63));
}
template <bool CROSS>
__global__ void k_ratio_compact(const int32_t* idx, const int32_t* dist, int nq, double ratio, const float* xy_q, const float* xy_t,
                                int32_t* q_out, int32_t* t_out, float* xyq_out, float* xyt_out, int32_t* m_out,
                                const uint32_t* colmin, int nt, const uint8_t* rd_q, const uint8_t* rd_t, int loop_max);

int sgbm_run(vo_ctx* ctx, FrameSlot& f, int w, int h, const uint8_t* srcL = nullptr, const uint8_t* srcR = nullptr, bool* deferred = nullptr);
enum { VO_GRP_FULL = 0, VO_GRP_CONSUMER = 1, VO_GRP_FLUSH = 2, VO_GRP_OTHER = 3 };
#define VO_SWEEP_GROUP_FEW_QUEUES 12
static inline int sweep_group_size(const vo_ctx* ctx)
{
    int b = ctx->sweep_group_req > 0 ? ctx->sweep_group_req : (ctx->hw_queues >= ctx->n_engines + 4 ? 1 : VO_SWEEP_GROUP_FEW_QUEUES);
    return b < ctx->n_engines ? b : ctx->n_engines;
}
int sweep_group_close(vo_ctx* ctx, int why);
int engine_behind_chain(vo_ctx* ctx, int engine);
bool sweep_group_has_engine(const vo_ctx* ctx, int engine);
int sweep_group_members(const vo_ctx* ctx);
void sweep_group_free(vo_ctx* ctx);
static inline int sweep_group_close_for(vo_ctx* ctx, const FrameSlot& f) { return f.in_group ? sweep_group_close(ctx, VO_GRP_CONSUMER) : VO_OK; }
int slot_health(vo_ctx* ctx, const FrameSlot& f, int slot);
int orb_prepare_tables(vo_ctx* ctx, int w, int h);
int orb_run(vo_ctx* ctx, FrameSlot* fs, const uint8_t* d_img, int img_stride, int w, int h,
            int nfeatures, int mask_mode, const int16_t* d_disp16, int disp_stride, int min_d16,
            int max_d16, const uint8_t* d_mask, int mask_stride);
#define VO_KNN_SPLITS 16
static inline size_t match_dist_bytes(int kp_cap)
{
    const size_t capq = ((size_t)kp_cap + 63) & ~(size_t)63;
    return capq * 8 + (size_t)VO_KNN_SPLITS * capq * 8 + (capq / 64 + 1) * 4 + capq * 4 + 256;
}
static inline uint32_t* match_colmin(int32_t* d_dist, int kp_cap)
{
    const size_t capq = ((size_t)kp_cap + 63) & ~(size_t)63;
    return (uint32_t*)((uint8_t*)d_dist + capq * 8 + (size_t)VO_KNN_SPLITS * capq * 8 + (capq / 64 + 1) * 4);
}
__device__ __forceinline__ bool knn_mutual(int t, int i, const uint32_t* __restrict__ colmin, int nt)
{
    if (t < 0 || t >= nt) return false;
    const uint32_t key = colmin[t];
    return key != 0xFFFFFFFFu && (key & 0xFFFFu) == (uint32_t)i;
}
enum { MATCH_WS_POSE = 1 };
hipError_t match_ws_alloc(vo_ctx* ctx, vo_ctx::MatchWs& m, int what);
void match_ws_free(vo_ctx::MatchWs& m);
int match_knn2(vo_ctx* ctx, const uint8_t* dq, int nq, const uint8_t* dt, int nt, int32_t* d_idx,
               int32_t* d_dist, int cross = 0, const float* xy_q = nullptr, const float* xy_t = nullptr, float rx = 0.f, float ry = 0.f);
int match_flags_check(vo_ctx* ctx, int match_flags, const char* who, bool loop_ok = false);
struct LoopGate { const uint8_t *rd_a = nullptr, *rd_b = nullptr; int max_h = 0; };
int match_loop_gate(vo_ctx* ctx, const FrameSlot& a, const FrameSlot& b, int match_flags, const char* who, LoopGate* g);
__device__ __forceinline__ bool loop_pass(const uint8_t* __restrict__ rd_q, const uint8_t* __restrict__ rd_t, int q, int t, int loop_max)
{
    const uint4 a0 = ((const uint4*)rd_q)[2 * (size_t)q], a1 = ((const uint4*)rd_q)[2 * (size_t)q + 1];
    const uint4 b0 = ((const uint4*)rd_t)[2 * (size_t)t], b1 = ((const uint4*)rd_t)[2 * (size_t)t + 1];
    const int d = (__popc(a0.x ^ b0.x) + __popc(a0.y ^ b0.y)) + (__popc(a0.z ^ b0.z) + __popc(a0.w ^ b0.w)) +
                  (__popc(a1.x ^ b1.x) + __popc(a1.y ^ b1.y)) + (__popc(a1.z ^ b1.z) + __popc(a1.w ^ b1.w));
    return d <= loop_max;
}
int match_knn2_slots(vo_ctx* ctx, const FrameSlot& a, const FrameSlot& b, int match_flags);
int points3d_launch(vo_ctx* ctx, const int16_t* d_disp16, int w, int h, const float* d_xy, int n,
                    float* d_xyz, uint8_t* d_status);
void host_svd3(const double* A, double* U, double* w, double* Vt);

struct PnpRec {
    int32_t M, n, best_iter, best_count;
    int32_t flags;
    int32_t rstatus, rsteps, pad;
    double Rt[12], Rtr[12];
};
static const size_t PNP_HDR = 1024;
static inline size_t pnp_cap(int kp_cap) { return ((size_t)kp_cap + 15) & ~(size_t)15; }
struct PnpDev { int32_t *hdr, *q, *t; float *X, *uv; };
int pnp_prep_launch(vo_ctx* ctx, FrameSlot& a, FrameSlot& b, double ratio, int cross, const PnpDev& d, const LoopGate& g);

static const size_t MONO_HDR = 4096;
int alt_open(vo_ctx* ctx, int kind, FrameSlot& a, FrameSlot& b, const char* who, int* k_out);
struct AltScope {
    vo_ctx* c;
    vo_ctx::AsyncAlt& p;
    AltScope(vo_ctx* c_, vo_ctx::AsyncAlt& p_) : c(c_), p(p_)
    {
        std::swap(c->stream, p.stream);
        c->mw = &p.mw;
    }
    ~AltScope()
    {
        c->mw = &c->main_mw;
        std::swap(c->stream, p.stream);
    }
    AltScope(const AltScope&) = delete;
    AltScope& operator=(const AltScope&) = delete;
};
int alt_close(vo_ctx* ctx, int kind, int k, FrameSlot& a, FrameSlot& b, int* ticket_out);
int alt_ticket(vo_ctx* ctx, int kind, int ticket, bool args_ok, const char* who);
int alt_wait(vo_ctx* ctx, vo_ctx::AsyncAlt& p);
void alt_free(vo_ctx* ctx);
```

Before: 2070.

## Route grouped dense SGBM work onto two shared lane streams

Adds two shared 'lane' streams. When sweep grouping is active, the dense stages of every member of a sweep group are issued on the same lane stream, which drops the cross-stream event waits, the stagger waits and the swept-chain handoffs between members. Engines switch streams through a new engine_enter helper that records a 'moved' event. With lanes on, the default group size is capped at half the engine count and the number of pose streams is capped to the hardware queue budget, which cuts hardware queue oversubscription. The cost is less concurrency across engines and more complex stream ownership tracking, which brings a risk of ordering bugs.

After: 2168, median of 6. 1.05x the previous value.

```diff
diff --git a/openvo_amd/csrc/match.hip b/openvo_amd/csrc/match.hip
--- a/openvo_amd/csrc/match.hip
+++ b/openvo_amd/csrc/match.hip
@@ -584,6 +584,7 @@
         if (int rc = alt_prepare(ctx, kind, (k + i) % n)) return rc;
     if (int rc = sweep_group_close_for(ctx, a)) return rc;
     if (int rc = sweep_group_close_for(ctx, b)) return rc;
+    if (kind == vo_ctx::ALT_POSE) ctx->alt(kind, k).stream = ctx->pose_streams[k % pose_stream_count(ctx)];
     const hipStream_t st = ctx->alt(kind, k).stream;
     VO_HIP(ctx, hipEventRecord(ctx->ev0, ctx->stream));
     hipError_t e = hipStreamWaitEvent(st, ctx->ev0, 0);
diff --git a/openvo_amd/csrc/orb.hip b/openvo_amd/csrc/orb.hip
--- a/openvo_amd/csrc/orb.hip
+++ b/openvo_amd/csrc/orb.hip
@@ -153,8 +153,7 @@
             ++v0;
         }
     }
-    for (int k = 0; k < vo_ctx::MAX_ENGINES; k++)
-        if (ctx->la_stream[k]) VO_HIP(ctx, hipStreamSynchronize(ctx->la_stream[k]));
+    VO_HIP(ctx, engine_streams_sync(ctx));
     for (int kind : { vo_ctx::ALT_POSE, vo_ctx::ALT_MONO })
         for (int k = 0; k < vo_ctx::alt_count(kind); k++)
             if (ctx->alt(kind, k).stream) VO_HIP(ctx, hipStreamSynchronize(ctx->alt(kind, k).stream));
diff --git a/openvo_amd/csrc/sgbm.hip b/openvo_amd/csrc/sgbm.hip
--- a/openvo_amd/csrc/sgbm.hip
+++ b/openvo_amd/csrc/sgbm.hip
@@ -1383,6 +1383,7 @@
     typedef int (*WeLaunch)(vo_ctx*, const WeJobs&, int, const SgbmGeom&);
     struct Member {
         int engine;
+        hipStream_t stream;
         FrameSlot* f;
         int w, h;
         SgbmGeom g;
@@ -1394,6 +1395,7 @@
     WeLaunch we_launch = nullptr;
     int nstrips = 0;
     int n = 0;
+    hipStream_t lane = nullptr;
     Member m[DG_MAXJOBS];
     bool want_defer = false, did_defer = false;
     Member cand;
@@ -1580,6 +1582,7 @@
         VO_HIP(ctx, hipEventRecord(ctx->ws->done, ctx->stream));
         ctx->ws->done_valid = true;
         ctx->ws->done_on_engine0 = false;
+        ctx->ws->done_lane = nullptr;
     }
     return VO_OK;
 }
@@ -1590,7 +1593,7 @@
     if (deferred) *deferred = false;
     if (ctx->cur_engine < 0 && sweep_group_has_engine(ctx, 0) && (rc = sweep_group_close(ctx, VO_GRP_CONSUMER))) return rc;
     const bool shared = ctx->ws == &ctx->main_ws;
-    if (shared && ctx->ws->done_valid && !(ctx->cur_engine == 0 && ctx->ws->done_on_engine0)) VO_HIP(ctx, hipStreamWaitEvent(ctx->stream, ctx->ws->done, 0));
+    if (shared && ctx->ws->done_valid && !(ctx->cur_engine == 0 && ctx->ws->done_on_engine0) && !(ctx->ws->done_lane && ctx->ws->done_lane == ctx->stream)) VO_HIP(ctx, hipStreamWaitEvent(ctx->stream, ctx->ws->done, 0));
     if (++ctx->sweep_gen_next <= 0) ctx->sweep_gen_next = 1;
     f.disp_gen = ctx->sweep_gen_next;
     const bool defer = deferred && ctx->cur_engine >= 0 && sweep_group_size(ctx) > 1 && ctx->sg.set && ctx->sg.ur < 100 && ctx->sg.mode == 0 &&
@@ -1612,7 +1615,8 @@
                 return rc;
             SweepGroup::Member& m = G->m[G->n++];
             m = G->cand;
-            m.engine = ctx->cur_engine; m.f = &f; m.w = w; m.h = h;
+            m.engine = ctx->cur_engine; m.stream = ctx->stream; m.f = &f; m.w = w; m.h = h;
+            if (G->n == 1) G->lane = stream_is_lane(ctx, ctx->stream) ? ctx->stream : nullptr;
             m.post = post_job(ctx, f);
             G->launch = G->cand_launch; G->we_launch = G->cand_we_launch; G->nstrips = G->cand_nstrips;
             f.in_group = true;
@@ -1622,6 +1626,13 @@
     }
     if (int rcd = sgbm_run_done(ctx)) return rcd;
     return rc;
+}
+
+hipStream_t dense_stream(const vo_ctx* ctx, int engine)
+{
+    if (!lane_mode(ctx) || !ctx->sg.set || ctx->sg.ur >= 100 || ctx->sg.mode != 0) return ctx->la_stream[engine];
+    const SweepGroup* const G = ctx->grp;
+    return G && G->n > 0 && G->lane ? G->lane : ctx->lane[ctx->lane_next];
 }
 
 bool sweep_group_has_engine(const vo_ctx* ctx, int engine)
@@ -1672,6 +1683,20 @@
     }
     a.chain = nullptr;
     return VO_OK;
+}
+
+int engine_enter(vo_ctx* ctx, int engine, hipStream_t target)
+{
+    vo_ctx::SgbmWs& a = ctx->ws_alt[engine];
+    hipStream_t const from = a.on ? a.on : ctx->la_stream[engine];
+    if (from != target) {
+        VO_HIP(ctx, hipEventRecord(a.moved, from));
+        VO_HIP(ctx, hipStreamWaitEvent(target, a.moved, 0));
+    }
+    a.on = target == ctx->la_stream[engine] ? nullptr : target;
+    ctx->lane_used = a.on != nullptr;
+    ctx->stream = target;
+    return engine_behind_chain(ctx, engine);
 }
 
 int sweep_group_close(vo_ctx* ctx, int why)
@@ -1688,6 +1713,12 @@
         MemberScope scope(ctx);
         SweepGroup::Member& last = G->m[n - 1];
         scope.enter(last.engine);
+        hipStream_t const lane = G->lane;
+        G->lane = nullptr;
+        if (lane) {
+            ctx->stream = lane;
+            ctx->lane_next = lane == ctx->lane[0] ? 1 : 0;
+        }
         DiagJobs jobs;
         WeJobs we;
         PostJobs post;
@@ -1701,6 +1732,7 @@
             jobs.j[i + 1] = G->m[i].job; we.j[i + 1] = G->m[i].we; post.j[i + 1] = G->m[i].post;
             main_member |= G->m[i].engine == 0;
             const vo_ctx::SgbmWs& a = ctx->ws_alt[G->m[i].engine];
+            if (lane && G->m[i].stream == lane) continue;
             if (!a.mid_valid || hipStreamWaitEvent(ctx->stream, a.mid, 0) != hipSuccess) rc = vo_fail(ctx, VO_E_HIP, "sweep group: waiting for a member's early stages failed");
         }
         if (!rc && G->we_launch) {
@@ -1718,7 +1750,7 @@
                 rc = sgbm_post_launch(ctx, post, n, last.g, true);
             }
             if (!rc && main_member && ctx->main_ws.done) {
-                if (hipEventRecord(ctx->main_ws.done, ctx->stream) == hipSuccess) { ctx->main_ws.done_valid = true; ctx->main_ws.done_on_engine0 = false; }
+                if (hipEventRecord(ctx->main_ws.done, ctx->stream) == hipSuccess) { ctx->main_ws.done_valid = true; ctx->main_ws.done_on_engine0 = false; ctx->main_ws.done_lane = lane; }
                 else rc = vo_fail(ctx, VO_E_HIP, "hipEventRecord failed");
             }
         }
@@ -1734,17 +1766,18 @@
             }
             for (int i = 0; i < n && !rc; i++)
                 if (hipEventRecord(G->m[i].f->ready, ctx->stream) != hipSuccess) rc = vo_fail(ctx, VO_E_HIP, "hipEventRecord failed");
-            if (!rc && n > 1) {
+            if (!rc && n > 1 && !lane) {
                 if (hipEventRecord(swept, ctx->stream) != hipSuccess) rc = vo_fail(ctx, VO_E_HIP, "hipEventRecord failed");
                 for (int i = 0; i + 1 < n && !rc; i++) ctx->ws_alt[G->m[i].engine].chain = swept;
             }
-            if (!rc && main_member) ctx->main_ws.done_on_engine0 = last.engine == 0;
+            if (!rc && main_member) ctx->main_ws.done_on_engine0 = !lane && last.engine == 0;
         } else if (!rc) {
-            if (n > 1 && hipEventRecord(swept, ctx->stream) != hipSuccess) rc = vo_fail(ctx, VO_E_HIP, "hipEventRecord failed");
+            if (n > 1 && !lane && hipEventRecord(swept, ctx->stream) != hipSuccess) rc = vo_fail(ctx, VO_E_HIP, "hipEventRecord failed");
             if (!rc) rc = sweep_member_back(ctx, last);
             for (int i = 0; i + 1 < n && !rc; i++) {
                 scope.enter(G->m[i].engine);
-                if (hipStreamWaitEvent(ctx->stream, swept, 0) != hipSuccess) rc = vo_fail(ctx, VO_E_HIP, "hipStreamWaitEvent failed");
+                if (lane) ctx->stream = lane;
+                else if (hipStreamWaitEvent(ctx->stream, swept, 0) != hipSuccess) rc = vo_fail(ctx, VO_E_HIP, "hipStreamWaitEvent failed");
                 if (!rc) rc = sweep_member_back(ctx, G->m[i]);
             }
         }
diff --git a/openvo_amd/csrc/vo_ctx.hip b/openvo_amd/csrc/vo_ctx.hip
--- a/openvo_amd/csrc/vo_ctx.hip
+++ b/openvo_amd/csrc/vo_ctx.hip
@@ -14,6 +14,7 @@
 }
 
 static thread_local std::string g_create_err;
+static int lanes_ensure(vo_ctx* ctx);
 
 static const size_t ARENA_BASE = 4096;
 
@@ -174,6 +175,11 @@
         snprintf(ctx->devname, sizeof(ctx->devname), "%s (%s)", prop.name[0] ? prop.name : generic, prop.gcnArchName);
     }
     if ((e = hipStreamCreateWithFlags(&ctx->stream, hipStreamNonBlocking)) != hipSuccess) { g_create_err = hipGetErrorString(e); delete ctx; return VO_E_HIP; }
+    if (const char* e8 = getenv("VO_ENGINES")) { int v = atoi(e8); if (v >= 1 && v <= vo_ctx::MAX_ENGINES) ctx->n_engines = v; }
+    if (const char* eq = getenv("GPU_MAX_HW_QUEUES")) { int v = atoi(eq); if (v >= 1) ctx->hw_queues = v; }
+    if (const char* eg = getenv("VO_SWEEP_GROUP")) { int v = atoi(eg); if (v >= 1 && v <= VO_MAX_SWEEP_GROUP) ctx->sweep_group_req = v; }
+    if (const char* el = getenv("VO_GROUP_LANES")) ctx->lanes_on = atoi(el) != 0;
+    if (lanes_ensure(ctx)) { g_create_err = "hipStreamCreate failed (lane streams)"; vo_destroy(ctx); return VO_E_HIP; }
     (void)hipEventCreate(&ctx->ev0);
     (void)hipEventCreate(&ctx->ev1);
 
@@ -226,7 +232,6 @@
     ctx->sparse_r.n_kp_host = ctx->slot_words + 32;
     DALLOC(ctx->d_sweep_errs, 64);
     if (dev_zero(ctx->d_sweep_errs, 64 * sizeof(int)) != hipSuccess) { g_create_err = "clearing the sweep error counter failed"; vo_destroy(ctx); return VO_E_HIP; }
-    if (const char* e8 = getenv("VO_ENGINES")) { int v = atoi(e8); if (v >= 1 && v <= vo_ctx::MAX_ENGINES) ctx->n_engines = v; }
     {
         const double per_engine = (double)ctx->vol_cells * 2.0 * 5.0 + (double)npx * 64.0;
         size_t free_b = 0, total_b = 0;
@@ -236,9 +241,7 @@
         ctx->engines_fit = fit < 2 ? 2 : fit;
         if (ctx->n_engines > ctx->engines_fit) ctx->n_engines = ctx->engines_fit;
     }
-    if (const char* eq = getenv("GPU_MAX_HW_QUEUES")) { int v = atoi(eq); if (v >= 1) ctx->hw_queues = v; }
-    if (const char* eg = getenv("VO_SWEEP_GROUP")) { int v = atoi(eg); if (v >= 1 && v <= VO_MAX_SWEEP_GROUP) ctx->sweep_group_req = v; }
-    if (const char* e9 = getenv("VO_POSE_STREAMS")) { int v = atoi(e9); if (v >= 1 && v <= vo_ctx::N_POSE_STREAMS) ctx->n_pose_streams = v; }
+    if (const char* e9 = getenv("VO_POSE_STREAMS")) { int v = atoi(e9); if (v >= 1 && v <= vo_ctx::N_POSE_STREAMS) { ctx->n_pose_streams = v; ctx->pose_streams_env = true; } }
     if (const char* e27 = getenv("VO_STAGGER")) ctx->tune_stagger = atoi(e27);
     if (const char* e25 = getenv("VO_DIAG_WAVES")) { const int v = atoi(e25); ctx->tune_diag_nwc = (v == 7 || v == 11 || v == 15) ? v : 0; }
 #ifdef VO_TEST_HOOKS
@@ -249,7 +252,17 @@
     if (const char* e12 = getenv("VO_FAULT_PNP_RANGE")) ctx->fault_pnp_range = atoi(e12);
 #endif
     if (const char* e6 = getenv("VO_SWEEP_TY")) { int v = atoi(e6); if (v >= 4 && v <= 4096) ctx->tune_sweep_ty = v; }
+    if (lanes_ensure(ctx)) { g_create_err = "hipStreamCreate failed (lane streams)"; vo_destroy(ctx); return VO_E_HIP; }
     *out = ctx;
+    return VO_OK;
+}
+
+static int lanes_ensure(vo_ctx* ctx)
+{
+    if (!ctx->lanes_on || sweep_group_size(ctx) <= 1) return VO_OK;
+    for (hipStream_t& l : ctx->lane)
+        if (!l) VO_HIP(ctx, hipStreamCreateWithFlags(&l, hipStreamNonBlocking));
+    if (!ctx->pose_streams[0]) VO_HIP(ctx, hipStreamCreateWithFlags(&ctx->pose_streams[0], hipStreamNonBlocking));
     return VO_OK;
 }
 
@@ -264,7 +277,7 @@
         ctx->stage_cv.notify_all();
         ctx->stage_thread.join();
     }
-    for (int k = 0; k < vo_ctx::MAX_ENGINES; k++) if (ctx->la_stream[k]) (void)hipStreamSynchronize(ctx->la_stream[k]);
+    (void)engine_streams_sync(ctx);
     if (ctx->stream) (void)hipStreamSynchronize(ctx->stream);
     for (int s = 0; s <= VO_NUM_SLOTS; s++) {
         FrameSlot& f = ctx->slots[s];
@@ -297,6 +310,7 @@
         if (a.h2d_done) (void)hipEventDestroy(a.h2d_done);
         if (a.mid) (void)hipEventDestroy(a.mid);
         if (a.swept) (void)hipEventDestroy(a.swept);
+        if (a.moved) (void)hipEventDestroy(a.moved);
         if (ctx->la_stream[k]) (void)hipStreamDestroy(ctx->la_stream[k]);
     }
     for (vo_ctx::HostStage& hs : ctx->host_stage) {
@@ -305,6 +319,7 @@
     }
     if (ctx->ev0) (void)hipEventDestroy(ctx->ev0);
     if (ctx->ev1) (void)hipEventDestroy(ctx->ev1);
+    for (hipStream_t l : ctx->lane) if (l) (void)hipStreamDestroy(l);
     if (ctx->stream) (void)hipStreamDestroy(ctx->stream);
     delete ctx;
 }
@@ -318,6 +333,7 @@
         if (n > ctx->engines_fit) n = ctx->engines_fit;
         ctx->n_engines = n;
         ctx->next_engine %= n;
+        if (int rc = lanes_ensure(ctx)) return rc;
     }
     return ctx->n_engines;
 }
@@ -328,6 +344,7 @@
     if (n > 0) {
         if (int rc = sweep_group_close(ctx, VO_GRP_OTHER)) return rc;
         ctx->sweep_group_req = n > VO_MAX_SWEEP_GROUP ? VO_MAX_SWEEP_GROUP : n;
+        if (int rc = lanes_ensure(ctx)) return rc;
     }
     return sweep_group_size(ctx);
 }
@@ -361,8 +378,7 @@
 {
     if (!ctx) return VO_E_ARG;
     if (int rc = sweep_group_close(ctx, VO_GRP_CONSUMER)) return rc;
-    for (int k = 0; k < vo_ctx::MAX_ENGINES; k++)
-        if (ctx->la_stream[k]) VO_HIP(ctx, hipStreamSynchronize(ctx->la_stream[k]));
+    VO_HIP(ctx, engine_streams_sync(ctx));
     for (int kind : { vo_ctx::ALT_POSE, vo_ctx::ALT_MONO })
         for (int k = 0; k < vo_ctx::alt_count(kind); k++)
             if (ctx->alt(kind, k).stream) VO_HIP(ctx, hipStreamSynchronize(ctx->alt(kind, k).stream));
@@ -625,6 +641,7 @@
     if (!ctx->ws_alt[engine].mid) {
         VO_HIP(ctx, hipEventCreateWithFlags(&ctx->ws_alt[engine].mid, hipEventDisableTiming));
         VO_HIP(ctx, hipEventCreateWithFlags(&ctx->ws_alt[engine].swept, hipEventDisableTiming));
+        VO_HIP(ctx, hipEventCreateWithFlags(&ctx->ws_alt[engine].moved, hipEventDisableTiming));
     }
     if (!ctx->la_stage[engine]) {
         VO_HIP(ctx, hipMalloc((void**)&ctx->la_stage[engine], ctx->stage_bytes * 2 + 256));
@@ -710,9 +727,11 @@
     if (sp) { f.mono_serial = 0; f.kp_params[0] = f.kp_params[1] = f.kp_params[2] = f.kp_params[3] = -1; }
     {
         EngineScope on_engine(ctx, engine);
-        rc = engine_behind_chain(ctx, engine);
+        hipStream_t const target = sp ? ctx->la_stream[engine] : dense_stream(ctx, engine);
+        const bool on_lane = stream_is_lane(ctx, target);
+        rc = engine_enter(ctx, engine, target);
         const int stagger = ctx->tune_stagger >= 0 ? ctx->tune_stagger : (7 * ctx->n_engines + 8) / 16;
-        if (!sp && stagger > 0 && stagger < ctx->n_engines) {
+        if (!sp && !on_lane && stagger > 0 && stagger < ctx->n_engines) {
             vo_ctx::SgbmWs& p = ctx->ws_alt[(engine - stagger + ctx->n_engines) % ctx->n_engines];
             if (p.mid_valid) (void)hipStreamWaitEvent(ctx->stream, p.mid, 0);
         }
@@ -842,7 +861,7 @@
     f.w = w; f.h = h; f.has_kp = false; f.kp_depth = false; f.sp_pending = false; f.n_kp = 0; f.kp_pending = false; f.has_disp = false;
     {
         EngineScope on_engine(ctx, engine);
-        rc = engine_behind_chain(ctx, engine);
+        rc = engine_enter(ctx, engine, ctx->la_stream[engine]);
         if (!rc) rc = slot_before_overwrite(ctx, f);
         if (!rc) {
             StageTimer t(ctx, VO_T_UPLOAD);
@@ -1206,8 +1225,7 @@
     *n_out = 0;
     if (ctx->ev_used == 0) return VO_OK;
     VO_HIP(ctx, hipSetDevice(ctx->device));
-    for (int k = 0; k < vo_ctx::MAX_ENGINES; k++)
-        if (ctx->la_stream[k]) VO_HIP(ctx, hipStreamSynchronize(ctx->la_stream[k]));
+    VO_HIP(ctx, engine_streams_sync(ctx));
     for (int kind : { vo_ctx::ALT_POSE, vo_ctx::ALT_MONO })
         for (int k = 0; k < vo_ctx::alt_count(kind); k++)
             if (ctx->alt(kind, k).stream) VO_HIP(ctx, hipStreamSynchronize(ctx->alt(kind, k).stream));
@@ -1266,8 +1284,7 @@
     bytes &= ~(int64_t)4095;
     if (bytes <= 0 || !ctx->ws->C || !ctx->ws->S) return vo_fail(ctx, VO_E_STATE, "vo_measure_copy: no volumes to copy between");
     VO_HIP(ctx, hipSetDevice(ctx->device));
-    for (int k = 0; k < vo_ctx::MAX_ENGINES; k++)
-        if (ctx->la_stream[k]) VO_HIP(ctx, hipStreamSynchronize(ctx->la_stream[k]));
+    VO_HIP(ctx, engine_streams_sync(ctx));
     VO_HIP(ctx, hipStreamSynchronize(ctx->stream));
     hipEvent_t e0, e1;
     VO_HIP(ctx, hipEventCreate(&e0));
diff --git a/openvo_amd/csrc/vo_internal.h b/openvo_amd/csrc/vo_internal.h
--- a/openvo_amd/csrc/vo_internal.h
+++ b/openvo_amd/csrc/vo_internal.h
@@ -107,6 +107,10 @@
     hipStream_t stream = nullptr;
     static const int MAX_ENGINES = 24;
     hipStream_t la_stream[MAX_ENGINES] = {};
+    hipStream_t lane[2] = {nullptr, nullptr};
+    bool lanes_on = true;
+    bool lane_used = false;
+    int lane_next = 0;
     int cur_engine = -1;
     int tune_stagger = -1;
     uint8_t* la_stage[MAX_ENGINES] = {};
@@ -123,6 +127,7 @@
         hipEvent_t done = nullptr;
         bool done_valid = false;
         bool done_on_engine0 = false;
+        hipStream_t done_lane = nullptr;
         bool ready = false;
         OrbWs orb;
         uint8_t* pinned = nullptr;
@@ -132,6 +137,8 @@
         bool mid_valid = false;
         hipEvent_t swept = nullptr;
         hipEvent_t chain = nullptr;
+        hipStream_t on = nullptr;
+        hipEvent_t moved = nullptr;
     } ws_alt[MAX_ENGINES];
     SgbmWs main_ws;
     SgbmWs* ws = &main_ws;
@@ -226,6 +233,7 @@
     static const int N_POSE_ALT = VO_NUM_POSE_ASYNC;
     static const int N_POSE_STREAMS = 3;
     int n_pose_streams = N_POSE_STREAMS;
+    bool pose_streams_env = false;
     hipStream_t pose_streams[N_POSE_STREAMS] = {};
     struct PoseAlt : AsyncAlt {
         int slot_a = -1, slot_b = -1;
@@ -358,11 +366,31 @@
 #define VO_SWEEP_GROUP_FEW_QUEUES 12
 static inline int sweep_group_size(const vo_ctx* ctx)
 {
-    int b = ctx->sweep_group_req > 0 ? ctx->sweep_group_req : (ctx->hw_queues >= ctx->n_engines + 4 ? 1 : VO_SWEEP_GROUP_FEW_QUEUES);
+    int few = VO_SWEEP_GROUP_FEW_QUEUES;
+    if (ctx->lanes_on && few > ctx->n_engines / 2) few = ctx->n_engines >= 2 ? ctx->n_engines / 2 : 1;
+    int b = ctx->sweep_group_req > 0 ? ctx->sweep_group_req : (ctx->hw_queues >= ctx->n_engines + 4 ? 1 : few);
     return b < ctx->n_engines ? b : ctx->n_engines;
+}
+static inline bool lane_mode(const vo_ctx* ctx) { return ctx->lanes_on && ctx->lane[0] && ctx->lane[1] && sweep_group_size(ctx) > 1; }
+static inline int pose_stream_count(const vo_ctx* ctx)
+{
+    int n = ctx->n_pose_streams;
+    if (!ctx->pose_streams_env && ctx->lane_used && lane_mode(ctx) && n > ctx->hw_queues - 3) n = ctx->hw_queues - 3 > 1 ? ctx->hw_queues - 3 : 1;
+    return n;
+}
+static inline bool stream_is_lane(const vo_ctx* ctx, hipStream_t s) { return s && (s == ctx->lane[0] || s == ctx->lane[1]); }
+static inline hipError_t engine_streams_sync(const vo_ctx* ctx)
+{
+    for (int k = 0; k < 2; k++)
+        if (ctx->lane[k]) { const hipError_t e = hipStreamSynchronize(ctx->lane[k]); if (e != hipSuccess) return e; }
+    for (int k = 0; k < vo_ctx::MAX_ENGINES; k++)
+        if (ctx->la_stream[k]) { const hipError_t e = hipStreamSynchronize(ctx->la_stream[k]); if (e != hipSuccess) return e; }
+    return hipSuccess;
 }
 int sweep_group_close(vo_ctx* ctx, int why);
 int engine_behind_chain(vo_ctx* ctx, int engine);
+int engine_enter(vo_ctx* ctx, int engine, hipStream_t target);
+hipStream_t dense_stream(const vo_ctx* ctx, int engine);
 bool sweep_group_has_engine(const vo_ctx* ctx, int engine);
 int sweep_group_members(const vo_ctx* ctx);
 void sweep_group_free(vo_ctx* ctx);
```
